# clejacquet/rust-wgpu-raytracing

Hardware: AMD Instinct MI355X
Metric: Mray/s (higher is better)
Workload: dtype f32; 1 GPU; suzanne_lowpoly.obj 1920x1080 1spp primary rays, reference camera + 2 spheres (configs[1]); width=1920, height=1080, spp=1, bounces=0, faces=111, partition=single GPU, frames_in_flight=2, device=AMD Radeon Graphics (gfx950:sramecc+:xnack-)

## Files before the change

include/rwr_hip.h:

```cpp
#ifndef RWR_HIP_H
#define RWR_HIP_H

#include <stddef.h>
#include <stdint.h>

#ifdef __cplusplus
extern "C" {
#endif

#if defined(__GNUC__)
#define RWR_API __attribute__((visibility("default")))
#else
#define RWR_API
#endif

typedef enum rwr_status {
    RWR_OK = 0,
    RWR_ERR_INVALID_ARGUMENT = -1,
    RWR_ERR_HIP = -2,
    RWR_ERR_NOT_READY = -3,
    RWR_ERR_IO = -4,
    RWR_ERR_PARSE = -5,
    RWR_ERR_UNSUPPORTED = -6
} rwr_status;


typedef struct rwr_camera_inv_uniform {
    float viewmodel_inv[4][4];
    float proj_inv[4][4];
    float origin[3];
    uint32_t _padding;
} rwr_camera_inv_uniform;

typedef struct rwr_screen {
    uint32_t width, height;
} rwr_screen;

typedef struct rwr_model_vertex_small {
    float position[3];
    float pad0;
    float tex_coords[2];
    float pad1[2];
} rwr_model_vertex_small;

typedef struct rwr_model_face_small {
    uint32_t indices[3];
    uint32_t pad0;
} rwr_model_face_small;

typedef struct rwr_material_data {
    float ambient[3];  float pad0;
    float diffuse[3];  float pad1;
    float specular[3]; float pad2;
} rwr_material_data;

typedef struct rwr_sphere_buffer_data {
    float center[3];
    float radius;
} rwr_sphere_buffer_data;

typedef struct rwr_triangle_buffer_data {
    float p0[3]; float pad0;
    float p1[3]; float pad1;
    float p2[3]; float pad2;
} rwr_triangle_buffer_data;

typedef struct rwr_instance_raw {
    float model[4][4];
} rwr_instance_raw;

typedef struct rwr_camera {
    float eye[3];
    float target[3];
    float up[3];
    float aspect;
    float fovy;
    float znear;
    float zfar;
} rwr_camera;

typedef struct rwr_render_params {
    uint32_t spp;
    uint32_t max_bounces;
    uint32_t seed;
    uint32_t flags;
} rwr_render_params;

enum {
    RWR_FLAG_AUX_OUTPUTS = 1u << 0,
    RWR_FLAG_NO_CULL     = 1u << 1,
    RWR_FLAG_USE_BVH     = 1u << 2,
    RWR_FLAG_ORTHO_RAYS  = 1u << 3,
    RWR_FLAG_NORMAL_MAP  = 1u << 4,
    RWR_FLAG_ACCUMULATE  = 1u << 5,
    RWR_FLAG_MULTI_BOUNCE = 1u << 6,
    RWR_FLAG_SHADOWS = 1u << 7,
    RWR_FLAG_DENOISE = 1u << 8,
    RWR_FLAG_SKY = 1u << 9,
    RWR_FLAG_MIRRORS = 1u << 10,
    RWR_FLAG_GLASS = 1u << 11,
    RWR_FLAG_REPROJECT = 1u << 12,
    RWR_FLAG_GLOSSY = 1u << 13
};

#define RWR_MAX_BOUNCES 8u

#define RWR_MAX_SPHERES 8
#define RWR_MAX_TRIANGLES 8


typedef struct rwr_context rwr_context;


RWR_API int rwr_ctx_create(int device_id, rwr_context **out_ctx);
RWR_API void rwr_ctx_destroy(rwr_context *ctx);
RWR_API const char *rwr_last_error_string(void);
RWR_API int rwr_device_count(int *out_count);
RWR_API int rwr_ctx_device_info(rwr_context *ctx, char *name, size_t name_cap, int *cu_count, int *wave_size);

RWR_API int rwr_ctx_set_frames_in_flight(rwr_context *ctx, uint32_t n);

RWR_API int rwr_ctx_set_stream(rwr_context *ctx, void *hip_stream);
RWR_API void *rwr_ctx_get_stream(rwr_context *ctx);


RWR_API int rwr_scene_upload_mesh(rwr_context *ctx,
                                  const rwr_model_vertex_small *verts, uint32_t n_verts,
                                  const rwr_model_face_small *faces, uint32_t n_faces,
                                  const rwr_material_data *material,
                                  const uint8_t *rgba8_srgb, uint32_t tex_w, uint32_t tex_h);

RWR_API int rwr_scene_clear(rwr_context *ctx);
RWR_API int rwr_scene_add_mesh(rwr_context *ctx,
                               const rwr_model_vertex_small *verts, uint32_t n_verts,
                               const rwr_model_face_small *faces, uint32_t n_faces,
                               const rwr_material_data *material,
                               const uint8_t *rgba8_srgb, uint32_t tex_w, uint32_t tex_h);
RWR_API int rwr_scene_commit(rwr_context *ctx);

RWR_API int rwr_scene_set_normal_map(rwr_context *ctx, uint32_t part, const uint8_t *rgba8_linear, uint32_t tex_w, uint32_t tex_h);
RWR_API int rwr_scene_part_count(rwr_context *ctx, uint32_t *n_parts);

RWR_API int rwr_scene_set_part_mirror(rwr_context *ctx, uint32_t part, const float *reflectance);
RWR_API int rwr_scene_set_sphere_mirror(rwr_context *ctx, uint32_t sphere, const float *reflectance);
RWR_API int rwr_scene_get_part_mirror(rwr_context *ctx, uint32_t part, int *is_mirror, float reflectance[3]);
RWR_API int rwr_scene_get_sphere_mirror(rwr_context *ctx, uint32_t sphere, int *is_mirror, float reflectance[3]);

RWR_API int rwr_scene_set_part_glass(rwr_context *ctx, uint32_t part, float ior, const float *tint);
RWR_API int rwr_scene_set_sphere_glass(rwr_context *ctx, uint32_t sphere, float ior, const float *tint);
RWR_API int rwr_scene_get_part_glass(rwr_context *ctx, uint32_t part, int *is_glass, float *ior, float tint[3]);
RWR_API int rwr_scene_get_sphere_glass(rwr_context *ctx, uint32_t sphere, int *is_glass, float *ior, float tint[3]);

RWR_API int rwr_scene_set_part_gloss(rwr_context *ctx, uint32_t part, const float *reflectance, float roughness);
RWR_API int rwr_scene_set_sphere_gloss(rwr_context *ctx, uint32_t sphere, const float *reflectance, float roughness);
RWR_API int rwr_scene_get_part_gloss(rwr_context *ctx, uint32_t part, int *is_glossy, float reflectance[3], float *roughness);
RWR_API int rwr_scene_get_sphere_gloss(rwr_context *ctx, uint32_t sphere, int *is_glossy, float reflectance[3], float *roughness);

RWR_API int rwr_scene_set_spheres(rwr_context *ctx, const rwr_sphere_buffer_data *spheres, uint32_t n);

RWR_API int rwr_scene_set_triangles(rwr_context *ctx, const rwr_triangle_buffer_data *triangles, uint32_t n);

RWR_API int rwr_scene_set_instances(rwr_context *ctx, const rwr_instance_raw *instances, uint32_t n);


RWR_API int rwr_resize(rwr_context *ctx, const rwr_screen *screen);

RWR_API int rwr_render(rwr_context *ctx, const rwr_camera_inv_uniform *camera, const rwr_render_params *params);

RWR_API int rwr_render_rows(rwr_context *ctx, const rwr_camera_inv_uniform *camera,
                            const rwr_render_params *params, uint32_t row_begin, uint32_t row_end);

#define RWR_STRIP_ROWS 8u
RWR_API int rwr_render_strips(rwr_context *ctx, const rwr_camera_inv_uniform *camera,
                              const rwr_render_params *params, uint32_t first_strip, uint32_t strip_stride);

RWR_API int rwr_synchronize(rwr_context *ctx);

RWR_API int rwr_readback(rwr_context *ctx, uint8_t *rgba8, float *depth,
                         float *rgba_f32, int32_t *obj_id, float *hit_t);

RWR_API int rwr_get_device_targets(rwr_context *ctx, void **d_rgba8, void **d_depth);

#define RWR_DIST_ID_BYTES 128
RWR_API int rwr_dist_get_unique_id(uint8_t id[RWR_DIST_ID_BYTES]);
RWR_API int rwr_dist_init(rwr_context *ctx, int rank, int world, const uint8_t id[RWR_DIST_ID_BYTES]);
RWR_API int rwr_dist_band(uint32_t rank, uint32_t world, uint32_t height, uint32_t *row_begin, uint32_t *row_end);
RWR_API int rwr_dist_gather_rgba8(rwr_context *ctx, int root);
RWR_API int rwr_dist_gather_strips_rgba8(rwr_context *ctx, int root);
RWR_API int rwr_dist_frame(rwr_context *ctx, void **d_rgba8);
RWR_API int rwr_dist_readback(rwr_context *ctx, uint8_t *rgba8);
RWR_API int rwr_dist_barrier(rwr_context *ctx);
RWR_API int rwr_dist_destroy(rwr_context *ctx);

typedef struct rwr_strip_layout {
    uint32_t n_strips, strips, rows, recv_row, recv_rows_total, owns_tail;
} rwr_strip_layout;
RWR_API int rwr_dist_strip_layout(uint32_t rank, uint32_t world, uint32_t height, rwr_strip_layout *out);
RWR_API int rwr_dist_host_pack_strips(uint32_t rank, uint32_t world, uint32_t width, uint32_t height,
                                      const uint8_t *frame_rgba8, uint8_t *message);
RWR_API int rwr_dist_host_deal_strips(uint32_t world, uint32_t width, uint32_t height, const uint8_t *recv, uint8_t *frame_rgba8);
RWR_API int rwr_host_texture_quads(const uint8_t *rgba8_srgb, uint32_t tex_w, uint32_t tex_h, uint32_t *out);
RWR_API int rwr_dist_loopback_deposit(rwr_context *ctx, uint32_t rank, uint32_t world, int strips);
RWR_API int rwr_dist_loopback_finish(rwr_context *ctx, uint32_t world, int strips);

RWR_API int rwr_timer_begin(rwr_context *ctx);
RWR_API int rwr_timer_end(rwr_context *ctx, float *elapsed_ms);
RWR_API int rwr_timer_stop(rwr_context *ctx);
RWR_API int rwr_timer_elapsed(rwr_context *ctx, float *elapsed_ms);

RWR_API int rwr_ctx_set_kernel_timing(rwr_context *ctx, uint32_t every_n);
RWR_API int rwr_kernel_timing_stats(rwr_context *ctx, double *mean_us, uint32_t *count);

RWR_API int rwr_last_render_stats(rwr_context *ctx, uint64_t *primary_rays, uint64_t *bounce_rays);

RWR_API int rwr_frame_setup_launches(rwr_context *ctx, uint64_t *launches);

RWR_API int rwr_ray_plane_stats(rwr_context *ctx, uint64_t *builds, uint64_t *frames);

RWR_API int rwr_debug_tile_classes(rwr_context *ctx, uint32_t *classes, size_t capacity, uint32_t *grid_x, uint32_t *grid_y);

RWR_API int rwr_debug_tile_cover(rwr_context *ctx, uint32_t *cover, size_t capacity, uint32_t *grid_x, uint32_t *grid_y);

RWR_API int rwr_tile_cover_stats(rwr_context *ctx, uint64_t *frames, uint64_t *tiles_last);

RWR_API int rwr_last_shadow_stats(rwr_context *ctx, uint64_t *shadow_rays, uint64_t *occluded);

RWR_API int rwr_last_glass_stats(rwr_context *ctx, uint64_t *reflected, uint64_t *transmitted, uint64_t *tir);

RWR_API int rwr_last_gloss_stats(rwr_context *ctx, uint64_t *glossy_rays);

RWR_API int rwr_accum_reset(rwr_context *ctx);
RWR_API int rwr_accum_samples(rwr_context *ctx, uint64_t *samples);

typedef struct rwr_denoise_params {
    uint32_t iterations;
    float sigma_color, normal_cos_min, depth_rel;
} rwr_denoise_params;
RWR_API int rwr_denoise_set_params(rwr_context *ctx, const rwr_denoise_params *params);
RWR_API int rwr_denoise_get_params(rwr_context *ctx, rwr_denoise_params *out);

typedef struct rwr_sky_params {
    float zenith[3];
    float horizon[3];
} rwr_sky_params;
#define RWR_SKY_DEFAULTS {{0.5f, 0.7f, 1.0f}, {1.0f, 1.0f, 1.0f}}
#define RWR_SKY_COMPONENT_MAX 16.0f
RWR_API int rwr_sky_set_params(rwr_context *ctx, const rwr_sky_params *params);
RWR_API int rwr_sky_get_params(rwr_context *ctx, rwr_sky_params *out);

typedef struct rwr_reproject_params {
    uint32_t max_history;
    float normal_cos_min, depth_rel;
} rwr_reproject_params;
RWR_API int rwr_reproject_set_params(rwr_context *ctx, const rwr_reproject_params *params);
RWR_API int rwr_reproject_get_params(rwr_context *ctx, rwr_reproject_params *out);
RWR_API int rwr_reproject_reset(rwr_context *ctx);
RWR_API int rwr_reproject_frames(rwr_context *ctx, uint64_t *frames);
RWR_API int rwr_last_reproject_stats(rwr_context *ctx, uint64_t *reused, uint64_t *fresh, uint64_t *background);
RWR_API int rwr_reproject_readback(rwr_context *ctx, float *history_len);

RWR_API int rwr_selftest_exact_math(rwr_context *ctx, uint32_t normalize_count, uint32_t seed, uint64_t out4[4]);

RWR_API int rwr_selftest_exact_div(rwr_context *ctx, uint32_t count, uint32_t seed, uint64_t out4[4]);

RWR_API int rwr_measure_valu_clock(rwr_context *ctx, uint32_t waves_per_simd, double out4[4]);
RWR_API int rwr_clock_probe_start(rwr_context *ctx, uint32_t micros);
RWR_API int rwr_clock_probe_read(rwr_context *ctx, double *shader_mhz);


RWR_API int rwr_camera_build_inv_uniform(const rwr_camera *camera, rwr_camera_inv_uniform *out);

enum { RWR_KEY_FORWARD = 1, RWR_KEY_BACKWARD = 2, RWR_KEY_LEFT = 4, RWR_KEY_RIGHT = 8,
       RWR_KEY_UP = 16, RWR_KEY_DOWN = 32 };
RWR_API int rwr_circle_controller_update(float speed, uint32_t pressed_keys, rwr_camera *camera);

typedef struct rwr_model rwr_model;
RWR_API int rwr_load_model_compute(const char *res_dir, const char *file_name, rwr_model **out_model);
RWR_API void rwr_model_free(rwr_model *model);
RWR_API int rwr_model_info(const rwr_model *model, uint32_t *n_meshes, uint32_t *n_materials,
                           uint32_t *n_verts, uint32_t *n_faces, uint32_t *tex_w, uint32_t *tex_h);
RWR_API const rwr_model_vertex_small *rwr_model_vertices(const rwr_model *model);
RWR_API const rwr_model_face_small *rwr_model_faces(const rwr_model *model);
RWR_API const rwr_material_data *rwr_model_material(const rwr_model *model);
RWR_API const uint8_t *rwr_model_texture_rgba8(const rwr_model *model);
RWR_API int rwr_scene_upload_model(rwr_context *ctx, const rwr_model *model);
RWR_API int rwr_model_part_count(const rwr_model *model, uint32_t *n_parts);
RWR_API int rwr_model_part(const rwr_model *model, uint32_t part,
                           const rwr_model_vertex_small **verts, uint32_t *n_verts,
                           const rwr_model_face_small **faces, uint32_t *n_faces,
                           rwr_material_data *material, const uint8_t **rgba8, uint32_t *tex_w, uint32_t *tex_h);
RWR_API int rwr_scene_upload_model_all(rwr_context *ctx, const rwr_model *model);
RWR_API int rwr_model_part_normal_map(const rwr_model *model, uint32_t part, const uint8_t **rgba8, uint32_t *tex_w, uint32_t *tex_h);

RWR_API int rwr_decode_image_rgba8(const uint8_t *bytes, size_t n_bytes,
                                   uint8_t **out_rgba, uint32_t *out_w, uint32_t *out_h);
RWR_API void rwr_free(void *p);

RWR_API int rwr_write_png_rgba8(const char *path, const uint8_t *rgba8, uint32_t width, uint32_t height,
                                int flip_vertical, int encode_srgb);

RWR_API int rwr_make_instance_grid(uint32_t per_row, float space_between, rwr_instance_raw *out);

#ifdef __cplusplus
}
#endif
#endif
```

rust-wgpu-raytracing_amd/__init__.py:

```python
from __future__ import annotations

import ctypes as C
import os
import subprocess

import numpy as np

_HERE = os.path.dirname(os.path.abspath(__file__))
LIB_PATH = os.environ.get("RWR_HIP_LIB") or os.path.join(_HERE, "lib", "librwr_hip.so")
RES_DIR = os.path.join(_HERE, "res")
HEADER_PATH = os.path.join(os.path.dirname(_HERE), "include", "rwr_hip.h")

CAMERA_INV_DTYPE = np.dtype(
    [("viewmodel_inv", "<f4", (4, 4)), ("proj_inv", "<f4", (4, 4)), ("origin", "<f4", (3,)), ("_padding", "<u4")])
SCREEN_DTYPE = np.dtype([("width", "<u4"), ("height", "<u4")])
VERTEX_DTYPE = np.dtype([("position", "<f4", (3,)), ("pad0", "<f4"), ("tex_coords", "<f4", (2,)), ("pad1", "<f4", (2,))])
FACE_DTYPE = np.dtype([("indices", "<u4", (3,)), ("pad0", "<u4")])
MATERIAL_DTYPE = np.dtype([("ambient", "<f4", (3,)), ("pad0", "<f4"), ("diffuse", "<f4", (3,)), ("pad1", "<f4"),
                           ("specular", "<f4", (3,)), ("pad2", "<f4")])
SPHERE_DTYPE = np.dtype([("center", "<f4", (3,)), ("radius", "<f4")])
INSTANCE_DTYPE = np.dtype([("model", "<f4", (4, 4))])
TRIANGLE_DTYPE = np.dtype([("p0", "<f4", (3,)), ("pad0", "<f4"), ("p1", "<f4", (3,)), ("pad1", "<f4"),
                           ("p2", "<f4", (3,)), ("pad2", "<f4")])
CAMERA_DTYPE = np.dtype([("eye", "<f4", (3,)), ("target", "<f4", (3,)), ("up", "<f4", (3,)),
                         ("aspect", "<f4"), ("fovy", "<f4"), ("znear", "<f4"), ("zfar", "<f4")])
PARAMS_DTYPE = np.dtype([("spp", "<u4"), ("max_bounces", "<u4"), ("seed", "<u4"), ("flags", "<u4")])
assert (CAMERA_INV_DTYPE.itemsize, VERTEX_DTYPE.itemsize, FACE_DTYPE.itemsize, MATERIAL_DTYPE.itemsize,
        SPHERE_DTYPE.itemsize, INSTANCE_DTYPE.itemsize, CAMERA_DTYPE.itemsize) == (144, 32, 16, 48, 16, 64, 52)

FLAG_AUX_OUTPUTS, FLAG_NO_CULL, FLAG_USE_BVH = 1, 2, 4
FLAG_ORTHO_RAYS = 1 << 3
FLAG_NORMAL_MAP = 1 << 4
FLAG_ACCUMULATE = 1 << 5
FLAG_MULTI_BOUNCE = 1 << 6
FLAG_SHADOWS = 1 << 7
FLAG_DENOISE = 1 << 8
DENOISE_PARAMS_DTYPE = np.dtype([("iterations", "<u4"), ("sigma_color", "<f4"), ("normal_cos_min", "<f4"), ("depth_rel", "<f4")])
FLAG_SKY = 1 << 9
SKY_PARAMS_DTYPE = np.dtype([("zenith", "<f4", 3), ("horizon", "<f4", 3)])
FLAG_MIRRORS = 1 << 10
FLAG_GLASS = 1 << 11
FLAG_REPROJECT = 1 << 12
FLAG_GLOSSY = 1 << 13
REPROJECT_PARAMS_DTYPE = np.dtype([("max_history", "<u4"), ("normal_cos_min", "<f4"), ("depth_rel", "<f4")])
MAX_BOUNCES = 8
FLAG_DEBUG_COUNTS, FLAG_ONE_PIXEL_PER_LANE = 1 << 16, 1 << 17
KEY_FORWARD, KEY_BACKWARD, KEY_LEFT, KEY_RIGHT, KEY_UP, KEY_DOWN = 1, 2, 4, 8, 16, 32
OK, ERR_INVALID_ARGUMENT, ERR_HIP, ERR_NOT_READY, ERR_IO, ERR_PARSE, ERR_UNSUPPORTED = 0, -1, -2, -3, -4, -5, -6

REFERENCE_SPHERES = [((0.6, 0.5, -4.0), 0.4), ((0.4, 0.4, -3.0), 0.4)]
CONTROLLER_SPEED = 0.2


class RwrError(RuntimeError):
    def __init__(self, code: int, message: str):
        super().__init__(f"rwr error {code}: {message}")
        self.code = code
        self.message = message


def build(force: bool = False) -> str:
    cmd = ["make", "-C", _HERE, "-j4"] + (["-B"] if force else [])
    r = subprocess.run(cmd, capture_output=True, text=True)
    if r.returncode != 0:
        raise RuntimeError("building librwr_hip.so failed:\n" + r.stdout + r.stderr)
    return LIB_PATH


_lib = None


def lib() -> C.CDLL:
    global _lib
    if _lib is not None:
        return _lib
    if not os.path.exists(LIB_PATH):
        raise FileNotFoundError(
            f"{LIB_PATH} is missing: run `python -c 'import __graft_entry__ as g; g.build()'` "
            "(there is no CPU fallback for the render path)")
    try:
        import torch
    except Exception:
        pass
    L = C.CDLL(LIB_PATH)
    vp, u32, i32, f32 = C.c_void_p, C.c_uint32, C.c_int, C.c_float
    L.rwr_last_error_string.restype = C.c_char_p
    L.rwr_ctx_get_stream.restype = vp
    for name in ("rwr_model_vertices", "rwr_model_faces", "rwr_model_material", "rwr_model_texture_rgba8"):
        getattr(L, name).restype = vp
        getattr(L, name).argtypes = [vp]
    sigs = {
        "rwr_ctx_create": [i32, vp], "rwr_ctx_destroy": [vp], "rwr_device_count": [vp],
        "rwr_ctx_device_info": [vp, vp, C.c_size_t, vp, vp], "rwr_ctx_set_stream": [vp, vp], "rwr_ctx_get_stream": [vp],
        "rwr_scene_upload_mesh": [vp, vp, u32, vp, u32, vp, vp, u32, u32],
        "rwr_scene_clear": [vp], "rwr_scene_add_mesh": [vp, vp, u32, vp, u32, vp, vp, u32, u32], "rwr_scene_commit": [vp],
        "rwr_model_part_count": [vp, vp], "rwr_model_part": [vp, u32, vp, vp, vp, vp, vp, vp, vp, vp],
        "rwr_scene_upload_model_all": [vp, vp], "rwr_model_part_normal_map": [vp, u32, vp, vp, vp],
        "rwr_scene_set_normal_map": [vp, u32, vp, u32, u32], "rwr_scene_part_count": [vp, vp],
        "rwr_scene_set_spheres": [vp, vp, u32], "rwr_scene_set_triangles": [vp, vp, u32], "rwr_scene_set_instances": [vp, vp, u32],
        "rwr_resize": [vp, vp], "rwr_render": [vp, vp, vp], "rwr_render_rows": [vp, vp, vp, u32, u32], "rwr_render_strips": [vp, vp, vp, u32, u32],
        "rwr_synchronize": [vp], "rwr_readback": [vp, vp, vp, vp, vp, vp], "rwr_get_device_targets": [vp, vp, vp],
        "rwr_timer_begin": [vp], "rwr_timer_end": [vp, vp], "rwr_timer_stop": [vp], "rwr_timer_elapsed": [vp, vp], "rwr_last_render_stats": [vp, vp, vp],
        "rwr_last_shadow_stats": [vp, vp, vp], "rwr_frame_setup_launches": [vp, vp], "rwr_ray_plane_stats": [vp, vp, vp],
        "rwr_debug_tile_classes": [vp, vp, C.c_size_t, vp, vp],
        "rwr_debug_tile_cover": [vp, vp, C.c_size_t, vp, vp], "rwr_tile_cover_stats": [vp, vp, vp],
        "rwr_accum_reset": [vp], "rwr_accum_samples": [vp, vp],
        "rwr_denoise_set_params": [vp, vp], "rwr_denoise_get_params": [vp, vp],
        "rwr_sky_set_params": [vp, vp], "rwr_sky_get_params": [vp, vp],
        "rwr_reproject_set_params": [vp, vp], "rwr_reproject_get_params": [vp, vp], "rwr_reproject_reset": [vp],
        "rwr_reproject_frames": [vp, vp], "rwr_last_reproject_stats": [vp, vp, vp, vp], "rwr_reproject_readback": [vp, vp],
        "rwr_scene_set_part_mirror": [vp, u32, vp], "rwr_scene_set_sphere_mirror": [vp, u32, vp],
        "rwr_scene_get_part_mirror": [vp, u32, vp, vp], "rwr_scene_get_sphere_mirror": [vp, u32, vp, vp],
        "rwr_scene_set_part_glass": [vp, u32, f32, vp], "rwr_scene_set_sphere_glass": [vp, u32, f32, vp],
        "rwr_scene_get_part_glass": [vp, u32, vp, vp, vp], "rwr_scene_get_sphere_glass": [vp, u32, vp, vp, vp],
        "rwr_last_glass_stats": [vp, vp, vp, vp],
        "rwr_scene_set_part_gloss": [vp, u32, vp, f32], "rwr_scene_set_sphere_gloss": [vp, u32, vp, f32],
        "rwr_scene_get_part_gloss": [vp, u32, vp, vp, vp], "rwr_scene_get_sphere_gloss": [vp, u32, vp, vp, vp],
        "rwr_last_gloss_stats": [vp, vp],
        "rwr_camera_build_inv_uniform": [vp, vp], "rwr_circle_controller_update": [f32, u32, vp],
        "rwr_load_model_compute": [C.c_char_p, C.c_char_p, vp], "rwr_model_free": [vp],
        "rwr_model_info": [vp, vp, vp, vp, vp, vp, vp], "rwr_scene_upload_model": [vp, vp],
        "rwr_decode_image_rgba8": [vp, C.c_size_t, vp, vp, vp], "rwr_free": [vp],
        "rwr_make_instance_grid": [u32, f32, vp],
        "rwr_write_png_rgba8": [C.c_char_p, vp, u32, u32, i32, i32],
        "rwr_ctx_set_kernel_timing": [vp, u32], "rwr_kernel_timing_stats": [vp, vp, vp],
        "rwr_selftest_exact_math": [vp, u32, u32, vp], "rwr_selftest_exact_div": [vp, u32, u32, vp], "rwr_ctx_set_frames_in_flight": [vp, u32],
        "rwr_dist_get_unique_id": [vp], "rwr_dist_init": [vp, i32, i32, vp], "rwr_dist_band": [u32, u32, u32, vp, vp],
        "rwr_dist_gather_rgba8": [vp, i32], "rwr_dist_gather_strips_rgba8": [vp, i32], "rwr_dist_frame": [vp, vp], "rwr_dist_readback": [vp, vp],
        "rwr_dist_barrier": [vp], "rwr_dist_destroy": [vp],
        "rwr_dist_strip_layout": [u32, u32, u32, vp], "rwr_dist_host_pack_strips": [u32, u32, u32, u32, vp, vp],
        "rwr_dist_host_deal_strips": [u32, u32, u32, vp, vp], "rwr_host_texture_quads": [vp, u32, u32, vp],
        "rwr_dist_loopback_deposit": [vp, u32, u32, i32], "rwr_dist_loopback_finish": [vp, u32, i32],
        "rwr_measure_valu_clock": [vp, u32, vp], "rwr_clock_probe_start": [vp, u32], "rwr_clock_probe_read": [vp, vp],
    }
    _NEWER_ENTRY_POINTS = ("rwr_last_shadow_stats", "rwr_denoise_set_params", "rwr_denoise_get_params", "rwr_frame_setup_launches", "rwr_ray_plane_stats", "rwr_debug_tile_classes", "rwr_debug_tile_cover", "rwr_tile_cover_stats",
                           "rwr_sky_set_params", "rwr_sky_get_params", "rwr_scene_set_part_mirror", "rwr_scene_set_sphere_mirror",
                           "rwr_scene_get_part_mirror", "rwr_scene_get_sphere_mirror", "rwr_scene_set_part_glass", "rwr_scene_set_sphere_glass",
                           "rwr_scene_get_part_glass", "rwr_scene_get_sphere_glass", "rwr_last_glass_stats",
                           "rwr_reproject_set_params", "rwr_reproject_get_params", "rwr_reproject_reset", "rwr_reproject_frames",
                           "rwr_last_reproject_stats", "rwr_reproject_readback", "rwr_scene_set_part_gloss", "rwr_scene_set_sphere_gloss",
                           "rwr_scene_get_part_gloss", "rwr_scene_get_sphere_gloss", "rwr_last_gloss_stats")
    for name, argtypes in sigs.items():
        fn = getattr(L, name, None)
        if fn is None and name in _NEWER_ENTRY_POINTS and os.environ.get("RWR_HIP_LIB"):
            continue
        if fn is None:
            raise AttributeError(f"{LIB_PATH} does not export {name}")
        fn.argtypes = argtypes
        if name not in ("rwr_ctx_destroy", "rwr_model_free", "rwr_free", "rwr_ctx_get_stream"):
            fn.restype = C.c_int
        elif name != "rwr_ctx_get_stream":
            fn.restype = None
    _lib = L
    return L


def _check(rc: int):
    if rc != OK:
        raise RwrError(rc, lib().rwr_last_error_string().decode("utf-8", "replace"))


def _p(a):
    return None if a is None else a.ctypes.data_as(C.c_void_p)


def make_camera(eye=(0, 0, 0), target=(0, 0, -1), up=(0, 1, 0), aspect=1.0, fovy=60.0, znear=0.1, zfar=100.0):
    cam = np.zeros(1, dtype=CAMERA_DTYPE)
    cam["eye"], cam["target"], cam["up"] = eye, target, up
    cam["aspect"], cam["fovy"], cam["znear"], cam["zfar"] = aspect, fovy, znear, zfar
    return cam


def camera_build_inv_uniform(cam: np.ndarray) -> np.ndarray:
    out = np.zeros(1, dtype=CAMERA_INV_DTYPE)
    _check(lib().rwr_camera_build_inv_uniform(_p(cam), _p(out)))
    return out


def circle_controller_update(cam: np.ndarray, keys: int, speed: float = CONTROLLER_SPEED) -> np.ndarray:
    cam = cam.copy()
    _check(lib().rwr_circle_controller_update(speed, keys, _p(cam)))
    return cam


def make_screen(w: int, h: int) -> np.ndarray:
    s = np.zeros(1, dtype=SCREEN_DTYPE)
    s["width"], s["height"] = w, h
    return s


def make_spheres(spec=REFERENCE_SPHERES) -> np.ndarray:
    s = np.zeros(len(spec), dtype=SPHERE_DTYPE)
    for i, (c, r) in enumerate(spec):
        s[i]["center"], s[i]["radius"] = c, r
    return s


def make_triangles(spec=()) -> np.ndarray:
    t = np.zeros(len(spec), dtype=TRIANGLE_DTYPE)
    for i, (p0, p1, p2) in enumerate(spec):
        t[i]["p0"], t[i]["p1"], t[i]["p2"] = p0, p1, p2
    return t


def make_params(spp=1, max_bounces=0, seed=0, flags=0) -> np.ndarray:
    p = np.zeros(1, dtype=PARAMS_DTYPE)
    p["spp"], p["max_bounces"], p["seed"], p["flags"] = spp, max_bounces, seed, flags
    return p


def make_instance_grid(per_row: int, space_between: float = 3.0) -> np.ndarray:
    out = np.zeros(per_row * per_row, dtype=INSTANCE_DTYPE)
    _check(lib().rwr_make_instance_grid(per_row, space_between, _p(out)))
    return out


def decode_image_rgba8(data: bytes) -> np.ndarray:
    buf = np.frombuffer(data, dtype=np.uint8)
    out = C.c_void_p()
    w, h = C.c_uint32(), C.c_uint32()
    _check(lib().rwr_decode_image_rgba8(_p(buf), len(data), C.byref(out), C.byref(w), C.byref(h)))
    try:
        arr = np.ctypeslib.as_array(C.cast(out, C.POINTER(C.c_uint8)), shape=(h.value, w.value, 4)).copy()
    finally:
        lib().rwr_free(out)
    return arr


def write_png(path: str, rgba8: np.ndarray, flip_vertical: bool = True, encode_srgb: bool = False):
    rgba8 = np.ascontiguousarray(rgba8, dtype=np.uint8)
    h, w = rgba8.shape[:2]
    _check(lib().rwr_write_png_rgba8(path.encode(), _p(rgba8), w, h, int(flip_vertical), int(encode_srgb)))


def load_model_compute(file_name: str, res_dir: str = RES_DIR) -> dict:
    L = lib()
    h = C.c_void_p()
    _check(L.rwr_load_model_compute(res_dir.encode(), file_name.encode(), C.byref(h)))
    try:
        n = [C.c_uint32() for _ in range(6)]
        _check(L.rwr_model_info(h, *[C.byref(x) for x in n]))
        n_meshes, n_materials, n_verts, n_faces, tw, th = [x.value for x in n]
        verts = np.frombuffer(C.string_at(L.rwr_model_vertices(h), n_verts * 32), dtype=VERTEX_DTYPE).copy()
        faces = np.frombuffer(C.string_at(L.rwr_model_faces(h), n_faces * 16), dtype=FACE_DTYPE).copy()
        material = np.frombuffer(C.string_at(L.rwr_model_material(h), 48), dtype=MATERIAL_DTYPE).copy()
        tex = np.frombuffer(C.string_at(L.rwr_model_texture_rgba8(h), tw * th * 4), dtype=np.uint8).reshape(th, tw, 4).copy()
        nmap = _part_normal_map(L, h, 0)
    finally:
        L.rwr_model_free(h)
    return {"vertices": verts, "faces": faces, "material": material, "texture": tex, "normal_map": nmap,
            "n_meshes": n_meshes, "n_materials": n_materials}


def _part_normal_map(L, h, part):
    pn, nw, nh = C.c_void_p(), C.c_uint32(), C.c_uint32()
    _check(L.rwr_model_part_normal_map(h, part, C.byref(pn), C.byref(nw), C.byref(nh)))
    if not pn.value:
        return None
    return np.frombuffer(C.string_at(pn, nw.value * nh.value * 4), dtype=np.uint8).reshape(nh.value, nw.value, 4).copy()



def load_model_parts(file_name: str, res_dir: str = RES_DIR) -> list:
    L = lib()
    h = C.c_void_p()
    _check(L.rwr_load_model_compute(res_dir.encode(), file_name.encode(), C.byref(h)))
    parts = []
    try:
        n = C.c_uint32()
        _check(L.rwr_model_part_count(h, C.byref(n)))
        for i in range(n.value):
            pv, pf, pt = C.c_void_p(), C.c_void_p(), C.c_void_p()
            nv, nf, tw, th = C.c_uint32(), C.c_uint32(), C.c_uint32(), C.c_uint32()
            mat = np.zeros(1, dtype=MATERIAL_DTYPE)
            _check(L.rwr_model_part(h, i, C.byref(pv), C.byref(nv), C.byref(pf), C.byref(nf), _p(mat), C.byref(pt), C.byref(tw), C.byref(th)))
            parts.append({
                "vertices": np.frombuffer(C.string_at(pv, nv.value * 32), dtype=VERTEX_DTYPE).copy(),
                "faces": np.frombuffer(C.string_at(pf, nf.value * 16), dtype=FACE_DTYPE).copy(),
                "material": mat,
                "texture": np.frombuffer(C.string_at(pt, tw.value * th.value * 4), dtype=np.uint8).reshape(th.value, tw.value, 4).copy(),
                "normal_map": _part_normal_map(L, h, i),
            })
    finally:
        L.rwr_model_free(h)
    return parts


DIST_ID_BYTES = 128
STRIP_ROWS = 8


def dist_get_unique_id() -> bytes:
    buf = (C.c_uint8 * DIST_ID_BYTES)()
    _check(lib().rwr_dist_get_unique_id(buf))
    return bytes(buf)


def dist_band(rank: int, world: int, height: int) -> tuple[int, int]:
    a, b = C.c_uint32(), C.c_uint32()
    _check(lib().rwr_dist_band(rank, world, height, C.byref(a), C.byref(b)))
    return a.value, b.value


class _StripLayout(C.Structure):
    _fields_ = [(n, C.c_uint32) for n in ("n_strips", "strips", "rows", "recv_row", "recv_rows_total", "owns_tail")]


def dist_strip_layout(rank: int, world: int, height: int) -> dict:
    out = _StripLayout()
    _check(lib().rwr_dist_strip_layout(rank, world, height, C.byref(out)))
    return {n: int(getattr(out, n)) for n, _ in _StripLayout._fields_}


def dist_host_pack_strips(rank: int, world: int, frame: np.ndarray) -> np.ndarray:
    frame = np.ascontiguousarray(frame, np.uint8)
    h, w = frame.shape[:2]
    lay = dist_strip_layout(rank, world, h)
    msg = np.zeros((max(1, lay["strips"] * STRIP_ROWS), w, 4), np.uint8)
    _check(lib().rwr_dist_host_pack_strips(rank, world, w, h, _p(frame), _p(msg)))
    return msg[:lay["rows"]]


def host_texture_quads(rgba8: np.ndarray) -> np.ndarray:
    rgba8 = np.ascontiguousarray(rgba8, np.uint8)
    h, w = rgba8.shape[:2]
    out = np.zeros((h + 1, w + 1, 4), np.uint32)
    _check(lib().rwr_host_texture_quads(_p(rgba8), w, h, _p(out)))
    return out


def dist_host_deal_strips(world: int, recv: np.ndarray, height: int) -> np.ndarray:
    recv = np.ascontiguousarray(recv, np.uint8)
    w = recv.shape[1]
    assert recv.shape[0] == dist_strip_layout(0, world, height)["recv_rows_total"]
    frame = np.zeros((height, w, 4), np.uint8)
    _check(lib().rwr_dist_host_deal_strips(world, w, height, _p(recv), _p(frame)))
    return frame


def device_count() -> int:
    n = C.c_int()
    lib().rwr_device_count(C.byref(n))
    return n.value


class Context:

    def __init__(self, device_id: int = 0):
        self._h = C.c_void_p()
        _check(lib().rwr_ctx_create(device_id, C.byref(self._h)))
        self.width = self.height = 0

    def close(self):
        if getattr(self, "_h", None):
            lib().rwr_ctx_destroy(self._h)
            self._h = None

    def __del__(self):
        try:
            self.close()
        except Exception:
            pass

    def __enter__(self):
        return self

    def __exit__(self, *exc):
        self.close()

    def device_info(self) -> dict:
        name = C.create_string_buffer(256)
        cu, ws = C.c_int(), C.c_int()
        _check(lib().rwr_ctx_device_info(self._h, name, 256, C.byref(cu), C.byref(ws)))
        return {"name": name.value.decode(), "cu_count": cu.value, "wave_size": ws.value}

    def set_stream(self, hip_stream: int | None):
        _check(lib().rwr_ctx_set_stream(self._h, C.c_void_p(hip_stream or 0)))

    def upload_mesh(self, vertices, faces, material, texture):
        vertices = np.ascontiguousarray(vertices, dtype=VERTEX_DTYPE)
        faces = np.ascontiguousarray(faces, dtype=FACE_DTYPE)
        material = np.ascontiguousarray(material, dtype=MATERIAL_DTYPE)
        texture = np.ascontiguousarray(texture, dtype=np.uint8)
        th, tw = texture.shape[:2] if texture.ndim == 3 else (0, 0)
        _check(lib().rwr_scene_upload_mesh(self._h, _p(vertices), len(vertices), _p(faces), len(faces),
                                           _p(material), _p(texture), tw, th))

    def upload_model(self, model: dict):
        self.upload_mesh(model["vertices"], model["faces"], model["material"], model["texture"])
        if model.get("normal_map") is not None and len(model["faces"]):
            self.set_normal_map(0, model["normal_map"])

    def set_normal_map(self, part: int, rgba8_linear):
        if rgba8_linear is None:
            _check(lib().rwr_scene_set_normal_map(self._h, part, None, 0, 0))
            return
        t = np.ascontiguousarray(rgba8_linear, dtype=np.uint8)
        _check(lib().rwr_scene_set_normal_map(self._h, part, _p(t), t.shape[1], t.shape[0]))

    def upload_parts(self, parts: list):
        _check(lib().rwr_scene_clear(self._h))
        for m in parts:
            vertices = np.ascontiguousarray(m["vertices"], dtype=VERTEX_DTYPE)
            faces = np.ascontiguousarray(m["faces"], dtype=FACE_DTYPE)
            material = np.ascontiguousarray(m["material"], dtype=MATERIAL_DTYPE)
            texture = np.ascontiguousarray(m["texture"], dtype=np.uint8)
            th, tw = texture.shape[:2]
            _check(lib().rwr_scene_add_mesh(self._h, _p(vertices), len(vertices), _p(faces), len(faces), _p(material),
                                            _p(texture), tw, th))
            if m.get("normal_map") is not None and len(faces):
                n = C.c_uint32()
                _check(lib().rwr_scene_part_count(self._h, C.byref(n)))
                self.set_normal_map(n.value - 1, m["normal_map"])
        _check(lib().rwr_scene_commit(self._h))

    def set_spheres(self, spheres):
        spheres = np.ascontiguousarray(spheres, dtype=SPHERE_DTYPE)
        _check(lib().rwr_scene_set_spheres(self._h, _p(spheres) if len(spheres) else None, len(spheres)))

    @staticmethod
    def _reflectance(reflectance):
        if reflectance is None:
            return None
        r = np.ascontiguousarray(reflectance, dtype=np.float32)
        if r.shape != (3,):
            raise ValueError("reflectance: three floats, or None")
        return r

    def set_part_mirror(self, part: int, reflectance=(1.0, 1.0, 1.0)):
        r = self._reflectance(reflectance)
        _check(lib().rwr_scene_set_part_mirror(self._h, part, _p(r)))

    def set_sphere_mirror(self, sphere: int, reflectance=(1.0, 1.0, 1.0)):
        r = self._reflectance(reflectance)
        _check(lib().rwr_scene_set_sphere_mirror(self._h, sphere, _p(r)))

    def _get_mirror(self, fn, index: int):
        on = C.c_int(0)
        r = np.zeros(3, np.float32)
        _check(fn(self._h, index, C.byref(on), _p(r)))
        return r if on.value else None

    def get_part_mirror(self, part: int):
        return self._get_mirror(lib().rwr_scene_get_part_mirror, part)

    def get_sphere_mirror(self, sphere: int):
        return self._get_mirror(lib().rwr_scene_get_sphere_mirror, sphere)

    def set_part_glass(self, part: int, ior: float = 1.5, tint=(1.0, 1.0, 1.0)):
        t = self._reflectance(tint)
        _check(lib().rwr_scene_set_part_glass(self._h, part, ior, _p(t)))

    def set_sphere_glass(self, sphere: int, ior: float = 1.5, tint=(1.0, 1.0, 1.0)):
        t = self._reflectance(tint)
        _check(lib().rwr_scene_set_sphere_glass(self._h, sphere, ior, _p(t)))

    def _get_glass(self, fn, index: int):
        on = C.c_int(0)
        ior = C.c_float(0.0)
        t = np.zeros(3, np.float32)
        _check(fn(self._h, index, C.byref(on), C.byref(ior), _p(t)))
        return (float(ior.value), t) if on.value else None

    def get_part_glass(self, part: int):
        return self._get_glass(lib().rwr_scene_get_part_glass, part)

    def get_sphere_glass(self, sphere: int):
        return self._get_glass(lib().rwr_scene_get_sphere_glass, sphere)

    def last_glass_stats(self):
        a, b, c = C.c_uint64(0), C.c_uint64(0), C.c_uint64(0)
        _check(lib().rwr_last_glass_stats(self._h, C.byref(a), C.byref(b), C.byref(c)))
        return int(a.value), int(b.value), int(c.value)

    def set_part_gloss(self, part: int, roughness: float = 0.25, reflectance=(1.0, 1.0, 1.0)):
        r = self._reflectance(reflectance)
        _check(lib().rwr_scene_set_part_gloss(self._h, part, _p(r), roughness))

    def set_sphere_gloss(self, sphere: int, roughness: float = 0.25, reflectance=(1.0, 1.0, 1.0)):
        r = self._reflectance(reflectance)
        _check(lib().rwr_scene_set_sphere_gloss(self._h, sphere, _p(r), roughness))

    def _get_gloss(self, fn, index: int):
        on = C.c_int(0)
        rough = C.c_float(0.0)
        r = np.zeros(3, np.float32)
        _check(fn(self._h, index, C.byref(on), _p(r), C.byref(rough)))
        return (float(rough.value), r) if on.value else None

    def get_part_gloss(self, part: int):
        return self._get_gloss(lib().rwr_scene_get_part_gloss, part)

    def get_sphere_gloss(self, sphere: int):
        return self._get_gloss(lib().rwr_scene_get_sphere_gloss, sphere)

    def last_gloss_stats(self):
        a = C.c_uint64(0)
        _check(lib().rwr_last_gloss_stats(self._h, C.byref(a)))
        return int(a.value)

    def set_triangles(self, triangles):
        triangles = np.ascontiguousarray(triangles, dtype=TRIANGLE_DTYPE)
        _check(lib().rwr_scene_set_triangles(self._h, _p(triangles) if len(triangles) else None, len(triangles)))

    def set_instances(self, instances):
        n = 0 if instances is None else len(instances)
        arr = None if n == 0 else np.ascontiguousarray(instances, dtype=INSTANCE_DTYPE)
        _check(lib().rwr_scene_set_instances(self._h, _p(arr), n))

    def resize(self, width: int, height: int):
        _check(lib().rwr_resize(self._h, _p(make_screen(width, height))))
        self.width, self.height = width, height

    def render(self, cam_inv, params=None, rows=None, strips=None):
        if strips is not None:
            _check(lib().rwr_render_strips(self._h, _p(cam_inv), _p(params), strips[0], strips[1]))
        elif rows is None:
            _check(lib().rwr_render(self._h, _p(cam_inv), _p(params)))
        else:
            _check(lib().rwr_render_rows(self._h, _p(cam_inv), _p(params), rows[0], rows[1]))

    def render_call(self, cam_inv, params, rows=None, strips=None):
        fn, h = (lib().rwr_render_strips if strips is not None else lib().rwr_render_rows), self._h
        a, b = _p(cam_inv), _p(params)
        if strips is None and rows is None:
            rows = (0, self.height)
        r0, r1 = (C.c_uint32(strips[0]), C.c_uint32(strips[1])) if strips is not None else (C.c_uint32(rows[0]), C.c_uint32(rows[1]))

        def call(_keep=(cam_inv, params)):
            rc = fn(h, a, b, r0, r1)
            if rc:
                _check(rc)

        return call

    def loop_call(self, cam: np.ndarray, keys: list[int], params, speed: float = CONTROLLER_SPEED, render: bool = True):
        L, h = lib(), self._h
        upd, inv, ren = L.rwr_circle_controller_update, L.rwr_camera_build_inv_uniform, L.rwr_render
        uni = np.zeros(1, dtype=CAMERA_INV_DTYPE)
        pc, pu, pp = _p(cam), _p(uni), _p(params)
        sp = C.c_float(speed)
        masks = [C.c_uint32(k) for k in keys]
        state = [0]

        def call(_keep=(cam, uni, params)):
            i = state[0]
            state[0] = i + 1 if i + 1 < len(masks) else 0
            rc = upd(sp, masks[i], pc) or inv(pc, pu) or (ren(h, pu, pp) if render else 0)
            if rc:
                _check(rc)

        return call

    def synchronize(self):
        _check(lib().rwr_synchronize(self._h))

    def readback(self, aux: bool = False) -> dict:
        h, w = self.height, self.width
        out = {"color": np.zeros((h, w, 4), np.uint8), "depth": np.zeros((h, w), np.float32)}
        if aux:
            out["color_f32"] = np.zeros((h, w, 4), np.float32)
            out["obj_id"] = np.zeros((h, w), np.int32)
            out["hit_t"] = np.zeros((h, w), np.float32)
        _check(lib().rwr_readback(self._h, _p(out["color"]), _p(out["depth"]), _p(out.get("color_f32")),
                                  _p(out.get("obj_id")), _p(out.get("hit_t"))))
        return out

    def device_targets(self) -> tuple[int, int]:
        a, b = C.c_void_p(), C.c_void_p()
        _check(lib().rwr_get_device_targets(self._h, C.byref(a), C.byref(b)))
        return a.value, b.value

    def timer_begin(self):
        _check(lib().rwr_timer_begin(self._h))

    def timer_end(self) -> float:
        ms = C.c_float()
        _check(lib().rwr_timer_end(self._h, C.byref(ms)))
        return ms.value

    def timer_stop(self):
        _check(lib().rwr_timer_stop(self._h))

    def timer_elapsed(self) -> float:
        ms = C.c_float()
        _check(lib().rwr_timer_elapsed(self._h, C.byref(ms)))
        return ms.value

    def set_frames_in_flight(self, n: int):
        _check(lib().rwr_ctx_set_frames_in_flight(self._h, n))

    def set_kernel_timing(self, every_n: int):
        _check(lib().rwr_ctx_set_kernel_timing(self._h, every_n))

    def kernel_timing_stats(self) -> tuple[float, int]:
        mean, n = C.c_double(), C.c_uint32()
        _check(lib().rwr_kernel_timing_stats(self._h, C.byref(mean), C.byref(n)))
        return mean.value, n.value

    def selftest_exact_math(self, normalize_count: int = 1 << 30, seed: int = 1) -> tuple[int, int, int, int]:
        out = (C.c_uint64 * 4)()
        _check(lib().rwr_selftest_exact_math(self._h, normalize_count, seed, out))
        return tuple(int(v) for v in out)

    def selftest_exact_div(self, count: int = 1 << 30, seed: int = 1) -> tuple[int, int, int, int]:
        out = (C.c_uint64 * 4)()
        _check(lib().rwr_selftest_exact_div(self._h, count, seed, out))
        return tuple(int(v) for v in out)

    def measure_valu_clock(self, waves_per_simd: int = 8) -> dict:
        out = (C.c_double * 4)()
        _check(lib().rwr_measure_valu_clock(self._h, waves_per_simd, out))
        return {"shader_mhz": out[0], "cycles_per_v_fma_f32": out[1], "cycles_per_v_pk_fma_f32": out[2], "shader_mhz_pk": out[3]}

    def dist_init(self, rank: int, world: int, unique_id: bytes):
        assert len(unique_id) == DIST_ID_BYTES
        buf = (C.c_uint8 * DIST_ID_BYTES).from_buffer_copy(unique_id)
        _check(lib().rwr_dist_init(self._h, rank, world, buf))

    def dist_gather(self, root: int = 0):
        _check(lib().rwr_dist_gather_rgba8(self._h, root))

    def dist_gather_call(self, root: int = 0, strips: bool = False):
        fn, h, r = (lib().rwr_dist_gather_strips_rgba8 if strips else lib().rwr_dist_gather_rgba8), self._h, C.c_int(root)

        def call():
            rc = fn(h, r)
            if rc:
                _check(rc)

        return call

    def dist_loopback_deposit(self, rank: int, world: int, strips: bool = True):
        _check(lib().rwr_dist_loopback_deposit(self._h, rank, world, 1 if strips else 0))

    def dist_loopback_finish(self, world: int, strips: bool = True):
        _check(lib().rwr_dist_loopback_finish(self._h, world, 1 if strips else 0))

    def dist_readback(self) -> np.ndarray:
        out = np.zeros((self.height, self.width, 4), np.uint8)
        _check(lib().rwr_dist_readback(self._h, _p(out)))
        return out

    def dist_barrier(self):
        _check(lib().rwr_dist_barrier(self._h))

    def dist_destroy(self):
        _check(lib().rwr_dist_destroy(self._h))

    def clock_probe_start(self, micros: int):
        _check(lib().rwr_clock_probe_start(self._h, micros))

    def clock_probe_read(self) -> float:
        mhz = C.c_double()
        _check(lib().rwr_clock_probe_read(self._h, C.byref(mhz)))
        return mhz.value

    def last_render_stats(self) -> tuple[int, int]:
        a, b = C.c_uint64(), C.c_uint64()
        _check(lib().rwr_last_render_stats(self._h, C.byref(a), C.byref(b)))
        return a.value, b.value

    def frame_setup_launches(self) -> int:
        n = C.c_uint64()
        _check(lib().rwr_frame_setup_launches(self._h, C.byref(n)))
        return n.value

    def ray_plane_stats(self) -> tuple[int, int]:
        a, b = C.c_uint64(), C.c_uint64()
        _check(lib().rwr_ray_plane_stats(self._h, C.byref(a), C.byref(b)))
        return a.value, b.value

    def tile_classes(self) -> np.ndarray:
        gx, gy = C.c_uint32(), C.c_uint32()
        _check(lib().rwr_debug_tile_classes(self._h, None, 0, C.byref(gx), C.byref(gy)))
        words = np.empty(4 * gx.value * gy.value, np.uint32)
        _check(lib().rwr_debug_tile_classes(self._h, _p(words), words.size, C.byref(gx), C.byref(gy)))
        return np.ascontiguousarray(words.reshape(gy.value, gx.value, 2, 2).transpose(0, 2, 1, 3).reshape(2 * gy.value, 2 * gx.value))

    def tile_cover(self) -> np.ndarray:
        gx, gy = C.c_uint32(), C.c_uint32()
        _check(lib().rwr_debug_tile_cover(self._h, None, 0, C.byref(gx), C.byref(gy)))
        words = np.empty(4 * gx.value * gy.value, np.uint32)
        _check(lib().rwr_debug_tile_cover(self._h, _p(words), words.size, C.byref(gx), C.byref(gy)))
        return np.ascontiguousarray(words.reshape(gy.value, gx.value, 2, 2).transpose(0, 2, 1, 3).reshape(2 * gy.value, 2 * gx.value))

    def tile_cover_stats(self) -> tuple[int, int]:
        a, b = C.c_uint64(), C.c_uint64()
        _check(lib().rwr_tile_cover_stats(self._h, C.byref(a), C.byref(b)))
        return a.value, b.value

    def last_shadow_stats(self) -> tuple[int, int]:
        a, b = C.c_uint64(), C.c_uint64()
        _check(lib().rwr_last_shadow_stats(self._h, C.byref(a), C.byref(b)))
        return a.value, b.value

    def accum_reset(self):
        _check(lib().rwr_accum_reset(self._h))

    def accum_samples(self) -> int:
        n = C.c_uint64()
        _check(lib().rwr_accum_samples(self._h, C.byref(n)))
        return n.value

    def set_denoise_params(self, iterations=None, sigma_color=None, normal_cos_min=None, depth_rel=None):
        given = {"iterations": iterations, "sigma_color": sigma_color, "normal_cos_min": normal_cos_min, "depth_rel": depth_rel}
        if all(v is None for v in given.values()):
            _check(lib().rwr_denoise_set_params(self._h, None))
            return
        p = np.zeros(1, dtype=DENOISE_PARAMS_DTYPE)
        for k, v in self.denoise_params().items():
            p[k] = v if given[k] is None else given[k]
        _check(lib().rwr_denoise_set_params(self._h, _p(p)))

    def denoise_params(self) -> dict:
        p = np.zeros(1, dtype=DENOISE_PARAMS_DTYPE)
        _check(lib().rwr_denoise_get_params(self._h, _p(p)))
        return {"iterations": int(p["iterations"][0]), "sigma_color": float(p["sigma_color"][0]),
                "normal_cos_min": float(p["normal_cos_min"][0]), "depth_rel": float(p["depth_rel"][0])}

    def set_reproject_params(self, max_history=None, normal_cos_min=None, depth_rel=None):
        given = {"max_history": max_history, "normal_cos_min": normal_cos_min, "depth_rel": depth_rel}
        if all(v is None for v in given.values()):
            _check(lib().rwr_reproject_set_params(self._h, None))
            return
        p = np.zeros(1, dtype=REPROJECT_PARAMS_DTYPE)
        for k, v in self.reproject_params().items():
            p[k] = v if given[k] is None else given[k]
        _check(lib().rwr_reproject_set_params(self._h, _p(p)))

    def reproject_params(self) -> dict:
        p = np.zeros(1, dtype=REPROJECT_PARAMS_DTYPE)
        _check(lib().rwr_reproject_get_params(self._h, _p(p)))
        return {"max_history": int(p["max_history"][0]), "normal_cos_min": float(p["normal_cos_min"][0]), "depth_rel": float(p["depth_rel"][0])}

    def reproject_reset(self):
        _check(lib().rwr_reproject_reset(self._h))

    def reproject_frames(self) -> int:
        n = C.c_uint64()
        _check(lib().rwr_reproject_frames(self._h, C.byref(n)))
        return n.value

    def last_reproject_stats(self) -> tuple[int, int, int]:
        a, b, c = C.c_uint64(0), C.c_uint64(0), C.c_uint64(0)
        _check(lib().rwr_last_reproject_stats(self._h, C.byref(a), C.byref(b), C.byref(c)))
        return int(a.value), int(b.value), int(c.value)

    def reproject_history(self) -> np.ndarray:
        out = np.zeros((self.height, self.width), np.float32)
        _check(lib().rwr_reproject_readback(self._h, _p(out)))
        return out

    def sky_set_params(self, zenith=None, horizon=None):
        if zenith is None and horizon is None:
            _check(lib().rwr_sky_set_params(self._h, None))
            return
        p = np.zeros(1, dtype=SKY_PARAMS_DTYPE)
        now = self.sky_get_params()
        p["zenith"] = now["zenith"] if zenith is None else np.asarray(zenith, np.float32)
        p["horizon"] = now["horizon"] if horizon is None else np.asarray(horizon, np.float32)
        _check(lib().rwr_sky_set_params(self._h, _p(p)))

    def sky_get_params(self) -> dict:
        p = np.zeros(1, dtype=SKY_PARAMS_DTYPE)
        _check(lib().rwr_sky_get_params(self._h, _p(p)))
        return {"zenith": p["zenith"][0].copy(), "horizon": p["horizon"][0].copy()}


def csrc_tree() -> str:
    import hashlib

    h = hashlib.sha256()
    files = []
    for sub in ("csrc", "host"):
        d = os.path.join(_HERE, sub)
        files += [os.path.join(d, f) for f in os.listdir(d) if f.endswith((".h", ".hpp", ".hip", ".cpp"))]
    files += [os.path.join(_HERE, "Makefile"), HEADER_PATH]
    for f in sorted(files):
        h.update(os.path.relpath(f, _HERE).encode())
        with open(f, "rb") as fh:
            h.update(fh.read())
    return h.hexdigest()[:16]


def exported_symbols_declared_in_header() -> list[str]:
    import re

    with open(HEADER_PATH, "r") as fh:
        text = fh.read()
    return sorted(set(re.findall(r"RWR_API\s+[^;(]*?\b(rwr_[a-z0-9_]+)\s*\(", text)))
```

rust-wgpu-raytracing_amd/csrc/context.cpp:

```cpp
#include <hip/hip_runtime.h>

#include <algorithm>
#include <cmath>
#include <cstdarg>
#include <cstdio>
#include <cstdlib>
#include <new>
#include <string>
#include <vector>

#include "rwr_context.h"

namespace rwr {

static thread_local std::string g_last_error;

int set_error(int code, const char *fmt, ...)
{
    char buf[512];
    va_list ap;
    va_start(ap, fmt);
    vsnprintf(buf, sizeof buf, fmt, ap);
    va_end(ap);
    g_last_error = buf;
    return code;
}

hipError_t ensure_frame_buffers(rwr_context *ctx)
{
    const uint32_t total = (uint32_t)instanced_faces(ctx->n_faces, ctx->n_instances);
    for (uint32_t i = 0; i < ctx->n_slots; i++) {
        FrameSlot &sl = ctx->slots[i];
        const void *const before[4] = {sl.d_ftris.ptr, sl.d_tnum.ptr, sl.d_ray_colp.ptr, sl.d_ray_row.ptr};
        hipError_t e = hipSuccess;
        if (total && (e = sl.d_ftris.ensure(total)) == hipSuccess) e = sl.d_tnum.ensure(total);
        if (e == hipSuccess && ctx->screen.width) {
            e = sl.d_ray_colp.ensure(2u * (size_t)(((ctx->screen.width + 63u) / 64u) * 32u));
            if (e == hipSuccess) e = sl.d_ray_row.ensure(ctx->screen.height + 8u);
        }
        if (before[0] != sl.d_ftris.ptr || before[1] != sl.d_tnum.ptr || before[2] != sl.d_ray_colp.ptr || before[3] != sl.d_ray_row.ptr)
            sl.records_key.clear();
        if (before[2] != sl.d_ray_colp.ptr || before[3] != sl.d_ray_row.ptr) sl.forget_ray_plane();
        if (e != hipSuccess) return e;
    }
    return hipSuccess;
}

}

using namespace rwr;

namespace {

hipError_t ensure_slot_targets(rwr_context *ctx, uint32_t i)
{
    FrameSlot &sl = ctx->slots[i];
    const size_t n = (size_t)ctx->screen.width * ctx->screen.height;
    if (n == 0) return hipSuccess;
    hipError_t e;
    if ((e = sl.d_color.ensure(n * 4)) != hipSuccess || (e = sl.d_depth.ensure(n)) != hipSuccess) return e;
    if ((e = hipMemsetAsync(sl.d_color.ptr, 0, n * 4, sl.stream)) != hipSuccess) return e;
    return hipMemsetAsync(sl.d_depth.ptr, 0, n * sizeof(float), sl.stream);
}

bool env_u64(const char *name, uint64_t *v) { const char *e = std::getenv(name); if (e) *v = std::strtoull(e, nullptr, 10); return e != nullptr; }
bool env_u32(const char *name, uint32_t *v) { uint64_t w = 0; const bool set = env_u64(name, &w); if (set) *v = (uint32_t)w; return set; }
bool env_f32(const char *name, float *v) { const char *e = std::getenv(name); if (e) *v = (float)std::atof(e); return e != nullptr; }
bool env_flag(const char *name, bool *v) { const char *e = std::getenv(name); if (e) *v = std::atoi(e) != 0; return e != nullptr; }

void read_tunables(rwr_context *ctx)
{
    env_u32("RWR_WAVE_CULL_MIN", &ctx->wave_cull_min);
    env_flag("RWR_ONE_PIXEL_PER_LANE", &ctx->force_one_pixel);
    env_flag("RWR_FRAME_GRAPH", &ctx->frame_graph);
    if (env_flag("RWR_FUSED_SETUP", &ctx->fused_setup)) ctx->fused_setup_force = ctx->fused_setup;
    env_flag("RWR_TILE_LISTS", &ctx->tile_lists);
    env_flag("RWR_SETUP_CACHE", &ctx->setup_cache);
    env_flag("RWR_RAY_PLANE", &ctx->ray_plane);
    env_flag("RWR_TILE_CLASS", &ctx->tile_class);
    env_flag("RWR_TILE_COVER", &ctx->tile_cover);
    env_f32("RWR_AUTO_BVH_FACE_PX", &ctx->auto_bvh_face_px);
    if (env_u32("RWR_WF_GROUP", &ctx->wf_group)) ctx->wf_group = std::min(kWfMaxGroup, std::max(1u, ctx->wf_group));
    bool stats = false, wide = false;
    if (env_flag("RWR_WF_STATS", &stats) && stats && ctx->d_wf_dbg.ensure(4) == hipSuccess) {
        (void)hipMemset(ctx->d_wf_dbg.ptr, 0, 32);
        wf_trace_launch_counts(ctx->wf_launches_before);
    }
    if (env_u32("RWR_WF_OVERLAP", &ctx->wf_queues)) ctx->wf_queues = std::min(kWfMaxQueues, std::max(1u, ctx->wf_queues));
    env_u32("RWR_WF_ZSPLIT", &ctx->wf_z_split);
    env_u32("RWR_WF_PACKET_RAYS", &ctx->wf_packet_dense_rays);
    if (env_flag("RWR_WF_WIDE_LANE", &wide)) ctx->wf_wide_lane = wide ? 1 : 0;
    if (env_u32("RWR_WF_LANE_ITEMS", &ctx->wf_lane_items)) ctx->wf_lane_items = std::max(1u, ctx->wf_lane_items);
    env_u32("RWR_WF_MIN_PACKET_POOLS", &ctx->wf_min_packet_pools);
    env_f32("RWR_WF_PACKET_EXTENT", &ctx->wf_packet_extent);
    env_f32("RWR_WF_PACKET_FILL", &ctx->wf_packet_fill);
    env_u32("RWR_BIN_CAPACITY", &ctx->bin_min_capacity);
    env_u32("RWR_BIN_MIN_FACES", &ctx->bin_min_faces);
    if (env_u64("RWR_ACCUM_MAX_SAMPLES", &ctx->accum_max)) ctx->accum_max = std::min<uint64_t>(1u << 24, std::max<uint64_t>(1u, ctx->accum_max));
}
}

extern "C" {

const char *rwr_last_error_string(void) { return g_last_error.c_str(); }

int rwr_device_count(int *out_count)
{
    if (!out_count) return set_error(RWR_ERR_INVALID_ARGUMENT, "out_count is NULL");
    int n = 0;
    hipError_t e = hipGetDeviceCount(&n);
    if (e != hipSuccess) {
        *out_count = 0;
        return set_error(RWR_ERR_HIP, "hipGetDeviceCount failed: %s", hipGetErrorString(e));
    }
    *out_count = n;
    return RWR_OK;
}

int rwr_ctx_create(int device_id, rwr_context **out_ctx)
{
    if (!out_ctx) return set_error(RWR_ERR_INVALID_ARGUMENT, "out_ctx is NULL");
    *out_ctx = nullptr;
    int n = 0;
    hipError_t e = hipGetDeviceCount(&n);
    if (e != hipSuccess || n == 0)
        return set_error(RWR_ERR_HIP, "no HIP device available (%s)", e == hipSuccess ? "count 0" : hipGetErrorString(e));
    if (device_id < 0 || device_id >= n)
        return set_error(RWR_ERR_INVALID_ARGUMENT, "device_id %d out of range [0,%d)", device_id, n);
    rwr_context *ctx = new (std::nothrow) rwr_context();
    if (!ctx) return set_error(RWR_ERR_HIP, "out of host memory");
    ctx->device = device_id;
    DeviceGuard g(device_id);
    if (!g.ok) {
        delete ctx;
        return set_error(RWR_ERR_HIP, "hipSetDevice(%d) failed", device_id);
    }
    if ((e = hipStreamCreateWithFlags(&ctx->own_stream.h, hipStreamNonBlocking)) != hipSuccess ||
        (e = hipEventCreate(&ctx->ev_begin.h)) != hipSuccess || (e = hipEventCreate(&ctx->ev_end.h)) != hipSuccess) {
        rwr_ctx_destroy(ctx);
        return set_error(RWR_ERR_HIP, "stream/event creation failed: %s", hipGetErrorString(e));
    }
    {
        float lut[256];
        build_srgb_lut(lut);
        if ((e = ctx->d_srgb_lut.ensure(256)) != hipSuccess || (e = hipMemcpy(ctx->d_srgb_lut.ptr, lut, sizeof lut, hipMemcpyHostToDevice)) != hipSuccess) {
            rwr_ctx_destroy(ctx);
            return set_error(RWR_ERR_HIP, "sRGB table upload failed: %s", hipGetErrorString(e));
        }
    }
    ctx->stream = ctx->own_stream;
    ctx->slots[0].stream = ctx->stream;
    (void)preload_kernels();
    read_tunables(ctx);
    *out_ctx = ctx;
    return RWR_OK;
}

void rwr_ctx_destroy(rwr_context *ctx)
{
    if (!ctx) return;
    DeviceGuard g(ctx->device);
    (void)sync_all(ctx);
    for (WfState &w : ctx->wf_state)
        for (hipStream_t q : w.streams)
            if (q) (void)hipStreamSynchronize(q);
    if (ctx->probe_stream) (void)hipStreamSynchronize(ctx->probe_stream);
    if (ctx->d_wf_dbg.ptr) {
        unsigned long long h[4] = {0, 0, 0, 0};
        (void)hipMemcpy(h, ctx->d_wf_dbg.ptr, sizeof h, hipMemcpyDeviceToHost);
        std::fprintf(stderr, "rwr wavefront pools: packets %llu pools / %llu rays, per-lane %llu pools / %llu rays (leaf extent %g)\n",
                     h[0], h[1], h[2], h[3], (double)ctx->bvh_leaf_extent);
        uint64_t n[3];
        wf_trace_launch_counts(n);
        std::fprintf(stderr, "rwr wavefront launches: packet %llu, per-lane %llu, per-lane wide %llu\n",
                     (unsigned long long)(n[0] - ctx->wf_launches_before[0]), (unsigned long long)(n[1] - ctx->wf_launches_before[1]),
                     (unsigned long long)(n[2] - ctx->wf_launches_before[2]));
    }
    (void)rwr_dist_destroy(ctx);
    delete ctx;
}

int rwr_ctx_device_info(rwr_context *ctx, char *name, size_t name_cap, int *cu_count, int *wave_size)
{
    if (!ctx) return set_error(RWR_ERR_INVALID_ARGUMENT, "ctx is NULL");
    hipDeviceProp_t prop;
    RWR_HIP_CHECK(hipGetDeviceProperties(&prop, ctx->device));
    if (name && name_cap) {
        std::snprintf(name, name_cap, "%s (%s)", prop.name, prop.gcnArchName);
    }
    if (cu_count) *cu_count = prop.multiProcessorCount;
    if (wave_size) *wave_size = prop.warpSize;
    return RWR_OK;
}

int rwr_ctx_set_stream(rwr_context *ctx, void *hip_stream)
{
    if (!ctx) return set_error(RWR_ERR_INVALID_ARGUMENT, "ctx is NULL");
    DeviceGuard g(ctx->device);
    RWR_HIP_CHECK(sync_all(ctx));
    ctx->stream = hip_stream ? reinterpret_cast<hipStream_t>(hip_stream) : ctx->own_stream;
    ctx->slots[0].stream = ctx->stream;
    return RWR_OK;
}

void *rwr_ctx_get_stream(rwr_context *ctx) { return ctx ? reinterpret_cast<void *>(ctx->stream) : nullptr; }

int rwr_resize(rwr_context *ctx, const rwr_screen *screen)
{
    if (!ctx || !screen) return set_error(RWR_ERR_INVALID_ARGUMENT, "NULL argument");
    if (screen->width == 0 || screen->height == 0) return set_error(RWR_ERR_INVALID_ARGUMENT, "zero-sized screen");
    if ((uint64_t)screen->width * screen->height > (1ull << 30)) return set_error(RWR_ERR_INVALID_ARGUMENT, "screen too large");
    DeviceGuard g(ctx->device);
    RWR_HIP_CHECK(sync_all(ctx));
    ctx->screen = *screen;
    ctx->accum.reset();
    ctx->reproj.reset();
    ctx->last_reproject_frames = 0;
    for (uint32_t i = 0; i < ctx->n_slots; i++) {
        RWR_HIP_CHECK(ensure_slot_targets(ctx, i));
        ctx->slots[i].aux_valid = false;
        ctx->slots[i].forget_ray_plane();
    }
    for (GatherSet &gs : ctx->gather) gs.valid = false;
    RWR_HIP_CHECK(ensure_frame_buffers(ctx));
    return RWR_OK;
}

int rwr_synchronize(rwr_context *ctx)
{
    if (!ctx) return set_error(RWR_ERR_INVALID_ARGUMENT, "ctx is NULL");
    DeviceGuard g(ctx->device);
    RWR_HIP_CHECK(sync_all(ctx));
    for (uint32_t i = 0; i < ctx->n_slots; i++) {
        const int rc = check_fused_frame(ctx, i);
        if (rc != RWR_OK) return rc;
    }
    return RWR_OK;
}

int rwr_readback(rwr_context *ctx, uint8_t *rgba8, float *depth, float *rgba_f32, int32_t *obj_id, float *hit_t)
{
    if (!ctx) return set_error(RWR_ERR_INVALID_ARGUMENT, "ctx is NULL");
    if (ctx->screen.width == 0) return set_error(RWR_ERR_NOT_READY, "rwr_resize has not been called");
    if ((rgba_f32 || obj_id || hit_t) && !ctx->slots[ctx->cur].aux_valid)
        return set_error(RWR_ERR_NOT_READY, "aux planes requested but the last render did not set RWR_FLAG_AUX_OUTPUTS");
    DeviceGuard g(ctx->device);
    const size_t n = (size_t)ctx->screen.width * ctx->screen.height;
    RWR_HIP_CHECK(hipStreamSynchronize(ctx->slots[ctx->cur].stream));
    {
        const int rc = check_fused_frame(ctx, ctx->cur);
        if (rc != RWR_OK) return rc;
    }
    if (rgba8) RWR_HIP_CHECK(hipMemcpy(rgba8, ctx->slots[ctx->cur].d_color.ptr, n * 4, hipMemcpyDeviceToHost));
    if (depth) RWR_HIP_CHECK(hipMemcpy(depth, ctx->slots[ctx->cur].d_depth.ptr, n * sizeof(float), hipMemcpyDeviceToHost));
    if (rgba_f32) RWR_HIP_CHECK(hipMemcpy(rgba_f32, ctx->slots[ctx->cur].d_color_f32.ptr, n * 4 * sizeof(float), hipMemcpyDeviceToHost));
    if (obj_id) RWR_HIP_CHECK(hipMemcpy(obj_id, ctx->slots[ctx->cur].d_obj_id.ptr, n * sizeof(int32_t), hipMemcpyDeviceToHost));
    if (hit_t) RWR_HIP_CHECK(hipMemcpy(hit_t, ctx->slots[ctx->cur].d_hit_t.ptr, n * sizeof(float), hipMemcpyDeviceToHost));
    return RWR_OK;
}

int rwr_get_device_targets(rwr_context *ctx, void **d_rgba8, void **d_depth)
{
    if (!ctx) return set_error(RWR_ERR_INVALID_ARGUMENT, "ctx is NULL");
    if (ctx->screen.width == 0) return set_error(RWR_ERR_NOT_READY, "rwr_resize has not been called");
    if (ctx->cur != 0u) {
        DeviceGuard g(ctx->device);
        FrameSlot &sl = ctx->slots[ctx->cur];
        RWR_HIP_CHECK(hipEventRecord(sl.done, sl.stream));
        RWR_HIP_CHECK(hipStreamWaitEvent(ctx->stream, sl.done, 0));
    }
    if (d_rgba8) *d_rgba8 = ctx->slots[ctx->cur].d_color.ptr;
    if (d_depth) *d_depth = ctx->slots[ctx->cur].d_depth.ptr;
    return RWR_OK;
}

int rwr_ctx_set_frames_in_flight(rwr_context *ctx, uint32_t n)
{
    if (!ctx) return set_error(RWR_ERR_INVALID_ARGUMENT, "ctx is NULL");
    if (n < 1u || n > kMaxFramesInFlight)
        return set_error(RWR_ERR_INVALID_ARGUMENT, "frames in flight must be 1..%u", kMaxFramesInFlight);
    DeviceGuard g(ctx->device);
    RWR_HIP_CHECK(sync_all(ctx));
    for (uint32_t i = 1; i < n; i++) {
        FrameSlot &sl = ctx->slots[i];
        if (!sl.owned) RWR_HIP_CHECK(hipStreamCreateWithFlags(&sl.owned.h, hipStreamNonBlocking));
        if (!sl.done) RWR_HIP_CHECK(hipEventCreateWithFlags(&sl.done.h, hipEventDisableTiming));
        sl.stream = sl.owned;
    }
    for (uint32_t i = n; i < kMaxFramesInFlight; i++) {
        ctx->slots[i].reset();
        ctx->wf_state[i] = WfState{};
        ctx->gather[i] = GatherSet{};
    }
    if (ctx->last_gather >= n) ctx->last_gather = 0;
    if (ctx->last_wf_state >= n) { ctx->last_wf_state = 0; ctx->last_segments = 0; ctx->last_spp = 0; }
    ctx->n_slots = n;
    if (ctx->cur >= n) ctx->cur = 0;
    for (uint32_t i = 0; i < n; i++)
        if (!ctx->slots[i].d_color.ptr) RWR_HIP_CHECK(ensure_slot_targets(ctx, i));
    RWR_HIP_CHECK(ensure_frame_buffers(ctx));
    RWR_HIP_CHECK(sync_all(ctx));
    return RWR_OK;
}

int rwr_timer_begin(rwr_context *ctx)
{
    if (!ctx) return set_error(RWR_ERR_INVALID_ARGUMENT, "ctx is NULL");
    DeviceGuard g(ctx->device);
    if (ctx->n_slots > 1u) RWR_HIP_CHECK(sync_all(ctx));
    RWR_HIP_CHECK(hipEventRecord(ctx->ev_begin, ctx->stream));
    return RWR_OK;
}

int rwr_timer_end(rwr_context *ctx, float *elapsed_ms)
{
    if (!ctx || !elapsed_ms) return set_error(RWR_ERR_INVALID_ARGUMENT, "NULL argument");
    DeviceGuard g(ctx->device);
    const int rc = rwr_timer_stop(ctx);
    return rc == RWR_OK ? rwr_timer_elapsed(ctx, elapsed_ms) : rc;
}

int rwr_timer_stop(rwr_context *ctx)
{
    if (!ctx) return set_error(RWR_ERR_INVALID_ARGUMENT, "ctx is NULL");
    DeviceGuard g(ctx->device);
    for (uint32_t i = 1; i < ctx->n_slots; i++) {
        RWR_HIP_CHECK(hipEventRecord(ctx->slots[i].done, ctx->slots[i].stream));
        RWR_HIP_CHECK(hipStreamWaitEvent(ctx->stream, ctx->slots[i].done, 0));
    }
    RWR_HIP_CHECK(hipEventRecord(ctx->ev_end, ctx->stream));
    return RWR_OK;
}

int rwr_timer_elapsed(rwr_context *ctx, float *elapsed_ms)
{
    if (!ctx || !elapsed_ms) return set_error(RWR_ERR_INVALID_ARGUMENT, "NULL argument");
    DeviceGuard g(ctx->device);
    RWR_HIP_CHECK(hipEventSynchronize(ctx->ev_end));
    RWR_HIP_CHECK(hipEventElapsedTime(elapsed_ms, ctx->ev_begin, ctx->ev_end));
    return RWR_OK;
}

int rwr_ctx_set_kernel_timing(rwr_context *ctx, uint32_t every_n)
{
    if (!ctx) return set_error(RWR_ERR_INVALID_ARGUMENT, "ctx is NULL");
    ctx->timing_every = every_n;
    ctx->timing_calls = 0;
    ctx->timing_pairs = 0;
    return RWR_OK;
}

int rwr_kernel_timing_stats(rwr_context *ctx, double *mean_us, uint32_t *count)
{
    if (!ctx || !mean_us || !count) return set_error(RWR_ERR_INVALID_ARGUMENT, "NULL argument");
    DeviceGuard g(ctx->device);
    RWR_HIP_CHECK(sync_all(ctx));
    double sum = 0.0;
    for (uint32_t i = 0; i < ctx->timing_pairs; i++) {
        float ms = 0.0f;
        RWR_HIP_CHECK(hipEventElapsedTime(&ms, ctx->timing_events[2 * i], ctx->timing_events[2 * i + 1]));
        sum += ms * 1e3;
    }
    *count = ctx->timing_pairs;
    *mean_us = ctx->timing_pairs ? sum / ctx->timing_pairs : 0.0;
    return RWR_OK;
}

int rwr_last_render_stats(rwr_context *ctx, uint64_t *primary_rays, uint64_t *bounce_rays)
{
    if (!ctx) return set_error(RWR_ERR_INVALID_ARGUMENT, "ctx is NULL");
    if (ctx->last_spp && ctx->last_had_bounce) {
        DeviceGuard g(ctx->device);
        std::vector<uint32_t> counts((size_t)ctx->last_segments * 4u);
        RWR_HIP_CHECK(hipStreamSynchronize(ctx->slots[ctx->cur].stream));
        RWR_HIP_CHECK(hipMemcpy(counts.data(), ctx->wf_state[ctx->last_wf_state].d_wave_total.ptr, counts.size() * sizeof(uint32_t), hipMemcpyDeviceToHost));
        ctx->last_bounce = 0;
        for (uint32_t c : counts) ctx->last_bounce += c;
    }
    if (primary_rays) *primary_rays = ctx->last_primary;
    if (bounce_rays) *bounce_rays = ctx->last_bounce;
    return RWR_OK;
}

int rwr_frame_setup_launches(rwr_context *ctx, uint64_t *launches)
{
    if (!ctx || !launches) return set_error(RWR_ERR_INVALID_ARGUMENT, "NULL argument");
    *launches = ctx->setup_launches;
    return RWR_OK;
}

int rwr_ray_plane_stats(rwr_context *ctx, uint64_t *builds, uint64_t *frames)
{
    if (!ctx || !builds || !frames) return set_error(RWR_ERR_INVALID_ARGUMENT, "NULL argument");
    *builds = ctx->ray_plane_builds;
    *frames = ctx->ray_plane_frames;
    return RWR_OK;
}

int rwr_last_shadow_stats(rwr_context *ctx, uint64_t *shadow_rays, uint64_t *occluded)
{
    if (!ctx || !shadow_rays || !occluded) return set_error(RWR_ERR_INVALID_ARGUMENT, "NULL argument");
    unsigned long long counts[2] = {0ull, 0ull};
    if (ctx->last_shadows && ctx->wf_state[ctx->last_wf_state].d_shadow_counts.ptr) {
        DeviceGuard g(ctx->device);
        RWR_HIP_CHECK(hipStreamSynchronize(ctx->slots[ctx->cur].stream));
        RWR_HIP_CHECK(hipMemcpy(counts, ctx->wf_state[ctx->last_wf_state].d_shadow_counts.ptr, sizeof counts, hipMemcpyDeviceToHost));
    }
    *shadow_rays = counts[0];
    *occluded = counts[1];
    return RWR_OK;
}

int rwr_last_glass_stats(rwr_context *ctx, uint64_t *reflected, uint64_t *transmitted, uint64_t *tir)
{
    if (!ctx || !reflected || !transmitted || !tir) return set_error(RWR_ERR_INVALID_ARGUMENT, "NULL argument");
    unsigned long long counts[3] = {0ull, 0ull, 0ull};
    if (ctx->last_glass && ctx->wf_state[ctx->last_wf_state].d_glass_counts.ptr) {
        DeviceGuard g(ctx->device);
        RWR_HIP_CHECK(hipStreamSynchronize(ctx->slots[ctx->cur].stream));
        RWR_HIP_CHECK(hipMemcpy(counts, ctx->wf_state[ctx->last_wf_state].d_glass_counts.ptr, sizeof counts, hipMemcpyDeviceToHost));
    }
    *reflected = counts[0];
    *transmitted = counts[1];
    *tir = counts[2];
    return RWR_OK;
}

int rwr_last_gloss_stats(rwr_context *ctx, uint64_t *glossy_rays)
{
    if (!ctx || !glossy_rays) return set_error(RWR_ERR_INVALID_ARGUMENT, "NULL argument");
    unsigned long long count = 0ull;
    if (ctx->last_gloss && ctx->wf_state[ctx->last_wf_state].d_glass_counts.ptr) {
        DeviceGuard g(ctx->device);
        RWR_HIP_CHECK(hipStreamSynchronize(ctx->slots[ctx->cur].stream));
        RWR_HIP_CHECK(hipMemcpy(&count, ctx->wf_state[ctx->last_wf_state].d_glass_counts.ptr + 3, sizeof count, hipMemcpyDeviceToHost));
    }
    *glossy_rays = count;
    return RWR_OK;
}

int rwr_denoise_set_params(rwr_context *ctx, const rwr_denoise_params *params)
{
    if (!ctx) return set_error(RWR_ERR_INVALID_ARGUMENT, "ctx is NULL");
    if (!params) {
        ctx->denoise = kDenoiseDefaults;
        return RWR_OK;
    }
    const rwr_denoise_params p = *params;
    if (p.iterations < 1u || p.iterations > 5u) return set_error(RWR_ERR_INVALID_ARGUMENT, "denoise iterations %u: 1 ... 5", p.iterations);
    const float s2 = p.sigma_color * p.sigma_color, inv4 = 1.0f / s2 * 256.0f;
    if (!(p.sigma_color > 0.0f) || !std::isfinite(p.sigma_color) || !(s2 > 0.0f) || !std::isfinite(inv4))
        return set_error(RWR_ERR_INVALID_ARGUMENT, "denoise sigma_color %g: positive, finite, 256 / sigma^2 finite", (double)p.sigma_color);
    if (std::isnan(p.normal_cos_min)) return set_error(RWR_ERR_INVALID_ARGUMENT, "denoise normal_cos_min is NaN");
    if (!(p.depth_rel >= 0.0f)) return set_error(RWR_ERR_INVALID_ARGUMENT, "denoise depth_rel %g: >= 0", (double)p.depth_rel);
    ctx->denoise = p;
    return RWR_OK;
}

int rwr_denoise_get_params(rwr_context *ctx, rwr_denoise_params *out)
{
    if (!ctx || !out) return set_error(RWR_ERR_INVALID_ARGUMENT, "NULL argument");
    *out = ctx->denoise;
    return RWR_OK;
}

int rwr_reproject_set_params(rwr_context *ctx, const rwr_reproject_params *params)
{
    if (!ctx) return set_error(RWR_ERR_INVALID_ARGUMENT, "ctx is NULL");
    rwr_reproject_params p = kReprojectDefaults;
    if (params) p = *params;
    if (p.max_history < 1u || p.max_history > 1024u) return set_error(RWR_ERR_INVALID_ARGUMENT, "reproject max_history %u: 1 ... 1024", p.max_history);
    if (!(p.normal_cos_min >= -1.0f && p.normal_cos_min <= 1.0f))
        return set_error(RWR_ERR_INVALID_ARGUMENT, "reproject normal_cos_min %g: finite, -1 ... 1", (double)p.normal_cos_min);
    if (!(p.depth_rel >= 0.0f) || !std::isfinite(p.depth_rel))
        return set_error(RWR_ERR_INVALID_ARGUMENT, "reproject depth_rel %g: finite, >= 0", (double)p.depth_rel);
    ctx->reproject = p;
    ctx->reproj.key.clear();
    return RWR_OK;
}

int rwr_reproject_get_params(rwr_context *ctx, rwr_reproject_params *out)
{
    if (!ctx || !out) return set_error(RWR_ERR_INVALID_ARGUMENT, "NULL argument");
    *out = ctx->reproject;
    return RWR_OK;
}

int rwr_reproject_reset(rwr_context *ctx)
{
    if (!ctx) return set_error(RWR_ERR_INVALID_ARGUMENT, "ctx is NULL");
    ctx->reproj.key.clear();
    return RWR_OK;
}

int rwr_reproject_frames(rwr_context *ctx, uint64_t *frames)
{
    if (!ctx || !frames) return set_error(RWR_ERR_INVALID_ARGUMENT, "NULL argument");
    *frames = ctx->last_reproject_frames;
    return RWR_OK;
}

int rwr_last_reproject_stats(rwr_context *ctx, uint64_t *reused, uint64_t *fresh, uint64_t *background)
{
    if (!ctx || !reused || !fresh || !background) return set_error(RWR_ERR_INVALID_ARGUMENT, "NULL argument");
    unsigned long long counts[3] = {0ull, 0ull, 0ull};
    if (ctx->last_reproject_frames != 0 && ctx->reproj.d_counts.ptr) {
        DeviceGuard g(ctx->device);
        RWR_HIP_CHECK(hipStreamSynchronize(ctx->slots[ctx->cur].stream));
        RWR_HIP_CHECK(hipMemcpy(counts, ctx->reproj.d_counts.ptr + 3u * ctx->last_reproject_set, sizeof counts, hipMemcpyDeviceToHost));
    }
    *reused = counts[0];
    *fresh = counts[1];
    *background = counts[2];
    return RWR_OK;
}

int rwr_reproject_readback(rwr_context *ctx, float *history_len)
{
    if (!ctx || !history_len) return set_error(RWR_ERR_INVALID_ARGUMENT, "NULL argument");
    const DeviceBuffer<float4> &plane = ctx->reproj.d_colour[ctx->last_reproject_set];
    const size_t n = (size_t)ctx->screen.width * ctx->screen.height;
    if (ctx->last_reproject_frames == 0 || !plane.ptr || plane.count < n)
        return set_error(RWR_ERR_NOT_READY, "the last render did not set RWR_FLAG_REPROJECT");
    DeviceGuard g(ctx->device);
    RWR_HIP_CHECK(hipStreamSynchronize(ctx->slots[ctx->cur].stream));
    std::vector<float4> records(n);
    RWR_HIP_CHECK(hipMemcpy(records.data(), plane.ptr, n * sizeof(float4), hipMemcpyDeviceToHost));
    for (size_t i = 0; i < n; i++) history_len[i] = records[i].w;
    return RWR_OK;
}

int rwr_sky_set_params(rwr_context *ctx, const rwr_sky_params *params)
{
    if (!ctx) return set_error(RWR_ERR_INVALID_ARGUMENT, "ctx is NULL");
    if (!params) {
        ctx->sky = kSkyDefaults;
        return RWR_OK;
    }
    const rwr_sky_params p = *params;
    for (int c = 0; c < 3; c++) {
        if (!(p.zenith[c] >= 0.0f && p.zenith[c] <= RWR_SKY_COMPONENT_MAX))
            return set_error(RWR_ERR_INVALID_ARGUMENT, "sky zenith[%d] %g: finite, 0 ... 16", c, (double)p.zenith[c]);
        if (!(p.horizon[c] >= 0.0f && p.horizon[c] <= RWR_SKY_COMPONENT_MAX))
            return set_error(RWR_ERR_INVALID_ARGUMENT, "sky horizon[%d] %g: finite, 0 ... 16", c, (double)p.horizon[c]);
    }
    ctx->sky = p;
    return RWR_OK;
}

int rwr_sky_get_params(rwr_context *ctx, rwr_sky_params *out)
{
    if (!ctx || !out) return set_error(RWR_ERR_INVALID_ARGUMENT, "NULL argument");
    *out = ctx->sky;
    return RWR_OK;
}

int rwr_accum_reset(rwr_context *ctx)
{
    if (!ctx) return set_error(RWR_ERR_INVALID_ARGUMENT, "ctx is NULL");
    ctx->accum.key.clear();
    ctx->accum.samples = 0;
    return RWR_OK;
}

int rwr_accum_samples(rwr_context *ctx, uint64_t *samples)
{
    if (!ctx || !samples) return set_error(RWR_ERR_INVALID_ARGUMENT, "NULL argument");
    *samples = ctx->last_accum_samples;
    return RWR_OK;
}

}
```

rust-wgpu-raytracing_amd/csrc/diagnostics.cpp:

```cpp
#include <hip/hip_runtime.h>

#include <algorithm>
#include <vector>

#include "rwr_context.h"

using namespace rwr;

template <typename Launch>
static int run_selftest(rwr_context *ctx, uint64_t out4[4], Launch launch)
{
    if (!ctx || !out4) return set_error(RWR_ERR_INVALID_ARGUMENT, "NULL argument");
    DeviceGuard g(ctx->device);
    DeviceBuffer<unsigned long long> d_out;
    RWR_HIP_CHECK(d_out.ensure(4));
    RWR_HIP_CHECK(hipMemsetAsync(d_out.ptr, 0, 4 * sizeof(unsigned long long), ctx->stream));
    RWR_HIP_CHECK(launch(d_out.ptr));
    unsigned long long h[4];
    RWR_HIP_CHECK(hipMemcpyAsync(h, d_out.ptr, sizeof(h), hipMemcpyDeviceToHost, ctx->stream));
    RWR_HIP_CHECK(hipStreamSynchronize(ctx->stream));
    for (int k = 0; k < 4; k++) out4[k] = h[k];
    return RWR_OK;
}

extern "C" {

int rwr_selftest_exact_math(rwr_context *ctx, uint32_t normalize_count, uint32_t seed, uint64_t out4[4])
{
    return run_selftest(ctx, out4, [&](unsigned long long *d) { return launch_selftest_exact_math(ctx->stream, d, normalize_count, seed); });
}

int rwr_selftest_exact_div(rwr_context *ctx, uint32_t count, uint32_t seed, uint64_t out4[4])
{
    return run_selftest(ctx, out4, [&](unsigned long long *d) { return launch_selftest_exact_div(ctx->stream, d, count, seed); });
}

int rwr_debug_tile_classes(rwr_context *ctx, uint32_t *classes, size_t capacity, uint32_t *grid_x, uint32_t *grid_y)
{
    if (!ctx || !grid_x || !grid_y) return set_error(RWR_ERR_INVALID_ARGUMENT, "NULL argument");
    const rwr_context::LastClasses lc = ctx->last_classes;
    const size_t n = (size_t)lc.gx * lc.gy * 4u;
    if (n == 0 || lc.slot >= ctx->n_slots || ctx->slots[lc.slot].d_tile_lists.count < tile_list_words(lc.gx, lc.gy))
        return set_error(RWR_ERR_NOT_READY, "the frame rendered last has no tile classes (they come with the per-tile face sets of the "
                         "two-pixel frame kernel's two-launch form: a scene of at most %u faces, culled)", kTileListMaxFaces);
    *grid_x = lc.gx;
    *grid_y = lc.gy;
    if (!classes) return RWR_OK;
    if (capacity < n) return set_error(RWR_ERR_INVALID_ARGUMENT, "room for %zu class words, the frame has %zu", capacity, n);
    DeviceGuard g(ctx->device);
    FrameSlot &sl = ctx->slots[lc.slot];
    RWR_HIP_CHECK(hipMemcpyAsync(classes, sl.d_tile_lists.ptr + n * kTileListWords, n * sizeof(uint32_t), hipMemcpyDeviceToHost, sl.stream));
    RWR_HIP_CHECK(hipStreamSynchronize(sl.stream));
    return RWR_OK;
}

int rwr_debug_tile_cover(rwr_context *ctx, uint32_t *cover, size_t capacity, uint32_t *grid_x, uint32_t *grid_y)
{
    if (!ctx || !grid_x || !grid_y) return set_error(RWR_ERR_INVALID_ARGUMENT, "NULL argument");
    const rwr_context::LastClasses lc = ctx->last_classes;
    const size_t n = (size_t)lc.gx * lc.gy * 4u;
    if (n == 0 || lc.slot >= ctx->n_slots || ctx->slots[lc.slot].d_tile_lists.count < tile_list_words(lc.gx, lc.gy))
        return set_error(RWR_ERR_NOT_READY, "the frame rendered last has no cover words (they lie beside the tile classes: rwr_debug_tile_classes)");
    *grid_x = lc.gx;
    *grid_y = lc.gy;
    if (!cover) return RWR_OK;
    if (capacity < n) return set_error(RWR_ERR_INVALID_ARGUMENT, "room for %zu cover words, the frame has %zu", capacity, n);
    DeviceGuard g(ctx->device);
    FrameSlot &sl = ctx->slots[lc.slot];
    RWR_HIP_CHECK(hipMemcpyAsync(cover, sl.d_tile_lists.ptr + n * (kTileListWords + 1u), n * sizeof(uint32_t), hipMemcpyDeviceToHost, sl.stream));
    RWR_HIP_CHECK(hipStreamSynchronize(sl.stream));
    return RWR_OK;
}

int rwr_tile_cover_stats(rwr_context *ctx, uint64_t *frames, uint64_t *tiles_last)
{
    if (!ctx || !frames || !tiles_last) return set_error(RWR_ERR_INVALID_ARGUMENT, "NULL argument");
    *frames = ctx->tile_cover_frames;
    *tiles_last = 0;
    if (ctx->last_cover_frames < 2u) return RWR_OK;
    uint32_t gx = 0, gy = 0;
    int rc = rwr_debug_tile_cover(ctx, nullptr, 0, &gx, &gy);
    if (rc != RWR_OK) return rc;
    std::vector<uint32_t> words((size_t)gx * gy * 4u);
    if ((rc = rwr_debug_tile_cover(ctx, words.data(), words.size(), &gx, &gy)) != RWR_OK) return rc;
    for (uint32_t w : words) *tiles_last += w == kTileCovered ? 1u : 0u;
    return RWR_OK;
}

int rwr_measure_valu_clock(rwr_context *ctx, uint32_t waves_per_simd, double out4[4])
{
    if (!ctx || !out4) return set_error(RWR_ERR_INVALID_ARGUMENT, "NULL argument");
    if (waves_per_simd < 1u || waves_per_simd > 8u) return set_error(RWR_ERR_INVALID_ARGUMENT, "waves_per_simd must be 1..8");
    DeviceGuard g(ctx->device);
    hipDeviceProp_t prop;
    RWR_HIP_CHECK(hipGetDeviceProperties(&prop, ctx->device));
    const uint32_t n_wg = (uint32_t)prop.multiProcessorCount * waves_per_simd, n_waves = n_wg * 4u, iters = 1u << 15;
    DeviceBuffer<ulonglong2> d_out;
    OwnedEvent e0, e1;
    RWR_HIP_CHECK(d_out.ensure(n_waves));
    RWR_HIP_CHECK(hipEventCreate(&e0.h));
    RWR_HIP_CHECK(hipEventCreate(&e1.h));
    std::vector<ulonglong2> h(n_waves);
    RWR_HIP_CHECK(sync_all(ctx));
    for (int mode = 0; mode < 2; mode++) {
        RWR_HIP_CHECK(launch_measure_valu(ctx->stream, mode, d_out.ptr, n_wg, iters));
        RWR_HIP_CHECK(hipEventRecord(e0, ctx->stream));
        RWR_HIP_CHECK(launch_measure_valu(ctx->stream, mode, d_out.ptr, n_wg, iters));
        RWR_HIP_CHECK(hipEventRecord(e1, ctx->stream));
        RWR_HIP_CHECK(hipMemcpyAsync(h.data(), d_out.ptr, n_waves * sizeof(ulonglong2), hipMemcpyDeviceToHost, ctx->stream));
        RWR_HIP_CHECK(hipStreamSynchronize(ctx->stream));
        float ms = 0.0f;
        RWR_HIP_CHECK(hipEventElapsedTime(&ms, e0, e1));
        std::vector<double> mhz(n_waves);
        for (uint32_t i = 0; i < n_waves; i++) mhz[i] = h[i].y ? (double)h[i].x / (double)h[i].y * 100.0 : 0.0;
        std::nth_element(mhz.begin(), mhz.begin() + n_waves / 2, mhz.end());
        const double clock_mhz = mhz[n_waves / 2];
        const double instr_per_simd = (double)n_waves / (4.0 * prop.multiProcessorCount) * iters * 8.0;
        const double per_instr = (double)ms * 1e-3 * clock_mhz * 1e6 / instr_per_simd;
        if (mode == 0) { out4[0] = clock_mhz; out4[1] = per_instr; }
        else { out4[2] = per_instr; out4[3] = clock_mhz; }
    }
    return RWR_OK;
}

int rwr_clock_probe_start(rwr_context *ctx, uint32_t micros)
{
    if (!ctx) return set_error(RWR_ERR_INVALID_ARGUMENT, "ctx is NULL");
    if (micros == 0u || micros > 100000u) return set_error(RWR_ERR_INVALID_ARGUMENT, "probe duration must be 1..100000 us");
    DeviceGuard g(ctx->device);
    if (!ctx->probe_stream) RWR_HIP_CHECK(hipStreamCreateWithFlags(&ctx->probe_stream.h, hipStreamNonBlocking));
    RWR_HIP_CHECK(ctx->d_probe.ensure(1));
    RWR_HIP_CHECK(hipStreamSynchronize(ctx->probe_stream));
    RWR_HIP_CHECK(launch_clock_probe(ctx->probe_stream, ctx->d_probe.ptr, micros * 100u));
    return RWR_OK;
}

int rwr_clock_probe_read(rwr_context *ctx, double *shader_mhz)
{
    if (!ctx || !shader_mhz) return set_error(RWR_ERR_INVALID_ARGUMENT, "NULL argument");
    if (!ctx->probe_stream) return set_error(RWR_ERR_NOT_READY, "rwr_clock_probe_start has not been called");
    DeviceGuard g(ctx->device);
    ulonglong2 h{0, 0};
    RWR_HIP_CHECK(hipMemcpyAsync(&h, ctx->d_probe.ptr, sizeof h, hipMemcpyDeviceToHost, ctx->probe_stream));
    RWR_HIP_CHECK(hipStreamSynchronize(ctx->probe_stream));
    *shader_mhz = h.y ? (double)h.x / (double)h.y * 100.0 : 0.0;
    return RWR_OK;
}

}
```

rust-wgpu-raytracing_amd/csrc/kernels_primary_p2.hip:

```cpp
#include <hip/hip_ext.h>

#include "rwr_frame_setup.h"
#include "rwr_p2_tile.h"
#include "rwr_primary.h"
#include "rwr_shade_p2.h"

namespace rwr {

#ifndef RWR_P2_OCC
#define RWR_P2_OCC 7
#endif
template <bool AUX, bool CULL, bool NMAP, bool FUSED = false, bool PLANE = false, bool COVER = false>
__global__ void __launch_bounds__(256, (AUX || NMAP) ? 4 : RWR_P2_OCC)
k_primary_p2(const FrameTri *__restrict__ ftris, const float4 *__restrict__ ray_colp, const float4 *__restrict__ ray_row,
             uint32_t n_tris, uint32_t row_begin, uint32_t bins_enabled, uint32_t row_pitch,
             int32_t mesh_x0, int32_t mesh_y0, int32_t mesh_x1, int32_t mesh_y1,
             const FrameParams p, const TriRecord *__restrict__ tris, const ShadeRec *__restrict__ shade,
             const QuadTex tex, const Targets tg, const FusedSetup fs)
{
    static_assert(!PLANE || (CULL && !NMAP && !FUSED), "the loading form exists for the culled two-launch frame without normal maps");
    static_assert(!COVER || (CULL && !NMAP && !FUSED), "cover words lie beside the face sets of the culled two-launch frame; normal maps take the general path");
    const uint32_t wave = threadIdx.x >> 6, lane = threadIdx.x & 63u;
    uint32_t by = blockIdx.y;
    const_ptr<TriRecord> tris_c = nullptr;
    const_ptr<ShadeRec> shade_c = nullptr;
    const_ptr<float> tnum_c = nullptr;
    if (FUSED) {
        if (blockIdx.y < fs.extra_rows) {
            const uint32_t f = blockIdx.y * gridDim.x + blockIdx.x;
            if (f < fs.n_blocks) {
                frame_setup_block(f, fs.n_blocks, fs.cc, p.cam, p.width, p.height, fs.cull, tris, n_tris, fs.nb_tris, fs.out);
                __threadfence();
                __syncthreads();
                if (threadIdx.x == 0u) atomicAdd(fs.flag, 1u);
            }
            return;
        }
        by -= fs.extra_rows;
        __shared__ uint32_t s_ready;
        if (wave == 0u) {
            uint32_t spins = 0;
            bool ok = true;
            while (__hip_atomic_load(fs.flag, __ATOMIC_RELAXED, __HIP_MEMORY_SCOPE_AGENT) - fs.flag_base < fs.n_blocks) {
                __builtin_amdgcn_s_sleep(16);
                if (++spins > (1u << 15)) { ok = false; break; }
            }
            if (lane == 0u) {
                s_ready = ok ? 1u : 0u;
                if (!ok) atomicOr(fs.flag + 1, 1u);
            }
        }
        __syncthreads();
        if (s_ready == 0u) return;
        asm volatile("" : "+s"(ftris), "+s"(ray_colp), "+s"(ray_row));
        const float *tn = p.tnum;
        asm volatile("" : "+s"(tn));
        tnum_c = to_const_space(tn);
        tris_c = to_const_space(tris);
        shade_c = to_const_space(shade);
    }
    const uint32_t blk_x0 = blockIdx.x * 64u;
#if RWR_P2_TILE_32x4
    const uint32_t tile_x0 = blk_x0 + (wave & 1u) * 32u;
    const uint32_t tile_y0 = row_begin + by * row_pitch + (wave >> 1) * 4u;
    const uint32_t px0 = tile_x0 + 2u * (lane & 15u), py = tile_y0 + (lane >> 4);
    constexpr float kTileWf = 32.0f, kTileHf = 4.0f;
#else
    const uint32_t tile_x0 = blk_x0 + wave * 16u;
    const uint32_t tile_y0 = p.row_begin + by * row_pitch;
    const uint32_t px0 = tile_x0 + 2u * (lane & 7u), py = tile_y0 + (lane >> 3);
    constexpr float kTileWf = 16.0f, kTileHf = 8.0f;
#endif

    const uint32_t wu = __builtin_amdgcn_readfirstlane(wave);
    uint32_t n_list = n_tris;
    const uint32_t *__restrict__ src = nullptr;
    bool live = true;
    if (CULL) {
        if (bins_enabled) {
            const uint32_t bin = ((by * row_pitch) / kBinH) * p.bins.bins_x + blk_x0 / kBinW;
            const uint32_t off = p.bins.offsets[bin];
            if (off != kBinNoList) {
                n_list = p.bins.counts[bin];
                src = p.bins.lists + off;
            }
        }
        const int32_t bx0 = (int32_t)blk_x0, by0 = (int32_t)(row_begin + by * row_pitch);
#if RWR_P2_TILE_32x4
        const int32_t sx0 = bx0 + (int32_t)(wu & 1u) * 32, sy0 = by0 + (int32_t)(wu >> 1) * 4;
        const int32_t sx1 = sx0 + 32, sy1 = sy0 + 4;
#else
        const int32_t sx0 = bx0 + (int32_t)wu * 16, sy0 = by0;
        const int32_t sx1 = sx0 + 16, sy1 = sy0 + 8;
#endif
        if (sx1 < mesh_x0 || sx0 > mesh_x1 || sy1 < mesh_y0 || sy0 > mesh_y1) live = false;
        if (bx0 + 64 < mesh_x0 || bx0 > mesh_x1 || by0 + 8 < mesh_y0 || by0 > mesh_y1) n_list = 0u;
    }
    n_list = __builtin_amdgcn_readfirstlane(n_list);
    const bool lists = CULL && !FUSED && p.tile_lists != nullptr;
    uint32_t set[kTileListWords] = {};
    if (lists) {
        const const_ptr<uint32_t> rec = to_const_space(p.tile_lists) + ((by * gridDim.x + blockIdx.x) * 4u + wu) * kTileListWords;
#pragma unroll
        for (uint32_t k = 0; k < kTileListWords; k++) set[k] = rec[k];
        n_list = 0u;
    }
    const bool classed = lists && (p.flags & RWR_FLAG_TILE_CLASS) != 0u;
    uint32_t cls = 0u;
    if (classed) cls = to_const_space(p.tile_lists)[gridDim.x * gridDim.y * 4u * kTileListWords + (by * gridDim.x + blockIdx.x) * 4u + wu];
    __shared__ float4 s_rec[CULL ? 4 : 1][CULL ? 256 : 1];
    __shared__ uint32_t s_face[CULL ? 256 : 1];
    __shared__ float s_lut[256];
    const uint32_t slot = 64u * wu + lane;
    auto load_round = [&](uint32_t base) {
        const uint32_t e = base + slot;
        if (e < n_list) {
            const uint32_t f = src ? src[e] : e;
            s_face[slot] = f;
            const char *r = reinterpret_cast<const char *>(ftris + f);
#pragma unroll
            for (int k = 0; k < 4; k++)
                __builtin_amdgcn_global_load_lds((__attribute__((address_space(1))) void *)(r + 16 * k),
                                                 (__attribute__((address_space(3))) void *)&s_rec[k][64u * wu], 16, 0, 0);
        }
    };
    auto rwait = []() { __builtin_amdgcn_s_waitcnt(0xF70); };
    if (CULL && !lists) load_round(0u);
    __builtin_amdgcn_global_load_lds((__attribute__((address_space(1))) void *)(tex.lut + threadIdx.x),
                                     (__attribute__((address_space(3))) void *)&s_lut[64u * wu], 4, 0, 0);

    const f3 O = ld3(p.cam.origin);
    v3 D;
    if constexpr (PLANE) {
        const uint32_t i = (by * gridDim.x + blockIdx.x) * 256u + threadIdx.x;
        const float4 dxy = ray_colp[i];
        const float2 dz = reinterpret_cast<const float2 *>(ray_row)[i];
        D = v3{f2{dxy.x, dxy.y}, f2{dxy.z, dxy.w}, f2{dz.x, dz.y}};
    } else {
        D = pixel_pair_ray_dir_tab(p.cam, ray_colp, ray_row, px0, py);
    }

    struct PairSlot { bool in_frame, both, pair_store; uint32_t o; };
    auto pair_slot = [&](uint32_t px0, uint32_t py) {
        PairSlot ps;
        ps.in_frame = py < p.row_end && px0 < p.width;
        ps.o = py * p.width + px0;
        ps.both = px0 + 1u < p.width;
        ps.pair_store = ps.both && (ps.o & 1u) == 0u;
        return ps;
    };
    auto store_depth = [&](const PairSlot &ps, f2 depth_tex) {
        if (ps.in_frame) {
            if (ps.pair_store) {
                __builtin_nontemporal_store(depth_tex, reinterpret_cast<f2 *>(tg.depth + ps.o));
            } else {
                tg.depth[ps.o] = depth_tex.x;
                if (ps.both) tg.depth[ps.o + 1] = depth_tex.y;
            }
        }
    };
    auto store_colour = [&](const PairSlot &ps, const uint32_t (&rgba)[2], const float4 (&cf)[2], i2 obj, f2 win_t, uint32_t dbg_listed,
                            uint32_t dbg_tested) {
        if (ps.in_frame) {
            const uint32_t o = ps.o;
            if (ps.pair_store) {
                __builtin_nontemporal_store(u2{rgba[0], rgba[1]}, reinterpret_cast<u2 *>(reinterpret_cast<uint32_t *>(tg.color) + o));
            } else {
                reinterpret_cast<uint32_t *>(tg.color)[o] = rgba[0];
                if (ps.both) reinterpret_cast<uint32_t *>(tg.color)[o + 1] = rgba[1];
            }
            if (AUX) {
                const bool dbg = (p.flags & RWR_FLAG_DEBUG_COUNTS) != 0;
                reinterpret_cast<float4 *>(tg.color_f32)[o] = cf[0];
                tg.obj_id[o] = dbg ? (int32_t)dbg_listed : obj.x;
                tg.hit_t[o] = dbg ? (float)dbg_tested : win_t.x;
                if (ps.both) {
                    reinterpret_cast<float4 *>(tg.color_f32)[o + 1] = cf[1];
                    tg.obj_id[o + 1] = dbg ? (int32_t)dbg_listed : obj.y;
                    tg.hit_t[o + 1] = dbg ? (float)dbg_tested : win_t.y;
                }
            }
        }
    };
    auto pack_mesh = [&](i2 obj, f2 cr, f2 cg, f2 cb, uint32_t (&rgba)[2], float4 (&cf)[2]) {
        const f2 sr = cr * 255.0f, sg = cg * 255.0f, sb = cb * 255.0f;
        const uint32_t m0 = pack_rgba8_scaled(sr.x, sg.x, sb.x, 0xff000000u);
        const uint32_t m1 = pack_rgba8_scaled(sr.y, sg.y, sb.y, 0xff000000u);
        rgba[0] = obj.x >= 0 ? m0 : rgba[0];
        rgba[1] = obj.y >= 0 ? m1 : rgba[1];
        if (AUX) {
            if (obj.x >= 0) cf[0] = make_float4(cr.x, cg.x, cb.x, 2.0f);
            if (obj.y >= 0) cf[1] = make_float4(cr.y, cg.y, cb.y, 2.0f);
        }
    };

    constexpr uint32_t kWayNone = 0u, kWayOne = 1u, kWayAll = 2u;
    const uint32_t tile_class = cls & (kTileFacesMask | kTileSphereMask);
    const uint32_t way = !classed ? kWayAll
                         : tile_class == kTileFacesNone ? kWayNone
                         : (tile_class == kTileFacesOne && !NMAP && !(p.n_materials > 1u)) ? kWayOne : kWayAll;
    f2 depth_tex = splat(0.0f), win_t = splat(0.0f);
    i2 obj = i2{-1, -1};
    MeshHit2 best;
    best.have = i2{0, 0};
    best.t = best.u = best.v = best.ndotd = splat(0.0f);
    best.idx = u2{0u, 0u};
    uint32_t dbg_listed = 0, dbg_tested = 0;
    uint32_t n_tested = 0;
    uint32_t last_idx = 0;
    ShadeRec one_shade = {};
    if (way == kWayNone) {
        rwait();
        __syncthreads();
    } else if (way == kWayOne) {
        const uint32_t idx = (cls >> kTileFaceShift) & 0xffu;
        const TriRecord T = tris[idx];
        const float tnum = to_const_space(p.tnum)[idx];
        one_shade = shade[idx];
        constexpr uint32_t kTileNotCovering = 2u;
        auto cover_at = [&](uint32_t w) { return gridDim.x * gridDim.y * 4u * (kTileListWords + 1u) + (by * gridDim.x + blockIdx.x) * 4u + w; };
        uint32_t cov = kTileNotCovering;
        if constexpr (COVER) {
            if ((p.flags & RWR_FLAG_TILE_COVER) != 0u) cov = to_const_space(p.tile_lists)[cover_at(wu)];
        }
        rwait();
        if constexpr (COVER) asm volatile("" ::"s"(T.p0[0]), "s"(T.p0[1]), "s"(T.p0[2]), "s"(T.e0[0]), "s"(T.e0[1]), "s"(T.e0[2]));
        __syncthreads();
        best.idx = u2{idx, idx};
        last_idx = idx;
        n_tested = 1u;
        if (AUX) dbg_listed = dbg_tested = 1u;
        if (COVER && cov == kTileCovered) {
            triangle_covered(T, tnum, O, D, best.t, best.u, best.v, best.ndotd);
            best.have = i2{-1, -1};
            depth_tex = 1.0f - to_non_linear_depth_fast(best.t);
            obj = i2{(int)idx, (int)idx};
            win_t = best.t;
        } else {
            f2 u, v;
            best.have = triangle_hit(T, tnum, O, D, best.t, u, v, best.ndotd);
            best.u = best.have ? u : splat(0.0f);
            best.v = best.have ? v : splat(0.0f);
            const bool fast = !__any(any2(best.have & ~depth_fast_domain(best.t)));
            const f2 depth = fast ? to_non_linear_depth_fast(best.t) : to_non_linear_depth(best.t);
            const i2 win = best.have & ~(depth >= 1.0f);
            depth_tex = win ? (1.0f - depth) : splat(0.0f);
            obj = win ? i2{(int)idx, (int)idx} : i2{-1, -1};
            win_t = win ? best.t : splat(0.0f);
            if (COVER && cov != kTileNotCovering) {
                const bool all = fast && hit_div_num_domain(tnum) && hit_div_lanes_in_domain(abs2(best.ndotd)) &&
                                 __builtin_amdgcn_ballot_w64((win.x & win.y) != 0) == __builtin_amdgcn_read_exec();
                uint32_t w = wu;
                asm volatile("" : "+s"(w));
                if (all && lane == 0u) const_cast<uint32_t *>(p.tile_lists)[cover_at(w)] = kTileCovered;
            }
        }
    } else {

    const float tx0 = (float)tile_x0, ty0 = (float)tile_y0;
    const uint32_t sph = classed ? (cls >> kTileSphereShift) & 0xffu : 0xffu;
    for (uint32_t s = 0; sph != 0u && s < p.n_spheres; s++) {
        if (classed ? ((sph >> s) & 1u) == 0u
                    : (CULL && ((tx0 + kTileWf < p.sphere_rect[s][0]) || (tx0 > p.sphere_rect[s][2]) ||
                                (ty0 + kTileHf < p.sphere_rect[s][1]) || (ty0 > p.sphere_rect[s][3]))))
            continue;
        f2 t = splat(0.0f);
        const i2 hit = sphere_ray_intersect_t(ld3(p.spheres[s].center), p.spheres[s].radius, O, D, t);
        if (any2(hit)) {
            const f2 current_depth = 1.0f - depth_tex;
            const f2 depth = to_non_linear_depth(t);
            const i2 win = hit & ~(depth >= current_depth);
            depth_tex = win ? (1.0f - depth) : depth_tex;
            obj = win ? i2{-2 - (int)s, -2 - (int)s} : obj;
            win_t = win ? t : win_t;
        }
    }

    if constexpr (CULL) {
        const TileRect tile_rect = {tx0, ty0, tx0 + kTileWf, ty0 + kTileHf};
        if (lists) {
            rwait();
            __syncthreads();
#pragma unroll
            for (uint32_t k = 0; k < kTileListWords / 2u; k++) {
                unsigned long long m = live ? ((unsigned long long)set[2u * k + 1u] << 32 | set[2u * k]) : 0ull;
                if (AUX) dbg_listed += (uint32_t)__popcll(m);
                while (m) {
                    const uint32_t idx = 64u * k + (uint32_t)__builtin_ctzll(m);
                    m &= m - 1ull;
                    intersect_and_select(tris[idx], to_const_space(p.tnum)[idx], idx, O, D, best);
                    last_idx = idx;
                    n_tested++;
                    if (AUX) dbg_tested++;
                }
            }
        }
        for (uint32_t base = 0; base < n_list; base += 256u) {
            if (base) {
                __syncthreads();
                load_round(base);
            }
            rwait();
            __syncthreads();
            const uint32_t n_round = min(n_list - base, 256u);
            for (uint32_t b = 0; b < n_round; b += 64u) {
                const uint32_t i = b + lane;
                const float4 q0 = s_rec[0][i], q1 = s_rec[1][i], q2 = s_rec[2][i], q3 = s_rec[3][i];
                const FrameTri rec = {q0.x, q0.y, q0.z, q0.w, {q1.x, q1.y, q1.z}, q1.w,
                                      {q2.x, q2.y, q2.z}, q2.w, {q3.x, q3.y, q3.z}, q3.w};
                const uint32_t my_face = s_face[i];
                unsigned long long m = live ? __builtin_amdgcn_ballot_w64(i < n_round && !rect_culls(rec, tile_rect)) : 0ull;
                if (AUX) dbg_listed += (uint32_t)__popcll(m);
                while (m) {
                    const uint32_t bit = (uint32_t)__builtin_ctzll(m);
                    m &= m - 1ull;
                    const uint32_t idx = (uint32_t)__builtin_amdgcn_readlane((int)my_face, (int)bit);
                    if (FUSED) intersect_and_select(load_tri_record(tris_c + idx), tnum_c[idx], idx, O, D, best);
                    else intersect_and_select(tris[idx], to_const_space(p.tnum)[idx], idx, O, D, best);
                    last_idx = idx;
                    n_tested++;
                    if (AUX) dbg_tested++;
                }
            }
        }
        if (n_list == 0u && !lists) {
            rwait();
            __syncthreads();
        }
    } else {
        rwait();
        __syncthreads();
        for (uint32_t base = 0; base < n_list; base += 64u) {
            unsigned long long m = __ballot(base + lane < n_list);
            if (AUX) dbg_listed += (uint32_t)__popcll(m);
            while (m) {
                const uint32_t idx = base + (uint32_t)__builtin_ctzll(m);
                m &= m - 1ull;
                intersect_and_select(tris[idx], to_const_space(p.tnum)[idx], idx, O, D, best);
                last_idx = idx;
                n_tested++;
                if (AUX) dbg_tested++;
            }
        }
    }
    if (any2(best.have)) {
        const f2 current_depth = 1.0f - depth_tex;
        const bool fast = !__any(any2(best.have & ~depth_fast_domain(best.t)));
        const f2 depth = fast ? to_non_linear_depth_fast(best.t) : to_non_linear_depth(best.t);
        const i2 win = best.have & ~(depth >= current_depth);
        depth_tex = win ? (1.0f - depth) : depth_tex;
        obj = win ? i2{(int)best.idx.x, (int)best.idx.y} : obj;
        win_t = win ? best.t : win_t;
    }
    }

    const PairSlot ps = pair_slot(px0, py);
    store_depth(ps, depth_tex);

    uint32_t rgba[2] = {0u, 0u};
    float4 cf[2];
    if (AUX) cf[0] = cf[1] = make_float4(0.0f, 0.0f, 0.0f, 0.0f);
    if (any2(obj < -1)) {
#pragma unroll
        for (int k = 0; k < 2; k++) {
            const int o = k ? obj.y : obj.x;
            if (o < -1) {
                const f3 Dk = lane3(D, k);
                const f3 center = ld3(p.spheres[-2 - o].center);
                float t = 0.0f;
                (void)sphere_ray_intersect_t(center, p.spheres[-2 - o].radius, O, Dk, t);
                const f3 c = shade_sphere(cnormalize(sub3(along(O, t, Dk), center)), Dk);
                rgba[k] = pack_rgba8(c.x, c.y, c.z, 2.0f);
                if (AUX) cf[k] = make_float4(c.x, c.y, c.z, 2.0f);
            }
        }
    }
    if (__any(any2(obj >= 0))) {
        f2 cr, cg, cb;
        QuadTex qt = tex;
        qt.lut = s_lut;
        const ShadeRec unused = {};
        if (NMAP) shade_mesh_pair<true, false, true, FrameParams, QuadTex>(p, shade, qt, obj, unused, best, D, cr, cg, cb);
        else if (p.n_materials > 1u) shade_mesh_pair<true, false, false, FrameParams, QuadTex>(p, shade, qt, obj, unused, best, D, cr, cg, cb);
        else if (n_tested == 1u) {
            const ShadeRec last_shade = way == kWayOne ? one_shade : FUSED ? load_shade_record(shade_c + last_idx) : shade[last_idx];
            shade_mesh_pair<false, true, false, FrameParams, QuadTex>(p, shade, qt, obj, last_shade, best, D, cr, cg, cb);
        } else shade_mesh_pair<false, false, false, FrameParams, QuadTex>(p, shade, qt, obj, unused, best, D, cr, cg, cb);
        pack_mesh(obj, cr, cg, cb, rgba, cf);
    }
    store_colour(ps, rgba, cf, obj, win_t, dbg_listed, dbg_tested);
}

uint32_t primary_p2_fused_rows(const FrameParams &fp, uint32_t n_blocks)
{
    const uint32_t gx = (fp.width + 63u) / 64u;
    return gx ? (n_blocks + gx - 1u) / gx : 0u;
}

hipError_t launch_primary_p2(hipStream_t s, const FrameParams &fp, const TriRecord *tris, const ShadeRec *shade,
                             const FrameTri *ftris, const QuadTex &tex, const Targets &tg, hipEvent_t ev_start,
                             hipEvent_t ev_stop, const FusedSetup *fused, const RayPlane *plane)
{
    if (fp.row_end <= fp.row_begin || fp.width == 0) return hipSuccess;
    if (fp.row_pitch % kStripRows != 0u) return hipErrorInvalidValue;
    if (!tex.lut) return hipErrorInvalidValue;
    const dim3 grid((fp.width + 63u) / 64u, band_strips(fp) + (fused ? fused->extra_rows : 0u));
    const dim3 block(256);
    const bool aux = (fp.flags & RWR_FLAG_AUX_OUTPUTS) != 0;
    const bool do_cull = (fp.flags & RWR_FLAG_NO_CULL) == 0;
    const bool nmap = (fp.flags & RWR_FLAG_NORMAL_MAP) != 0 && fp.tangents != nullptr;
    const FusedSetup fs = fused ? *fused : FusedSetup{};
#define RWR_P2_LAUNCH(A, C, N, F) hipExtLaunchKernelGGL((k_primary_p2<A, C, N, F>), grid, block, 0, s, ev_start, ev_stop, 0, ftris, fp.ray_colp, fp.ray_row, \
    fp.n_tris, fp.row_begin, fp.bins.enabled, fp.row_pitch, fp.mesh_px[0], fp.mesh_px[1], fp.mesh_px[2], fp.mesh_px[3], fp, tris, shade, tex, tg, fs)
    if (plane) {
        if (fused || nmap || !do_cull || !plane->xy || !plane->z) return hipErrorInvalidValue;
        const bool cover = (fp.flags & RWR_FLAG_TILE_COVER) != 0u;
        const float4 *const pxy = plane->xy, *const pz = reinterpret_cast<const float4 *>(plane->z);
#define RWR_P2_LAUNCH_PLANE(A, V) hipExtLaunchKernelGGL((k_primary_p2<A, true, false, false, true, V>), grid, block, 0, s, ev_start, ev_stop, 0, ftris, pxy, pz, \
    fp.n_tris, fp.row_begin, fp.bins.enabled, fp.row_pitch, fp.mesh_px[0], fp.mesh_px[1], fp.mesh_px[2], fp.mesh_px[3], fp, tris, shade, tex, tg, fs)
        if (aux && cover) RWR_P2_LAUNCH_PLANE(true, true);
        else if (aux) RWR_P2_LAUNCH_PLANE(true, false);
        else if (cover) RWR_P2_LAUNCH_PLANE(false, true);
        else RWR_P2_LAUNCH_PLANE(false, false);
#undef RWR_P2_LAUNCH_PLANE
    } else if (fused) {
        RWR_P2_LAUNCH(false, true, false, true);
    } else if (nmap) {
        if (aux && do_cull) RWR_P2_LAUNCH(true, true, true, false);
        else if (aux) RWR_P2_LAUNCH(true, false, true, false);
        else if (do_cull) RWR_P2_LAUNCH(false, true, true, false);
        else RWR_P2_LAUNCH(false, false, true, false);
    } else if ((fp.flags & RWR_FLAG_TILE_COVER) != 0u) {
        if (!do_cull) return hipErrorInvalidValue;
#define RWR_P2_LAUNCH_COVER(A) hipExtLaunchKernelGGL((k_primary_p2<A, true, false, false, false, true>), grid, block, 0, s, ev_start, ev_stop, 0, ftris, fp.ray_colp, fp.ray_row, \
    fp.n_tris, fp.row_begin, fp.bins.enabled, fp.row_pitch, fp.mesh_px[0], fp.mesh_px[1], fp.mesh_px[2], fp.mesh_px[3], fp, tris, shade, tex, tg, fs)
        if (aux) RWR_P2_LAUNCH_COVER(true);
        else RWR_P2_LAUNCH_COVER(false);
#undef RWR_P2_LAUNCH_COVER
    } else {
        if (aux && do_cull) RWR_P2_LAUNCH(true, true, false, false);
        else if (aux) RWR_P2_LAUNCH(true, false, false, false);
        else if (do_cull) RWR_P2_LAUNCH(false, true, false, false);
        else RWR_P2_LAUNCH(false, false, false, false);
    }
#undef RWR_P2_LAUNCH
    return hipGetLastError();
}

hipError_t preload_kernels_primary_p2()
{
    hipFuncAttributes attr;
    return hipFuncGetAttributes(&attr, reinterpret_cast<const void *>((&k_primary_p2<false, true, false>)));
}

}
```

rust-wgpu-raytracing_amd/csrc/render_reference.cpp:

```cpp
#include <algorithm>
#include <cstring>

#include "rwr_frame.h"

namespace rwr {

namespace {

int launch_frame_graph(rwr_context *ctx, FrameSlot &sl, const FrameConsts &fc, const FrameSetupOut &so, const QuadTex &quad_tex, const Targets &tg)
{
    const FrameParams &fp = fc.fp;
    const hipStream_t stream = sl.stream;
    sl.records_key.clear();
    std::vector<unsigned char> key(sizeof(FrameParams) + sizeof(CullConsts));
    std::memcpy(key.data(), &fp, sizeof fp);
    std::memcpy(key.data() + sizeof fp, &fc.cc, sizeof fc.cc);
    if (!sl.frame_graph || key != sl.frame_graph_key) {
        hipGraph_t g = nullptr;
        RWR_HIP_CHECK(hipStreamBeginCapture(stream, hipStreamCaptureModeThreadLocal));
        hipError_t e = launch_records(ctx, sl, fc, so, true);
        if (e == hipSuccess) e = launch_primary_p2(stream, fp, ctx->d_tris.ptr, ctx->d_shade.ptr, sl.d_ftris.ptr, quad_tex, tg);
        const hipError_t e2 = hipStreamEndCapture(stream, &g);
        RWR_HIP_CHECK(e);
        RWR_HIP_CHECK(e2);
        bool updated = false;
        if (sl.frame_graph) {
            hipGraphNode_t bad = nullptr;
            hipGraphExecUpdateResult res;
            updated = hipGraphExecUpdate(sl.frame_graph, g, &bad, &res) == hipSuccess;
            if (!updated) { (void)hipGetLastError(); sl.frame_graph = OwnedGraphExec{}; }
        }
        if (!updated) {
            const hipError_t e3 = hipGraphInstantiate(&sl.frame_graph.h, g, nullptr, nullptr, 0);
            if (e3 != hipSuccess) { (void)hipGraphDestroy(g); RWR_HIP_CHECK(e3); }
        }
        (void)hipGraphDestroy(g);
        sl.frame_graph_key.swap(key);
    }
    RWR_HIP_CHECK(hipGraphLaunch(sl.frame_graph, stream));
    ctx->setup_launches++;
    return RWR_OK;
}

bool fused_pays(const rwr_context *ctx, const FrameParams &fp)
{
    const uint32_t render_groups = ((fp.width + 63u) / 64u) * ((fp.row_end - fp.row_begin + fp.row_pitch - 1u) / std::max(1u, fp.row_pitch));
    return ctx->fused_setup_force || (ctx->n_slots > 1u && render_groups <= 1200u);
}

int launch_fused_frame(rwr_context *ctx, FrameSlot &sl, const FrameConsts &fc, const FrameSetupOut &so, const QuadTex &quad_tex, const Targets &tg)
{
    const hipStream_t stream = sl.stream;
    sl.records_key.clear();
    FusedSetup fs{};
    fs.cc = fc.cc;
    fs.cull = ctx->d_cull.ptr;
    fs.out = so;
    fs.nb_tris = (ctx->n_tris + 255u) / 256u;
    fs.n_blocks = fs.nb_tris + (so.ray_pairs + so.ray_rows + 255u) / 256u;
    fs.extra_rows = primary_p2_fused_rows(fc.fp, fs.n_blocks);
    if (!sl.d_fused.ptr || sl.fused_blocks != fs.n_blocks) {
        RWR_HIP_CHECK(hipStreamSynchronize(stream));
        RWR_HIP_CHECK(sl.d_fused.ensure(2));
        RWR_HIP_CHECK(hipMemsetAsync(sl.d_fused.ptr, 0, 2 * sizeof(uint32_t), stream));
        sl.fused_count = 0;
        sl.fused_blocks = fs.n_blocks;
    }
    fs.flag = sl.d_fused.ptr;
    fs.flag_base = sl.fused_count;
    sl.fused_count += fs.n_blocks;
    sl.fused_used = true;
    RWR_HIP_CHECK(launch_primary_p2(stream, fc.fp, ctx->d_tris.ptr, ctx->d_shade.ptr, sl.d_ftris.ptr, quad_tex, tg, nullptr, nullptr, &fs));
    return RWR_OK;
}

}

int enqueue_reference(rwr_context *ctx, FrameSlot &sl, const FrameRequest &rq, FrameKernel kernel, FrameConsts &fc, const Targets &tg,
                      FrameTiming &timing)
{
    FrameParams &fp = fc.fp;
    const hipStream_t stream = sl.stream;
    FrameSetupOut so{};
    int rc = frame_tables(ctx, sl, fp, so);
    if (rc != RWR_OK) return rc;
    const bool small_culled = small_culled_frame(ctx, rq, kernel), band = fp.row_end > fp.row_begin;
    if (small_culled && ctx->tile_lists && ctx->n_tris <= kTileListMaxFaces && band) {
        so.list_gx = (fp.width + 63u) / 64u;
        so.list_gy = band_strips(fp);
        so.list_row_begin = fp.row_begin;
        so.list_row_pitch = fp.row_pitch;
        const uint32_t regions = ((so.list_gx + kListRegionWgs - 1u) / kListRegionWgs) * ((so.list_gy + kListRegionWgs - 1u) / kListRegionWgs);
        so.list_blocks = (regions + 4u * kListRegionsPerWave - 1u) / (4u * kListRegionsPerWave);
        RWR_HIP_CHECK(sl.d_tile_lists.ensure(tile_list_words(so.list_gx, so.list_gy)));
        so.tile_lists = sl.d_tile_lists.ptr;
        fp.tile_lists = so.tile_lists;
    }
    fp.flags &= ~(RWR_FLAG_TILE_CLASS | RWR_FLAG_TILE_COVER);
    if (so.tile_lists && ctx->tile_class) fp.flags |= RWR_FLAG_TILE_CLASS;
    ctx->last_classes = rwr_context::LastClasses{so.tile_lists ? ctx->cur : 0u, so.list_gx, so.tile_lists ? so.list_gy : 0u};
    ctx->last_cover_frames = 0;
    const QuadTex quad_tex{ctx->d_quads.empty() ? nullptr : ctx->d_quads[0].ptr, ctx->d_mat_quads.ptr, ctx->d_srgb_lut.ptr};
    const bool plain = small_culled && !rq.aux && !ctx->timing_every;
    if (plain && ctx->frame_graph) return launch_frame_graph(ctx, sl, fc, so, quad_tex, tg);
    if (plain && ctx->fused_setup && fused_pays(ctx, fp) && !(fp.flags & RWR_FLAG_NORMAL_MAP) && band) {
        ctx->last_classes = rwr_context::LastClasses{};
        return launch_fused_frame(ctx, sl, fc, so, quad_tex, tg);
    }
    bool kept = false;
    if ((rc = enqueue_records(ctx, sl, kernel, fc, so, timing, &kept)) != RWR_OK) return rc;
    switch (kernel) {
    case FrameKernel::kDormant: {
        SingleTriangles st{};
        st.n = ctx->n_triangles;
        for (uint32_t i = 0; i < ctx->n_triangles; i++) st.t[i] = ctx->triangles[i];
        RWR_HIP_CHECK(launch_primary_dormant(stream, fp, st, ctx->d_tris.ptr, ctx->d_shade.ptr, tex0_of(ctx), tg));
        break;
    }
    case FrameKernel::kBvh: {
        const BvhDevice bvh_p{ctx->d_bvh_nodes.ptr, ctx->d_bvh_leaf_faces.ptr, ctx->bvh_n_nodes, 3u * ctx->bvh_depth + 2u, 0.0f, 0u, 0u, 0u, 0u};
        RWR_HIP_CHECK(launch_primary_bvh(stream, fp, ctx->d_tris.ptr, ctx->d_shade.ptr, bvh_p, tex0_of(ctx), tg));
        break;
    }
    case FrameKernel::kOnePixel:
        RWR_HIP_CHECK(launch_primary(stream, fp, ctx->d_tris.ptr, ctx->d_shade.ptr, sl.d_ftris.ptr, tex0_of(ctx), tg));
        break;
    default: {
        RayPlane plane{};
        const bool can_load = !(fp.flags & RWR_FLAG_NO_CULL) && !((fp.flags & RWR_FLAG_NORMAL_MAP) && fp.tangents);
        const bool load = can_load && ray_plane_step(ctx, sl, fp, plane);
        if (kept && (fp.flags & RWR_FLAG_TILE_CLASS) && ctx->tile_cover && can_load && fp.n_materials <= 1u) {
            fp.flags |= RWR_FLAG_TILE_COVER;
            ctx->tile_cover_frames++;
            ctx->last_cover_frames = ++sl.cover_frames;
        }
        RWR_HIP_CHECK(launch_primary_p2(stream, fp, ctx->d_tris.ptr, ctx->d_shade.ptr, sl.d_ftris.ptr, quad_tex, tg,
                                        timing.dispatch ? ctx->timing_events[2 * ctx->timing_pairs].h : nullptr,
                                        timing.dispatch ? ctx->timing_events[2 * ctx->timing_pairs + 1].h : nullptr, nullptr,
                                        load ? &plane : nullptr));
    }
    }
    return RWR_OK;
}

int check_fused_frame(rwr_context *ctx, uint32_t i)
{
    FrameSlot &sl = ctx->slots[i];
    if (!sl.fused_used || !sl.d_fused.ptr) return RWR_OK;
    uint32_t timed_out = 0;
    RWR_HIP_CHECK(hipMemcpy(&timed_out, sl.d_fused.ptr + 1, sizeof timed_out, hipMemcpyDeviceToHost));
    if (timed_out) {
        sl.fused_blocks = 0;
        return set_error(RWR_ERR_HIP, "a frame is incomplete: workgroups of the fused frame kernel waited in vain for the frame's records "
                         "(RWR_FUSED_SETUP=0 renders with two launches per frame)");
    }
    return RWR_OK;
}

}
```

rust-wgpu-raytracing_amd/csrc/rwr_context.h:

```cpp
#pragma once

#include <hip/hip_runtime.h>

#include <utility>
#include <vector>

#include "rwr_internal.h"

typedef struct ncclComm *ncclComm_t;

namespace rwr {

#define RWR_HIP_CHECK(expr)                                                                          \
    do {                                                                                             \
        hipError_t _e = (expr);                                                                      \
        if (_e != hipSuccess)                                                                        \
            return set_error(RWR_ERR_HIP, "%s failed: %s (%s:%d)", #expr, hipGetErrorString(_e), __FILE__, __LINE__); \
    } while (0)

template <typename T>
struct DeviceBuffer {
    T *ptr = nullptr;
    size_t count = 0;
    DeviceBuffer() = default;
    DeviceBuffer(const DeviceBuffer &) = delete;
    DeviceBuffer(DeviceBuffer &&o) noexcept : ptr(o.ptr), count(o.count) { o.ptr = nullptr; o.count = 0; }
    DeviceBuffer &operator=(DeviceBuffer &&o) noexcept { std::swap(ptr, o.ptr); std::swap(count, o.count); return *this; }
    ~DeviceBuffer() { release(); }
    hipError_t ensure(size_t n)
    {
        if (n <= count && ptr) return hipSuccess;
        release();
        if (n == 0) return hipSuccess;
        hipError_t e = hipMalloc(reinterpret_cast<void **>(&ptr), n * sizeof(T));
        if (e == hipSuccess) count = n;
        else ptr = nullptr;
        return e;
    }
    void release()
    {
        if (ptr) (void)hipFree(ptr);
        ptr = nullptr;
        count = 0;
    }
};

template <typename T, hipError_t (*Destroy)(T)>
struct Owned {
    T h = nullptr;
    Owned() = default;
    Owned(Owned &&o) noexcept : h(o.h) { o.h = nullptr; }
    Owned &operator=(Owned &&o) noexcept { std::swap(h, o.h); return *this; }
    ~Owned() { if (h) (void)Destroy(h); }
    operator T() const { return h; }
};
inline hipError_t free_pinned_words(uint32_t *p) { return hipHostFree(p); }
using OwnedStream = Owned<hipStream_t, hipStreamDestroy>;
using OwnedEvent = Owned<hipEvent_t, hipEventDestroy>;
using OwnedGraphExec = Owned<hipGraphExec_t, hipGraphExecDestroy>;
using PinnedWords = Owned<uint32_t *, free_pinned_words>;
struct MirrorRec { float r, g, b, on; };
static_assert(sizeof(MirrorRec) == sizeof(float4), "MirrorRec is a float4");
inline hipError_t free_pinned_mirror(MirrorRec *p) { return hipHostFree(p); }
using PinnedMirror = Owned<MirrorRec *, free_pinned_mirror>;

enum class SurfaceModel { kDiffuse, kMirror, kGlass, kGloss };
inline SurfaceModel surface_model(const MirrorRec &m)
{
    return m.on > 1.0f ? SurfaceModel::kGloss : m.on > 0.0f ? SurfaceModel::kMirror : m.on < 0.0f ? SurfaceModel::kGlass : SurfaceModel::kDiffuse;
}
constexpr float kGlassIorMin = 1.0f, kGlassIorMax = 4.0f, kGlossRoughnessMin = 0x1p-10f, kGlossRoughnessMax = 1.0f;
constexpr MirrorRec kDiffuseRec{0.0f, 0.0f, 0.0f, 0.0f};
inline MirrorRec mirror_rec(const float rgb[3]) { return MirrorRec{rgb[0], rgb[1], rgb[2], 1.0f}; }
inline MirrorRec glass_rec(const float rgb[3], float ior) { return MirrorRec{rgb[0], rgb[1], rgb[2], -ior}; }
inline MirrorRec gloss_rec(const float rgb[3], float roughness) { return MirrorRec{rgb[0], rgb[1], rgb[2], 1.0f + roughness}; }
inline float surface_param(const MirrorRec &m) { return m.on < 0.0f ? -m.on : m.on > 1.0f ? m.on - 1.0f : 0.0f; }
constexpr uint32_t surface_mode(SurfaceModel s)
{
    return s == SurfaceModel::kMirror ? 1u : s == SurfaceModel::kGlass ? 2u : s == SurfaceModel::kGloss ? 4u : 0u;
}

struct FrameSlot {
    hipStream_t stream = nullptr;
    OwnedStream owned;
    OwnedEvent done;
    DeviceBuffer<uint8_t> d_color;
    DeviceBuffer<float> d_depth;
    DeviceBuffer<float> d_color_f32;
    DeviceBuffer<int32_t> d_obj_id;
    DeviceBuffer<float> d_hit_t;
    DeviceBuffer<FrameTri> d_ftris;
    DeviceBuffer<float> d_tnum;
    DeviceBuffer<float4> d_ray_colp, d_ray_row;
    DeviceBuffer<uint32_t> d_tile_lists;
    DeviceBuffer<uint32_t> d_bin_lists, d_bin_counts, d_bin_offsets, d_bin_total;
    PinnedWords h_bin_total;
    bool aux_valid = false;
    DeviceBuffer<float4> d_dn_guide, d_dn_a, d_dn_b;
    OwnedGraphExec frame_graph;
    std::vector<unsigned char> frame_graph_key;
    std::vector<unsigned char> records_key;
    uint32_t cover_frames = 0;
    DeviceBuffer<float2> d_ray_plane;
    std::vector<unsigned char> ray_plane_key;
    bool ray_plane_built = false;
    void forget_ray_plane() { ray_plane_key.clear(); ray_plane_built = false; }
    DeviceBuffer<uint32_t> d_fused;
    uint32_t fused_count = 0, fused_blocks = 0;
    bool fused_used = false;
    void reset()
    {
        FrameSlot fresh;
        fresh.stream = stream;
        fresh.owned = std::move(owned);
        fresh.done = std::move(done);
        *this = std::move(fresh);
    }
};
constexpr uint32_t kMaxFramesInFlight = 3;
constexpr rwr_denoise_params kDenoiseDefaults{5u, 0.04f, 0.95f, 0.05f};
constexpr rwr_reproject_params kReprojectDefaults{32u, 0.95f, 0.05f};
constexpr rwr_sky_params kSkyDefaults = RWR_SKY_DEFAULTS;
constexpr uint32_t kWfMaxQueues = 4;

struct WfState {
    OwnedStream streams[kWfMaxQueues];
    OwnedEvent fork, join[kWfMaxQueues];
    DeviceBuffer<float4> d_rays;
    bool fix_clean = false;
    DeviceBuffer<unsigned long long> d_masks;
    DeviceBuffer<unsigned long long> d_masks_next;
    DeviceBuffer<uint16_t> d_sorted, d_bins;
    DeviceBuffer<uint32_t> d_wave_total;
    DeviceBuffer<unsigned long long> d_fix;
    DeviceBuffer<uint8_t> d_pool_info;
    DeviceBuffer<uint32_t> d_live;
    DeviceBuffer<uint32_t> d_pool_list;
    DeviceBuffer<ShadowRec> d_shadow_recs;
    DeviceBuffer<unsigned long long> d_shadow_masks, d_shadow_counts;
    DeviceBuffer<uint32_t> d_tiles;
    DeviceBuffer<float4> d_mirror;
    PinnedMirror h_mirror;
    size_t h_mirror_count = 0;
    OwnedEvent mirror_copied;
    uint64_t mirror_version = 0;
    uint32_t mirror_modes = 0;
    DeviceBuffer<unsigned long long> d_glass_counts;
};

struct Accum {
    DeviceBuffer<unsigned long long> d_hist;
    DeviceBuffer<float> d_depth;
    DeviceBuffer<int32_t> d_obj_id;
    DeviceBuffer<float> d_hit_t;
    std::vector<unsigned char> key;
    uint64_t samples = 0;
    OwnedEvent done;
    bool done_recorded = false;
    void reset()
    {
        Accum fresh;
        fresh.done = std::move(done);
        fresh.done_recorded = done_recorded;
        *this = std::move(fresh);
    }
};

struct Reproject {
    DeviceBuffer<float4> d_colour[2], d_guide[2];
    DeviceBuffer<int32_t> d_id[2];
    DeviceBuffer<unsigned long long> d_counts;
    std::vector<unsigned char> key;
    uint64_t frames = 0;
    RpCamera camera{};
    OwnedEvent done;
    bool done_recorded = false;
    void reset()
    {
        Reproject fresh;
        fresh.done = std::move(done);
        fresh.done_recorded = done_recorded;
        *this = std::move(fresh);
    }
};

struct GatherSet {
    DeviceBuffer<uint8_t> d_gathered;
    DeviceBuffer<uint8_t> d_pack, d_recv;
    OwnedEvent done;
    bool valid = false;
};

}

struct rwr_context {
    int device = 0;
    rwr::OwnedStream own_stream;
    hipStream_t stream = nullptr;
    rwr::OwnedEvent ev_begin, ev_end;
    rwr::FrameSlot slots[rwr::kMaxFramesInFlight];
    uint32_t n_slots = 1;
    uint32_t cur = 0;

    rwr::DeviceBuffer<rwr_model_vertex_small> d_verts;
    rwr::DeviceBuffer<rwr_model_face_small> d_faces;
    rwr::DeviceBuffer<rwr_instance_raw> d_instances;
    rwr::DeviceBuffer<rwr::TriRecord> d_tris;
    rwr::DeviceBuffer<rwr::ShadeRec> d_shade;
    rwr::DeviceBuffer<rwr::CullRec> d_cull;
    rwr::DeviceBuffer<rwr::TangentRec> d_tangent;
    std::vector<rwr::DeviceBuffer<float4>> d_nmaps;
    uint32_t bin_min_faces = 256;
    uint32_t bin_min_capacity = 65536;
    bool force_one_pixel = false;
    bool frame_graph = false;
    bool fused_setup = true;
    bool fused_setup_force = false;
    bool tile_lists = true;
    bool setup_cache = true;
    uint64_t setup_launches = 0;
    bool ray_plane = true;
    uint64_t ray_plane_builds = 0, ray_plane_frames = 0;
    bool tile_class = true;
    struct LastClasses { uint32_t slot = 0, gx = 0, gy = 0; };
    LastClasses last_classes;
    bool tile_cover = true;
    uint64_t tile_cover_frames = 0;
    uint32_t last_cover_frames = 0;
    rwr::DeviceBuffer<rwr::BvhNode4> d_bvh_nodes;
    rwr::DeviceBuffer<uint32_t> d_bvh_leaf_faces;
    uint32_t bvh_n_nodes = 0, bvh_depth = 0;
    float bvh_leaf_extent = 0.0f;
    float wf_packet_extent = 0.5f;
    uint32_t wf_min_packet_pools = 64;
    uint32_t wf_lane_items = 0;
    int32_t wf_wide_lane = -1;
    uint32_t wf_packet_dense_rays = 16384;
    float aabb_lo[3] = {0, 0, 0}, aabb_hi[3] = {0, 0, 0};
    float auto_bvh_face_px = 150.0f;
    rwr::PinnedWords h_wf_live;
    uint32_t wf_z_split = 0;
    rwr::DeviceBuffer<unsigned long long> d_wf_dbg;
    uint64_t wf_launches_before[3] = {0, 0, 0};
    uint32_t wf_group = 0;
    float wf_packet_fill = 0.25f;
    uint32_t last_segments = 0;
    uint32_t last_wf_state = 0;
    uint32_t wf_queues = 2;
    rwr::WfState wf_state[rwr::kMaxFramesInFlight];
    uint32_t last_spp = 0;
    bool last_had_bounce = false;
    rwr::Accum accum;
    uint64_t accum_max = 1u << 24;
    uint64_t last_accum_samples = 0;
    rwr::Reproject reproj;
    rwr_reproject_params reproject = rwr::kReprojectDefaults;
    uint64_t last_reproject_frames = 0;
    uint32_t last_reproject_set = 0;
    rwr_denoise_params denoise = rwr::kDenoiseDefaults;
    rwr_sky_params sky = rwr::kSkyDefaults;
    uint64_t scene_generation = 0;
    std::vector<rwr::DeviceBuffer<float4>> d_texs;
    std::vector<rwr::DeviceBuffer<uint4>> d_quads;
    rwr::DeviceBuffer<const uint4 *> d_mat_quads;
    rwr::DeviceBuffer<float> d_srgb_lut;
    rwr::DeviceBuffer<uint32_t> d_face_mat;
    rwr::DeviceBuffer<rwr::MaterialRec> d_materials;
    std::vector<rwr_model_vertex_small> st_verts;
    std::vector<rwr_model_face_small> st_faces;
    std::vector<uint32_t> st_face_mat;
    std::vector<rwr::MaterialRec> st_materials;
    uint32_t n_verts = 0, n_faces = 0, n_instances = 0, n_tris = 0;
    uint32_t tex_w = 0, tex_h = 0;
    rwr_material_data material{};
    bool have_mesh = false;
    bool tris_dirty = false;
    rwr_sphere_buffer_data spheres[RWR_MAX_SPHERES]{};
    uint32_t n_spheres = 0;
    std::vector<rwr::MirrorRec> part_mirrors;
    rwr::MirrorRec sphere_mirrors[RWR_MAX_SPHERES]{};
    uint64_t mirror_version = 1;
    rwr_triangle_buffer_data triangles[RWR_MAX_TRIANGLES]{};
    uint32_t n_triangles = 0;

    rwr_screen screen{0, 0};

    uint64_t last_primary = 0, last_bounce = 0;
    bool last_shadows = false;
    bool last_gloss = false;
    bool last_glass = false;
    uint32_t timing_every = 0;
    uint64_t timing_calls = 0;
    std::vector<rwr::OwnedEvent> timing_events;
    uint32_t timing_pairs = 0;
    uint32_t wave_cull_min = 4;
    ncclComm_t comm = nullptr;
    int dist_rank = 0, dist_world = 0;
    rwr::GatherSet gather[rwr::kMaxFramesInFlight];
    uint32_t last_gather = 0;
    rwr::OwnedEvent exchange_done;
    rwr::OwnedStream probe_stream;
    rwr::DeviceBuffer<ulonglong2> d_probe;
};

namespace rwr {

struct DeviceGuard {
    int prev = -1;
    bool ok = true;
    explicit DeviceGuard(int dev)
    {
        if (hipGetDevice(&prev) != hipSuccess) prev = -1;
        if (prev != dev) ok = (hipSetDevice(dev) == hipSuccess);
    }
    ~DeviceGuard()
    {
        if (prev >= 0) (void)hipSetDevice(prev);
    }
};

inline hipError_t sync_all(rwr_context *ctx)
{
    hipError_t first = hipSuccess;
    for (uint32_t i = 0; i < kMaxFramesInFlight; i++) {
        if (!ctx->slots[i].stream) continue;
        const hipError_t e = hipStreamSynchronize(ctx->slots[i].stream);
        if (first == hipSuccess) first = e;
    }
    return first;
}

inline uint64_t instanced_faces(uint64_t n_faces, uint32_t n_instances) { return n_faces * (n_instances ? n_instances : 1u); }

inline uint32_t surface_modes(const rwr_context *ctx)
{
    uint32_t modes = 0;
    for (const MirrorRec &m : ctx->part_mirrors) modes |= surface_mode(surface_model(m));
    for (uint32_t i = 0; i < ctx->n_spheres; i++) modes |= surface_mode(surface_model(ctx->sphere_mirrors[i]));
    return modes;
}

hipError_t ensure_frame_buffers(rwr_context *ctx);
int rebuild_tris(rwr_context *ctx);
int check_fused_frame(rwr_context *ctx, uint32_t i);

}
```

rust-wgpu-raytracing_amd/csrc/rwr_internal.h:

```cpp
#pragma once

#include <hip/hip_runtime.h>
#include <stdint.h>

#include "../../include/rwr_hip.h"

namespace rwr {

constexpr uint32_t RWR_FLAG_DEBUG_COUNTS = 1u << 16;
constexpr uint32_t RWR_FLAG_ONE_PIXEL_PER_LANE = 1u << 17;
constexpr uint32_t RWR_FLAG_TILE_CLASS = 1u << 18;
constexpr uint32_t RWR_FLAG_TILE_COVER = 1u << 19;

struct alignas(16) TriRecord {
    float p0[3]; float d;
    float p1[3]; float denom;
    float p2[3]; float pad0;
    float N[3];  float pad1;
    float e0[3]; float pad2;
    float e1[3]; float pad3;
    float e2[3]; float pad4;
    float nhat[3]; float pad5;
};
static_assert(sizeof(TriRecord) == 128, "TriRecord is 128 B");

struct alignas(16) ShadeRec {
    float n[3];  float ndl0;
    float c0[2], c1[2];
    float c2[2]; uint32_t material;
    float pad;
};
static_assert(sizeof(ShadeRec) == 48, "ShadeRec is 48 B");

constexpr uint32_t kMaxTextureDim = 16384;

struct alignas(16) MaterialRec {
    float ambient[3];  uint32_t tex_w;
    float specular[3]; uint32_t tex_h;
    const float4 *tex;
    float wmax, hmax;
    const float4 *nmap;
    uint32_t nmap_w, nmap_h;
};
static_assert(sizeof(MaterialRec) == 64, "MaterialRec is 64 B");

struct QuadTex {
    const uint4 *quad0;
    const uint4 *const *mats;
    const float *lut;
};
void build_tex_quads(const uint8_t *rgba8, uint32_t w, uint32_t h, uint32_t *out);
void build_srgb_lut(float *lut);

struct alignas(16) TangentRec {
    float t[3]; float pad0;
    float b[3]; float pad1;
};
static_assert(sizeof(TangentRec) == 32, "TangentRec is 32 B");

struct alignas(16) CullRec {
    float p0[3], p1[3], p2[3];
    float pad[3];
};
static_assert(sizeof(CullRec) == 48, "CullRec is 48 B");

struct Targets {
    uint8_t *color;
    float *depth;
    float *color_f32;
    int32_t *obj_id;
    float *hit_t;
};

constexpr double kCullRelHost = 2e-5;
constexpr double kCullWorldHost = 12.0 * 5.9604645e-8;
constexpr float kCullRel = (float)kCullRelHost;
constexpr float kCullWorld = (float)kCullWorldHost;

struct CullConsts {
    float A[4], Bx[4], By[4];
    float Ux[4], Vx[4];
    float Uy[4], Vy[4];
    float origin[4];
    float vxa, vya;
    float corner_margin;
    uint32_t enabled;
};

struct alignas(16) FrameTri {
    float bx0, by0, bx1, by1;
    float ea[3]; float me0;
    float ex[3]; float me1;
    float ey[3]; float me2;
};
static_assert(sizeof(FrameTri) == 64, "FrameTri is 64 B");

constexpr uint32_t kBinW = 64, kBinH = 32;
struct BinGrid {
    const uint32_t *lists;
    const uint32_t *counts;
    const uint32_t *offsets;
    uint32_t bins_x, bins_y, capacity, enabled;
};
constexpr uint32_t kBinNoList = 0xffffffffu;
constexpr uint32_t kStripRows = 8;
constexpr uint32_t kTileListMaxFaces = 256, kTileListWords = kTileListMaxFaces / 32;
constexpr uint32_t kListRegionWgs = 4, kListRegionsPerWave = 1;
constexpr uint32_t kTileFacesNone = 0u, kTileFacesOne = 1u, kTileFacesMore = 2u, kTileFacesMask = 3u;
constexpr uint32_t kTileFaceShift = 8u, kTileSphereShift = 16u, kTileSphereMask = 0xffu << kTileSphereShift;
static_assert(RWR_MAX_SPHERES <= 8 && kTileListMaxFaces <= 256, "a class word has 8 bits for the spheres and 8 for a face index");
constexpr uint32_t kTileCovered = 1u;
inline size_t tile_list_words(uint32_t gx, uint32_t gy) { return (size_t)gx * gy * 4u * (kTileListWords + 2u); }

struct FrameParams {
    rwr_camera_inv_uniform cam;
    BinGrid bins;
    uint32_t width, height;
    uint32_t row_begin, row_end;
    uint32_t row_pitch;
    uint32_t n_spheres;
    uint32_t n_tris;
    uint32_t tex_w, tex_h;
    float tex_wmax, tex_hmax;
    uint32_t flags;
    uint32_t wave_cull_min;
    uint32_t spp, jitter_spp, seed, bounces;
    rwr_sphere_buffer_data spheres[RWR_MAX_SPHERES];
    float sphere_rect[RWR_MAX_SPHERES][4];
    float mesh_rect[4];
    int32_t mesh_px[4];
    float ambient[4];
    float specular[4];
    const float4 *ray_colp;
    const float4 *ray_row;
    const float *tnum;
    const MaterialRec *materials;
    uint32_t n_materials;
    uint32_t pad_m;
    const TangentRec *tangents;
    const uint32_t *tile_lists;
};
inline uint32_t band_strips(const FrameParams &fp) { return fp.row_end > fp.row_begin ? (fp.row_end - fp.row_begin + fp.row_pitch - 1u) / fp.row_pitch : 0u; }

struct FrameScene {
    uint32_t width, height;
    const rwr_sphere_buffer_data *spheres;
    uint32_t n_spheres;
    uint32_t n_tris, tex_w, tex_h;
    const float *aabb_lo, *aabb_hi;
    const rwr_material_data *material;
    const MaterialRec *materials;
    uint32_t n_materials;
    const TangentRec *tangents;
    uint32_t wave_cull_min;
};
struct FrameConsts {
    FrameParams fp;
    CullConsts cc;
    double mean_face_px;
};
void fill_frame_consts(const FrameScene &scene, const rwr_camera_inv_uniform &cam, const rwr_render_params &rp, bool accumulate,
                       uint32_t row_begin, uint32_t row_end, uint32_t row_pitch, FrameConsts &out);

int set_error(int code, const char *fmt, ...) __attribute__((format(printf, 2, 3)));

hipError_t launch_prebake(hipStream_t s, const rwr_model_vertex_small *verts, const rwr_model_face_small *faces,
                          const uint32_t *face_material, uint32_t n_faces, const rwr_instance_raw *instances,
                          uint32_t n_instances, const MaterialRec *materials, TriRecord *tris, ShadeRec *shade, CullRec *cull,
                          TangentRec *tangents);
constexpr uint32_t kWfTileW = 64, kWfTileH = 8, kWfTilePixels = kWfTileW * kWfTileH;
#ifndef RWR_WF_MAX_GROUP
#define RWR_WF_MAX_GROUP 64
#endif
constexpr uint32_t kWfMaxGroup = RWR_WF_MAX_GROUP;
constexpr float kWfFixedScale = 67108864.0f;
constexpr uint32_t kWfE0Cap = 16;
#ifndef RWR_WF_CELL_BITS
#define RWR_WF_CELL_BITS 4
#endif
constexpr uint32_t kWfDirCellBits = RWR_WF_CELL_BITS;
constexpr uint32_t kWfDirBins = 8u << (2u * kWfDirCellBits);
struct WfBuffers {
    unsigned long long *fix;
    float4 *rays;
    unsigned long long *masks;
    uint16_t *bins;
    uint16_t *sorted;
    uint32_t *wave_total;
    uint32_t group;
    uint32_t tiles_x;
    unsigned long long *dbg;
    uint32_t *counters;
    uint32_t shared_planes;
    const uint32_t *live_list;
    const uint32_t *live_count;
    const uint32_t *tile_live;
};
struct WfEmit {
    unsigned long long *masks_out;
    uint32_t next_dim;
    uint32_t sample_base;
};
struct alignas(16) ShadowRec {
    float o[3]; uint32_t flags;
    uint32_t d[3]; uint32_t pad;
};
static_assert(sizeof(ShadowRec) == 32, "ShadowRec is 32 B");
struct WfShadow {
    ShadowRec *recs;
    unsigned long long *masks;
    unsigned long long *counts;
};
struct WfSky {
    float zr, zg, zb, hr, hg, hb;
};
static_assert(sizeof(WfSky) == sizeof(rwr_sky_params), "WfSky is rwr_sky_params");
struct WfMirror {
    const float4 *table;
    uint32_t n_parts;
    uint32_t pad;
    unsigned long long *glass_counts;
};
constexpr int kSurfNone = 0, kSurfMirrors = 1, kSurfGlass = 2, kSurfGloss = 3;
struct WfFeatures {
    WfEmit emit{nullptr, 0u, 0u};
    WfShadow shadow{nullptr, nullptr, nullptr};
    WfSky sky{0.0f, 0.0f, 0.0f, 0.0f, 0.0f, 0.0f};
    WfMirror mirror{nullptr, 0u, 0u, nullptr};
    bool emits = false, shadows = false, sky_on = false;
    int surf = kSurfNone;
    int primary_surf(const FrameParams &fp) const { return fp.bounces != 0u ? surf : kSurfNone; }
    int trace_surf() const { return emits ? surf : kSurfNone; }
};
struct BvhNode4;
struct BvhDevice {
    const BvhNode4 *nodes;
    const uint32_t *leaf_faces;
    uint32_t n_nodes;
    uint32_t stack_depth;
    float packet_extent;
    uint32_t min_packet_pools;
    uint32_t lane_items;
    uint32_t packet_dense_rays;
    uint32_t wide_lane;
};

struct RayPlane {
    float4 *xy;
    float2 *z;
};
constexpr uint32_t kRayPlaneMaxW = 3840, kRayPlaneMaxH = 2160;
inline size_t ray_plane_entries(const FrameParams &fp) { return (size_t)((fp.width + 63u) / 64u) * band_strips(fp) * 256u; }
hipError_t launch_ray_plane(hipStream_t s, const FrameParams &fp, const RayPlane &plane);
hipError_t preload_kernels_ray_plane();

struct FusedSetup;
hipError_t launch_primary_p2(hipStream_t s, const FrameParams &fp, const TriRecord *tris, const ShadeRec *shade,
                             const FrameTri *ftris, const QuadTex &tex, const Targets &tg, hipEvent_t ev_start = nullptr,
                             hipEvent_t ev_stop = nullptr, const FusedSetup *fused = nullptr, const RayPlane *plane = nullptr);
uint32_t primary_p2_fused_rows(const FrameParams &fp, uint32_t n_blocks);
hipError_t launch_wf_primary(hipStream_t s, const FrameParams &fp, const TriRecord *tris, const ShadeRec *shade,
                             const FrameTri *ftris, const float4 *tex, const Targets &tg,
                             const WfBuffers &wf, uint32_t sample_begin, uint32_t sample_count, uint32_t z_split, const WfFeatures &ft);
hipError_t launch_wf_classify(hipStream_t s, const FrameParams &fp, const FrameTri *ftris, const Targets &tg, uint32_t tiles_x,
                              uint32_t *live_list, uint32_t *live_count, uint32_t *tile_live);
hipError_t launch_wf_bounce(hipStream_t s, const FrameParams &fp, const TriRecord *tris, const ShadeRec *shade,
                            const BvhDevice &bvh, const float4 *tex, const WfBuffers &wf,
                            uint32_t n_tiles, uint32_t sample_count, uint32_t packet_min_rays, void *pool_info, uint32_t *pool_list,
                            const WfFeatures &ft);
hipError_t launch_wf_shadow(hipStream_t s, const FrameParams &fp, const TriRecord *tris, const BvhDevice &bvh, const WfBuffers &wf,
                            const WfShadow &shadow, uint32_t n_tiles, uint32_t expected_tiles, uint32_t sample_count, const float light_mesh[3],
                            const float light_sphere[3]);
size_t wf_pool_info_bytes();
void wf_trace_launch_counts(uint64_t out[3]);
hipError_t launch_primary_bvh(hipStream_t s, const FrameParams &fp, const TriRecord *tris, const ShadeRec *shade,
                              const BvhDevice &bvh, const float4 *tex, const Targets &tg);
hipError_t launch_wf_resolve(hipStream_t s, const FrameParams &fp, const Targets &tg, const WfBuffers &wf, const uint32_t *live_counters = nullptr,
                             uint32_t *host_live = nullptr);
struct AccumBuffers {
    unsigned long long *hist;
    float *depth;
    int32_t *obj_id;
    float *hit_t;
};
enum class AccumMode { kFirst, kAdd, kShow };
hipError_t launch_wf_resolve_accum(hipStream_t s, const FrameParams &fp, const Targets &tg, const WfBuffers &wf, const AccumBuffers &ac,
                                   AccumMode mode, uint32_t total_samples, const uint32_t *live_counters = nullptr,
                                   uint32_t *host_live = nullptr);

hipError_t launch_wf_denoise(hipStream_t s, uint32_t width, uint32_t height, const TriRecord *tris, const Targets &tg,
                             const rwr_denoise_params &dp, float4 *guide, float4 *plane_a, float4 *plane_b);

struct RpCamera {
    float o[3], c0[3], cx[3], cy[3], nrm[3];
    float nc0, nn;
};
struct RpHistory {
    float4 *colour;
    float4 *guide;
    int32_t *id;
};
hipError_t launch_wf_reproject(hipStream_t s, uint32_t width, uint32_t height, const TriRecord *tris, const Targets &tg,
                               const rwr_camera_inv_uniform &cam, const RpCamera *prev, const rwr_reproject_params &rp,
                               const RpHistory &from, const RpHistory &to, unsigned long long *counts);

struct FrameSetupOut {
    FrameTri *ftris;
    float *tnum;
    float4 *ray_colp;
    float4 *ray_row;
    uint32_t ray_pairs, ray_rows;
    uint32_t *zero_a, *zero_b;
    uint32_t n_zero_a, n_zero_b;
    uint32_t *tile_lists;
    uint32_t list_gx, list_gy, list_row_begin, list_row_pitch, list_blocks;
};
struct TileClassIn {
    uint32_t *classes;
    uint32_t *cover;
    int32_t mesh_px[4];
    uint32_t n_spheres, pad;
    float sphere_rect[RWR_MAX_SPHERES][4];
};
static_assert(sizeof(TileClassIn) == 8 + 8 + 16 + 8 + RWR_MAX_SPHERES * 16, "TileClassIn has no padding");
struct FusedSetup {
    CullConsts cc;
    const CullRec *cull;
    FrameSetupOut out;
    uint32_t n_blocks;
    uint32_t nb_tris;
    uint32_t extra_rows;
    uint32_t flag_base;
    uint32_t *flag;
};

struct SingleTriangles {
    uint32_t n;
    uint32_t pad[3];
    rwr_triangle_buffer_data t[RWR_MAX_TRIANGLES];
};
hipError_t launch_primary_dormant(hipStream_t s, const FrameParams &fp, const SingleTriangles &st, const TriRecord *tris,
                                  const ShadeRec *shade, const float4 *tex, const Targets &tg);

hipError_t preload_kernels();
hipError_t preload_kernels_primary();
hipError_t preload_kernels_primary_p2();
hipError_t preload_kernels_wavefront();
hipError_t preload_kernels_wf_primary();
hipError_t preload_kernels_wf_bounce();
hipError_t preload_kernels_wf_shadow();
hipError_t preload_kernels_dist();

struct StripLayout;
hipError_t launch_strips_pack(hipStream_t s, const StripLayout &L, uint32_t rank, uint32_t row_bytes, const uint8_t *frame, uint8_t *message);
hipError_t launch_strips_deal(hipStream_t s, const StripLayout &L, uint32_t row_bytes, const uint8_t *recv, uint8_t *frame);
void strips_pack_host(const StripLayout &L, uint32_t rank, size_t row_bytes, const uint8_t *frame, uint8_t *message);
void strips_deal_host(const StripLayout &L, size_t row_bytes, const uint8_t *recv, uint8_t *frame);

hipError_t launch_selftest_exact_math(hipStream_t s, unsigned long long *d_out4, uint32_t normalize_count, uint32_t seed);
hipError_t launch_selftest_exact_div(hipStream_t s, unsigned long long *d_out4, uint32_t count, uint32_t seed);

hipError_t launch_clock_probe(hipStream_t s, ulonglong2 *d_out, uint32_t ticks_100mhz);
hipError_t launch_measure_valu(hipStream_t s, int mode, ulonglong2 *d_out, uint32_t n_workgroups, uint32_t iters);

hipError_t launch_frame_setup(hipStream_t s, const CullConsts &cc, const rwr_camera_inv_uniform &cam, uint32_t width,
                              uint32_t height, const CullRec *cull, const TriRecord *tris, uint32_t n_tris,
                              const FrameSetupOut &out, const TileClassIn &tc);
hipError_t launch_bin_faces(hipStream_t s, const FrameTri *ftris, uint32_t n_tris, uint32_t row_begin, uint32_t *lists,
                            uint32_t *counts, uint32_t *offsets, uint32_t *total_out, uint32_t bins_x, uint32_t bins_y, uint32_t capacity,
                            const int32_t mesh_px[4], uint32_t *total_host);
hipError_t launch_primary(hipStream_t s, const FrameParams &fp, const TriRecord *tris, const ShadeRec *shade,
                          const FrameTri *ftris, const float4 *tex, const Targets &tg);

}
```

Before: 218,100 Mray/s.

## Add lean rest-of-frame primary kernel variant sharing a common body header

Moves the primary P2 kernel body into a shared header parameterised by a LISTS constexpr, so a lean specialisation can be built that reads tile lists directly and skips block-wide barriers and the multi-material path. The variant is gated by the RWR_LEAN_REST environment flag and counted via a new stats entry point. The aim is to cut per-block synchronisation and setup for tiles that already have precomputed face sets. Replacing __syncthreads with a compiler fence in the lists path assumes no cross-wave LDS dependency beyond the LUT.

```diff
diff --git a/include/rwr_hip.h b/include/rwr_hip.h
--- a/include/rwr_hip.h
+++ b/include/rwr_hip.h
@@ -222,6 +222,8 @@
 RWR_API int rwr_debug_tile_cover(rwr_context *ctx, uint32_t *cover, size_t capacity, uint32_t *grid_x, uint32_t *grid_y);
 
 RWR_API int rwr_tile_cover_stats(rwr_context *ctx, uint64_t *frames, uint64_t *tiles_last);
+
+RWR_API int rwr_lean_rest_stats(rwr_context *ctx, uint64_t *frames);
 
 RWR_API int rwr_last_shadow_stats(rwr_context *ctx, uint64_t *shadow_rays, uint64_t *occluded);
 
diff --git a/rust-wgpu-raytracing_amd/__init__.py b/rust-wgpu-raytracing_amd/__init__.py
--- a/rust-wgpu-raytracing_amd/__init__.py
+++ b/rust-wgpu-raytracing_amd/__init__.py
@@ -103,7 +103,7 @@
         "rwr_timer_begin": [vp], "rwr_timer_end": [vp, vp], "rwr_timer_stop": [vp], "rwr_timer_elapsed": [vp, vp], "rwr_last_render_stats": [vp, vp, vp],
         "rwr_last_shadow_stats": [vp, vp, vp], "rwr_frame_setup_launches": [vp, vp], "rwr_ray_plane_stats": [vp, vp, vp],
         "rwr_debug_tile_classes": [vp, vp, C.c_size_t, vp, vp],
-        "rwr_debug_tile_cover": [vp, vp, C.c_size_t, vp, vp], "rwr_tile_cover_stats": [vp, vp, vp],
+        "rwr_debug_tile_cover": [vp, vp, C.c_size_t, vp, vp], "rwr_tile_cover_stats": [vp, vp, vp], "rwr_lean_rest_stats": [vp, vp],
         "rwr_accum_reset": [vp], "rwr_accum_samples": [vp, vp],
         "rwr_denoise_set_params": [vp, vp], "rwr_denoise_get_params": [vp, vp],
         "rwr_sky_set_params": [vp, vp], "rwr_sky_get_params": [vp, vp],
@@ -133,7 +133,7 @@
         "rwr_dist_loopback_deposit": [vp, u32, u32, i32], "rwr_dist_loopback_finish": [vp, u32, i32],
         "rwr_measure_valu_clock": [vp, u32, vp], "rwr_clock_probe_start": [vp, u32], "rwr_clock_probe_read": [vp, vp],
     }
-    _NEWER_ENTRY_POINTS = ("rwr_last_shadow_stats", "rwr_denoise_set_params", "rwr_denoise_get_params", "rwr_frame_setup_launches", "rwr_ray_plane_stats", "rwr_debug_tile_classes", "rwr_debug_tile_cover", "rwr_tile_cover_stats",
+    _NEWER_ENTRY_POINTS = ("rwr_last_shadow_stats", "rwr_denoise_set_params", "rwr_denoise_get_params", "rwr_frame_setup_launches", "rwr_ray_plane_stats", "rwr_debug_tile_classes", "rwr_debug_tile_cover", "rwr_tile_cover_stats", "rwr_lean_rest_stats",
                            "rwr_sky_set_params", "rwr_sky_get_params", "rwr_scene_set_part_mirror", "rwr_scene_set_sphere_mirror",
                            "rwr_scene_get_part_mirror", "rwr_scene_get_sphere_mirror", "rwr_scene_set_part_glass", "rwr_scene_set_sphere_glass",
                            "rwr_scene_get_part_glass", "rwr_scene_get_sphere_glass", "rwr_last_glass_stats",
@@ -690,6 +690,11 @@
         _check(lib().rwr_tile_cover_stats(self._h, C.byref(a), C.byref(b)))
         return a.value, b.value
 
+    def lean_rest_stats(self) -> int:
+        a = C.c_uint64()
+        _check(lib().rwr_lean_rest_stats(self._h, C.byref(a)))
+        return a.value
+
     def last_shadow_stats(self) -> tuple[int, int]:
         a, b = C.c_uint64(), C.c_uint64()
         _check(lib().rwr_last_shadow_stats(self._h, C.byref(a), C.byref(b)))
diff --git a/rust-wgpu-raytracing_amd/csrc/context.cpp b/rust-wgpu-raytracing_amd/csrc/context.cpp
--- a/rust-wgpu-raytracing_amd/csrc/context.cpp
+++ b/rust-wgpu-raytracing_amd/csrc/context.cpp
@@ -79,6 +79,7 @@
     env_flag("RWR_RAY_PLANE", &ctx->ray_plane);
     env_flag("RWR_TILE_CLASS", &ctx->tile_class);
     env_flag("RWR_TILE_COVER", &ctx->tile_cover);
+    env_flag("RWR_LEAN_REST", &ctx->lean_rest);
     env_f32("RWR_AUTO_BVH_FACE_PX", &ctx->auto_bvh_face_px);
     if (env_u32("RWR_WF_GROUP", &ctx->wf_group)) ctx->wf_group = std::min(kWfMaxGroup, std::max(1u, ctx->wf_group));
     bool stats = false, wide = false;
diff --git a/rust-wgpu-raytracing_amd/csrc/diagnostics.cpp b/rust-wgpu-raytracing_amd/csrc/diagnostics.cpp
--- a/rust-wgpu-raytracing_amd/csrc/diagnostics.cpp
+++ b/rust-wgpu-raytracing_amd/csrc/diagnostics.cpp
@@ -87,6 +87,13 @@
     return RWR_OK;
 }
 
+int rwr_lean_rest_stats(rwr_context *ctx, uint64_t *frames)
+{
+    if (!ctx || !frames) return set_error(RWR_ERR_INVALID_ARGUMENT, "NULL argument");
+    *frames = ctx->lean_rest_frames;
+    return RWR_OK;
+}
+
 int rwr_measure_valu_clock(rwr_context *ctx, uint32_t waves_per_simd, double out4[4])
 {
     if (!ctx || !out4) return set_error(RWR_ERR_INVALID_ARGUMENT, "NULL argument");
diff --git a/rust-wgpu-raytracing_amd/csrc/kernels_primary_p2.hip b/rust-wgpu-raytracing_amd/csrc/kernels_primary_p2.hip
--- a/rust-wgpu-raytracing_amd/csrc/kernels_primary_p2.hip
+++ b/rust-wgpu-raytracing_amd/csrc/kernels_primary_p2.hip
@@ -18,377 +18,25 @@
              const FrameParams p, const TriRecord *__restrict__ tris, const ShadeRec *__restrict__ shade,
              const QuadTex tex, const Targets tg, const FusedSetup fs)
 {
-    static_assert(!PLANE || (CULL && !NMAP && !FUSED), "the loading form exists for the culled two-launch frame without normal maps");
-    static_assert(!COVER || (CULL && !NMAP && !FUSED), "cover words lie beside the face sets of the culled two-launch frame; normal maps take the general path");
-    const uint32_t wave = threadIdx.x >> 6, lane = threadIdx.x & 63u;
-    uint32_t by = blockIdx.y;
-    const_ptr<TriRecord> tris_c = nullptr;
-    const_ptr<ShadeRec> shade_c = nullptr;
-    const_ptr<float> tnum_c = nullptr;
-    if (FUSED) {
-        if (blockIdx.y < fs.extra_rows) {
-            const uint32_t f = blockIdx.y * gridDim.x + blockIdx.x;
-            if (f < fs.n_blocks) {
-                frame_setup_block(f, fs.n_blocks, fs.cc, p.cam, p.width, p.height, fs.cull, tris, n_tris, fs.nb_tris, fs.out);
-                __threadfence();
-                __syncthreads();
-                if (threadIdx.x == 0u) atomicAdd(fs.flag, 1u);
-            }
-            return;
-        }
-        by -= fs.extra_rows;
-        __shared__ uint32_t s_ready;
-        if (wave == 0u) {
-            uint32_t spins = 0;
-            bool ok = true;
-            while (__hip_atomic_load(fs.flag, __ATOMIC_RELAXED, __HIP_MEMORY_SCOPE_AGENT) - fs.flag_base < fs.n_blocks) {
-                __builtin_amdgcn_s_sleep(16);
-                if (++spins > (1u << 15)) { ok = false; break; }
-            }
-            if (lane == 0u) {
-                s_ready = ok ? 1u : 0u;
-                if (!ok) atomicOr(fs.flag + 1, 1u);
-            }
-        }
-        __syncthreads();
-        if (s_ready == 0u) return;
-        asm volatile("" : "+s"(ftris), "+s"(ray_colp), "+s"(ray_row));
-        const float *tn = p.tnum;
-        asm volatile("" : "+s"(tn));
-        tnum_c = to_const_space(tn);
-        tris_c = to_const_space(tris);
-        shade_c = to_const_space(shade);
-    }
-    const uint32_t blk_x0 = blockIdx.x * 64u;
-#if RWR_P2_TILE_32x4
-    const uint32_t tile_x0 = blk_x0 + (wave & 1u) * 32u;
-    const uint32_t tile_y0 = row_begin + by * row_pitch + (wave >> 1) * 4u;
-    const uint32_t px0 = tile_x0 + 2u * (lane & 15u), py = tile_y0 + (lane >> 4);
-    constexpr float kTileWf = 32.0f, kTileHf = 4.0f;
-#else
-    const uint32_t tile_x0 = blk_x0 + wave * 16u;
-    const uint32_t tile_y0 = p.row_begin + by * row_pitch;
-    const uint32_t px0 = tile_x0 + 2u * (lane & 7u), py = tile_y0 + (lane >> 3);
-    constexpr float kTileWf = 16.0f, kTileHf = 8.0f;
-#endif
+    constexpr bool LISTS = false;
+    const auto tl = [&]() { return p.tile_lists; };
+    const float *const lut_src = tex.lut;
+#include "rwr_primary_p2_body.h"
+}
 
-    const uint32_t wu = __builtin_amdgcn_readfirstlane(wave);
-    uint32_t n_list = n_tris;
-    const uint32_t *__restrict__ src = nullptr;
-    bool live = true;
-    if (CULL) {
-        if (bins_enabled) {
-            const uint32_t bin = ((by * row_pitch) / kBinH) * p.bins.bins_x + blk_x0 / kBinW;
-            const uint32_t off = p.bins.offsets[bin];
-            if (off != kBinNoList) {
-                n_list = p.bins.counts[bin];
-                src = p.bins.lists + off;
-            }
-        }
-        const int32_t bx0 = (int32_t)blk_x0, by0 = (int32_t)(row_begin + by * row_pitch);
-#if RWR_P2_TILE_32x4
-        const int32_t sx0 = bx0 + (int32_t)(wu & 1u) * 32, sy0 = by0 + (int32_t)(wu >> 1) * 4;
-        const int32_t sx1 = sx0 + 32, sy1 = sy0 + 4;
-#else
-        const int32_t sx0 = bx0 + (int32_t)wu * 16, sy0 = by0;
-        const int32_t sx1 = sx0 + 16, sy1 = sy0 + 8;
-#endif
-        if (sx1 < mesh_x0 || sx0 > mesh_x1 || sy1 < mesh_y0 || sy0 > mesh_y1) live = false;
-        if (bx0 + 64 < mesh_x0 || bx0 > mesh_x1 || by0 + 8 < mesh_y0 || by0 > mesh_y1) n_list = 0u;
-    }
-    n_list = __builtin_amdgcn_readfirstlane(n_list);
-    const bool lists = CULL && !FUSED && p.tile_lists != nullptr;
-    uint32_t set[kTileListWords] = {};
-    if (lists) {
-        const const_ptr<uint32_t> rec = to_const_space(p.tile_lists) + ((by * gridDim.x + blockIdx.x) * 4u + wu) * kTileListWords;
-#pragma unroll
-        for (uint32_t k = 0; k < kTileListWords; k++) set[k] = rec[k];
-        n_list = 0u;
-    }
-    const bool classed = lists && (p.flags & RWR_FLAG_TILE_CLASS) != 0u;
-    uint32_t cls = 0u;
-    if (classed) cls = to_const_space(p.tile_lists)[gridDim.x * gridDim.y * 4u * kTileListWords + (by * gridDim.x + blockIdx.x) * 4u + wu];
-    __shared__ float4 s_rec[CULL ? 4 : 1][CULL ? 256 : 1];
-    __shared__ uint32_t s_face[CULL ? 256 : 1];
-    __shared__ float s_lut[256];
-    const uint32_t slot = 64u * wu + lane;
-    auto load_round = [&](uint32_t base) {
-        const uint32_t e = base + slot;
-        if (e < n_list) {
-            const uint32_t f = src ? src[e] : e;
-            s_face[slot] = f;
-            const char *r = reinterpret_cast<const char *>(ftris + f);
-#pragma unroll
-            for (int k = 0; k < 4; k++)
-                __builtin_amdgcn_global_load_lds((__attribute__((address_space(1))) void *)(r + 16 * k),
-                                                 (__attribute__((address_space(3))) void *)&s_rec[k][64u * wu], 16, 0, 0);
-        }
-    };
-    auto rwait = []() { __builtin_amdgcn_s_waitcnt(0xF70); };
-    if (CULL && !lists) load_round(0u);
-    __builtin_amdgcn_global_load_lds((__attribute__((address_space(1))) void *)(tex.lut + threadIdx.x),
-                                     (__attribute__((address_space(3))) void *)&s_lut[64u * wu], 4, 0, 0);
-
-    const f3 O = ld3(p.cam.origin);
-    v3 D;
-    if constexpr (PLANE) {
-        const uint32_t i = (by * gridDim.x + blockIdx.x) * 256u + threadIdx.x;
-        const float4 dxy = ray_colp[i];
-        const float2 dz = reinterpret_cast<const float2 *>(ray_row)[i];
-        D = v3{f2{dxy.x, dxy.y}, f2{dxy.z, dxy.w}, f2{dz.x, dz.y}};
-    } else {
-        D = pixel_pair_ray_dir_tab(p.cam, ray_colp, ray_row, px0, py);
-    }
-
-    struct PairSlot { bool in_frame, both, pair_store; uint32_t o; };
-    auto pair_slot = [&](uint32_t px0, uint32_t py) {
-        PairSlot ps;
-        ps.in_frame = py < p.row_end && px0 < p.width;
-        ps.o = py * p.width + px0;
-        ps.both = px0 + 1u < p.width;
-        ps.pair_store = ps.both && (ps.o & 1u) == 0u;
-        return ps;
-    };
-    auto store_depth = [&](const PairSlot &ps, f2 depth_tex) {
-        if (ps.in_frame) {
-            if (ps.pair_store) {
-                __builtin_nontemporal_store(depth_tex, reinterpret_cast<f2 *>(tg.depth + ps.o));
-            } else {
-                tg.depth[ps.o] = depth_tex.x;
-                if (ps.both) tg.depth[ps.o + 1] = depth_tex.y;
-            }
-        }
-    };
-    auto store_colour = [&](const PairSlot &ps, const uint32_t (&rgba)[2], const float4 (&cf)[2], i2 obj, f2 win_t, uint32_t dbg_listed,
-                            uint32_t dbg_tested) {
-        if (ps.in_frame) {
-            const uint32_t o = ps.o;
-            if (ps.pair_store) {
-                __builtin_nontemporal_store(u2{rgba[0], rgba[1]}, reinterpret_cast<u2 *>(reinterpret_cast<uint32_t *>(tg.color) + o));
-            } else {
-                reinterpret_cast<uint32_t *>(tg.color)[o] = rgba[0];
-                if (ps.both) reinterpret_cast<uint32_t *>(tg.color)[o + 1] = rgba[1];
-            }
-            if (AUX) {
-                const bool dbg = (p.flags & RWR_FLAG_DEBUG_COUNTS) != 0;
-                reinterpret_cast<float4 *>(tg.color_f32)[o] = cf[0];
-                tg.obj_id[o] = dbg ? (int32_t)dbg_listed : obj.x;
-                tg.hit_t[o] = dbg ? (float)dbg_tested : win_t.x;
-                if (ps.both) {
-                    reinterpret_cast<float4 *>(tg.color_f32)[o + 1] = cf[1];
-                    tg.obj_id[o + 1] = dbg ? (int32_t)dbg_listed : obj.y;
-                    tg.hit_t[o + 1] = dbg ? (float)dbg_tested : win_t.y;
-                }
-            }
-        }
-    };
-    auto pack_mesh = [&](i2 obj, f2 cr, f2 cg, f2 cb, uint32_t (&rgba)[2], float4 (&cf)[2]) {
-        const f2 sr = cr * 255.0f, sg = cg * 255.0f, sb = cb * 255.0f;
-        const uint32_t m0 = pack_rgba8_scaled(sr.x, sg.x, sb.x, 0xff000000u);
-        const uint32_t m1 = pack_rgba8_scaled(sr.y, sg.y, sb.y, 0xff000000u);
-        rgba[0] = obj.x >= 0 ? m0 : rgba[0];
-        rgba[1] = obj.y >= 0 ? m1 : rgba[1];
-        if (AUX) {
-            if (obj.x >= 0) cf[0] = make_float4(cr.x, cg.x, cb.x, 2.0f);
-            if (obj.y >= 0) cf[1] = make_float4(cr.y, cg.y, cb.y, 2.0f);
-        }
-    };
-
-    constexpr uint32_t kWayNone = 0u, kWayOne = 1u, kWayAll = 2u;
-    const uint32_t tile_class = cls & (kTileFacesMask | kTileSphereMask);
-    const uint32_t way = !classed ? kWayAll
-                         : tile_class == kTileFacesNone ? kWayNone
-                         : (tile_class == kTileFacesOne && !NMAP && !(p.n_materials > 1u)) ? kWayOne : kWayAll;
-    f2 depth_tex = splat(0.0f), win_t = splat(0.0f);
-    i2 obj = i2{-1, -1};
-    MeshHit2 best;
-    best.have = i2{0, 0};
-    best.t = best.u = best.v = best.ndotd = splat(0.0f);
-    best.idx = u2{0u, 0u};
-    uint32_t dbg_listed = 0, dbg_tested = 0;
-    uint32_t n_tested = 0;
-    uint32_t last_idx = 0;
-    ShadeRec one_shade = {};
-    if (way == kWayNone) {
-        rwait();
-        __syncthreads();
-    } else if (way == kWayOne) {
-        const uint32_t idx = (cls >> kTileFaceShift) & 0xffu;
-        const TriRecord T = tris[idx];
-        const float tnum = to_const_space(p.tnum)[idx];
-        one_shade = shade[idx];
-        constexpr uint32_t kTileNotCovering = 2u;
-        auto cover_at = [&](uint32_t w) { return gridDim.x * gridDim.y * 4u * (kTileListWords + 1u) + (by * gridDim.x + blockIdx.x) * 4u + w; };
-        uint32_t cov = kTileNotCovering;
-        if constexpr (COVER) {
-            if ((p.flags & RWR_FLAG_TILE_COVER) != 0u) cov = to_const_space(p.tile_lists)[cover_at(wu)];
-        }
-        rwait();
-        if constexpr (COVER) asm volatile("" ::"s"(T.p0[0]), "s"(T.p0[1]), "s"(T.p0[2]), "s"(T.e0[0]), "s"(T.e0[1]), "s"(T.e0[2]));
-        __syncthreads();
-        best.idx = u2{idx, idx};
-        last_idx = idx;
-        n_tested = 1u;
-        if (AUX) dbg_listed = dbg_tested = 1u;
-        if (COVER && cov == kTileCovered) {
-            triangle_covered(T, tnum, O, D, best.t, best.u, best.v, best.ndotd);
-            best.have = i2{-1, -1};
-            depth_tex = 1.0f - to_non_linear_depth_fast(best.t);
-            obj = i2{(int)idx, (int)idx};
-            win_t = best.t;
-        } else {
-            f2 u, v;
-            best.have = triangle_hit(T, tnum, O, D, best.t, u, v, best.ndotd);
-            best.u = best.have ? u : splat(0.0f);
-            best.v = best.have ? v : splat(0.0f);
-            const bool fast = !__any(any2(best.have & ~depth_fast_domain(best.t)));
-            const f2 depth = fast ? to_non_linear_depth_fast(best.t) : to_non_linear_depth(best.t);
-            const i2 win = best.have & ~(depth >= 1.0f);
-            depth_tex = win ? (1.0f - depth) : splat(0.0f);
-            obj = win ? i2{(int)idx, (int)idx} : i2{-1, -1};
-            win_t = win ? best.t : splat(0.0f);
-            if (COVER && cov != kTileNotCovering) {
-                const bool all = fast && hit_div_num_domain(tnum) && hit_div_lanes_in_domain(abs2(best.ndotd)) &&
-                                 __builtin_amdgcn_ballot_w64((win.x & win.y) != 0) == __builtin_amdgcn_read_exec();
-                uint32_t w = wu;
-                asm volatile("" : "+s"(w));
-                if (all && lane == 0u) const_cast<uint32_t *>(p.tile_lists)[cover_at(w)] = kTileCovered;
-            }
-        }
-    } else {
-
-    const float tx0 = (float)tile_x0, ty0 = (float)tile_y0;
-    const uint32_t sph = classed ? (cls >> kTileSphereShift) & 0xffu : 0xffu;
-    for (uint32_t s = 0; sph != 0u && s < p.n_spheres; s++) {
-        if (classed ? ((sph >> s) & 1u) == 0u
-                    : (CULL && ((tx0 + kTileWf < p.sphere_rect[s][0]) || (tx0 > p.sphere_rect[s][2]) ||
-                                (ty0 + kTileHf < p.sphere_rect[s][1]) || (ty0 > p.sphere_rect[s][3]))))
-            continue;
-        f2 t = splat(0.0f);
-        const i2 hit = sphere_ray_intersect_t(ld3(p.spheres[s].center), p.spheres[s].radius, O, D, t);
-        if (any2(hit)) {
-            const f2 current_depth = 1.0f - depth_tex;
-            const f2 depth = to_non_linear_depth(t);
-            const i2 win = hit & ~(depth >= current_depth);
-            depth_tex = win ? (1.0f - depth) : depth_tex;
-            obj = win ? i2{-2 - (int)s, -2 - (int)s} : obj;
-            win_t = win ? t : win_t;
-        }
-    }
-
-    if constexpr (CULL) {
-        const TileRect tile_rect = {tx0, ty0, tx0 + kTileWf, ty0 + kTileHf};
-        if (lists) {
-            rwait();
-            __syncthreads();
-#pragma unroll
-            for (uint32_t k = 0; k < kTileListWords / 2u; k++) {
-                unsigned long long m = live ? ((unsigned long long)set[2u * k + 1u] << 32 | set[2u * k]) : 0ull;
-                if (AUX) dbg_listed += (uint32_t)__popcll(m);
-                while (m) {
-                    const uint32_t idx = 64u * k + (uint32_t)__builtin_ctzll(m);
-                    m &= m - 1ull;
-                    intersect_and_select(tris[idx], to_const_space(p.tnum)[idx], idx, O, D, best);
-                    last_idx = idx;
-                    n_tested++;
-                    if (AUX) dbg_tested++;
-                }
-            }
-        }
-        for (uint32_t base = 0; base < n_list; base += 256u) {
-            if (base) {
-                __syncthreads();
-                load_round(base);
-            }
-            rwait();
-            __syncthreads();
-            const uint32_t n_round = min(n_list - base, 256u);
-            for (uint32_t b = 0; b < n_round; b += 64u) {
-                const uint32_t i = b + lane;
-                const float4 q0 = s_rec[0][i], q1 = s_rec[1][i], q2 = s_rec[2][i], q3 = s_rec[3][i];
-                const FrameTri rec = {q0.x, q0.y, q0.z, q0.w, {q1.x, q1.y, q1.z}, q1.w,
-                                      {q2.x, q2.y, q2.z}, q2.w, {q3.x, q3.y, q3.z}, q3.w};
-                const uint32_t my_face = s_face[i];
-                unsigned long long m = live ? __builtin_amdgcn_ballot_w64(i < n_round && !rect_culls(rec, tile_rect)) : 0ull;
-                if (AUX) dbg_listed += (uint32_t)__popcll(m);
-                while (m) {
-                    const uint32_t bit = (uint32_t)__builtin_ctzll(m);
-                    m &= m - 1ull;
-                    const uint32_t idx = (uint32_t)__builtin_amdgcn_readlane((int)my_face, (int)bit);
-                    if (FUSED) intersect_and_select(load_tri_record(tris_c + idx), tnum_c[idx], idx, O, D, best);
-                    else intersect_and_select(tris[idx], to_const_space(p.tnum)[idx], idx, O, D, best);
-                    last_idx = idx;
-                    n_tested++;
-                    if (AUX) dbg_tested++;
-                }
-            }
-        }
-        if (n_list == 0u && !lists) {
-            rwait();
-            __syncthreads();
-        }
-    } else {
-        rwait();
-        __syncthreads();
-        for (uint32_t base = 0; base < n_list; base += 64u) {
-            unsigned long long m = __ballot(base + lane < n_list);
-            if (AUX) dbg_listed += (uint32_t)__popcll(m);
-            while (m) {
-                const uint32_t idx = base + (uint32_t)__builtin_ctzll(m);
-                m &= m - 1ull;
-                intersect_and_select(tris[idx], to_const_space(p.tnum)[idx], idx, O, D, best);
-                last_idx = idx;
-                n_tested++;
-                if (AUX) dbg_tested++;
-            }
-        }
-    }
-    if (any2(best.have)) {
-        const f2 current_depth = 1.0f - depth_tex;
-        const bool fast = !__any(any2(best.have & ~depth_fast_domain(best.t)));
-        const f2 depth = fast ? to_non_linear_depth_fast(best.t) : to_non_linear_depth(best.t);
-        const i2 win = best.have & ~(depth >= current_depth);
-        depth_tex = win ? (1.0f - depth) : depth_tex;
-        obj = win ? i2{(int)best.idx.x, (int)best.idx.y} : obj;
-        win_t = win ? best.t : win_t;
-    }
-    }
-
-    const PairSlot ps = pair_slot(px0, py);
-    store_depth(ps, depth_tex);
-
-    uint32_t rgba[2] = {0u, 0u};
-    float4 cf[2];
-    if (AUX) cf[0] = cf[1] = make_float4(0.0f, 0.0f, 0.0f, 0.0f);
-    if (any2(obj < -1)) {
-#pragma unroll
-        for (int k = 0; k < 2; k++) {
-            const int o = k ? obj.y : obj.x;
-            if (o < -1) {
-                const f3 Dk = lane3(D, k);
-                const f3 center = ld3(p.spheres[-2 - o].center);
-                float t = 0.0f;
-                (void)sphere_ray_intersect_t(center, p.spheres[-2 - o].radius, O, Dk, t);
-                const f3 c = shade_sphere(cnormalize(sub3(along(O, t, Dk), center)), Dk);
-                rgba[k] = pack_rgba8(c.x, c.y, c.z, 2.0f);
-                if (AUX) cf[k] = make_float4(c.x, c.y, c.z, 2.0f);
-            }
-        }
-    }
-    if (__any(any2(obj >= 0))) {
-        f2 cr, cg, cb;
-        QuadTex qt = tex;
-        qt.lut = s_lut;
-        const ShadeRec unused = {};
-        if (NMAP) shade_mesh_pair<true, false, true, FrameParams, QuadTex>(p, shade, qt, obj, unused, best, D, cr, cg, cb);
-        else if (p.n_materials > 1u) shade_mesh_pair<true, false, false, FrameParams, QuadTex>(p, shade, qt, obj, unused, best, D, cr, cg, cb);
-        else if (n_tested == 1u) {
-            const ShadeRec last_shade = way == kWayOne ? one_shade : FUSED ? load_shade_record(shade_c + last_idx) : shade[last_idx];
-            shade_mesh_pair<false, true, false, FrameParams, QuadTex>(p, shade, qt, obj, last_shade, best, D, cr, cg, cb);
-        } else shade_mesh_pair<false, false, false, FrameParams, QuadTex>(p, shade, qt, obj, unused, best, D, cr, cg, cb);
-        pack_mesh(obj, cr, cg, cb, rgba, cf);
-    }
-    store_colour(ps, rgba, cf, obj, win_t, dbg_listed, dbg_tested);
+__global__ void __launch_bounds__(256, 8)
+k_primary_p2_lean(const float4 *__restrict__ ray_colp, const float4 *__restrict__ ray_row, const uint32_t *__restrict__ tile_lists,
+                  const float *__restrict__ lut_src, uint32_t row_begin, uint32_t row_pitch,
+                  const FrameParams p, const TriRecord *__restrict__ tris, const ShadeRec *__restrict__ shade,
+                  const QuadTex tex, const Targets tg)
+{
+    constexpr bool AUX = false, CULL = true, NMAP = false, FUSED = false, PLANE = true, COVER = true, LISTS = true;
+    const FrameTri *ftris = nullptr;
+    const uint32_t n_tris = 0u, bins_enabled = 0u;
+    const int32_t mesh_x0 = 0, mesh_y0 = 0, mesh_x1 = 0, mesh_y1 = 0;
+    const FusedSetup fs{};
+    const auto tl = [&]() { return tile_lists; };
+#include "rwr_primary_p2_body.h"
 }
 
 uint32_t primary_p2_fused_rows(const FrameParams &fp, uint32_t n_blocks)
@@ -399,8 +47,10 @@
 
 hipError_t launch_primary_p2(hipStream_t s, const FrameParams &fp, const TriRecord *tris, const ShadeRec *shade,
                              const FrameTri *ftris, const QuadTex &tex, const Targets &tg, hipEvent_t ev_start,
-                             hipEvent_t ev_stop, const FusedSetup *fused, const RayPlane *plane)
+                             hipEvent_t ev_stop, const FusedSetup *fused, const RayPlane *plane, bool *lean)
 {
+    const bool lean_allowed = lean && *lean;
+    if (lean) *lean = false;
     if (fp.row_end <= fp.row_begin || fp.width == 0) return hipSuccess;
     if (fp.row_pitch % kStripRows != 0u) return hipErrorInvalidValue;
     if (!tex.lut) return hipErrorInvalidValue;
@@ -418,7 +68,11 @@
         const float4 *const pxy = plane->xy, *const pz = reinterpret_cast<const float4 *>(plane->z);
 #define RWR_P2_LAUNCH_PLANE(A, V) hipExtLaunchKernelGGL((k_primary_p2<A, true, false, false, true, V>), grid, block, 0, s, ev_start, ev_stop, 0, ftris, pxy, pz, \
     fp.n_tris, fp.row_begin, fp.bins.enabled, fp.row_pitch, fp.mesh_px[0], fp.mesh_px[1], fp.mesh_px[2], fp.mesh_px[3], fp, tris, shade, tex, tg, fs)
-        if (aux && cover) RWR_P2_LAUNCH_PLANE(true, true);
+        if (lean_allowed && cover && !aux && fp.tile_lists && (fp.flags & RWR_FLAG_TILE_CLASS) != 0u && fp.n_materials <= 1u) {
+            hipExtLaunchKernelGGL(k_primary_p2_lean, grid, block, 0, s, ev_start, ev_stop, 0, pxy, pz, fp.tile_lists, tex.lut, fp.row_begin, fp.row_pitch,
+                                  fp, tris, shade, tex, tg);
+            *lean = true;
+        } else if (aux && cover) RWR_P2_LAUNCH_PLANE(true, true);
         else if (aux) RWR_P2_LAUNCH_PLANE(true, false);
         else if (cover) RWR_P2_LAUNCH_PLANE(false, true);
         else RWR_P2_LAUNCH_PLANE(false, false);
diff --git a/rust-wgpu-raytracing_amd/csrc/render_reference.cpp b/rust-wgpu-raytracing_amd/csrc/render_reference.cpp
--- a/rust-wgpu-raytracing_amd/csrc/render_reference.cpp
+++ b/rust-wgpu-raytracing_amd/csrc/render_reference.cpp
@@ -134,10 +134,12 @@
             ctx->tile_cover_frames++;
             ctx->last_cover_frames = ++sl.cover_frames;
         }
+        bool lean = ctx->lean_rest;
         RWR_HIP_CHECK(launch_primary_p2(stream, fp, ctx->d_tris.ptr, ctx->d_shade.ptr, sl.d_ftris.ptr, quad_tex, tg,
                                         timing.dispatch ? ctx->timing_events[2 * ctx->timing_pairs].h : nullptr,
                                         timing.dispatch ? ctx->timing_events[2 * ctx->timing_pairs + 1].h : nullptr, nullptr,
-                                        load ? &plane : nullptr));
+                                        load ? &plane : nullptr, &lean));
+        if (lean) ctx->lean_rest_frames++;
     }
     }
     return RWR_OK;
diff --git a/rust-wgpu-raytracing_amd/csrc/rwr_context.h b/rust-wgpu-raytracing_amd/csrc/rwr_context.h
--- a/rust-wgpu-raytracing_amd/csrc/rwr_context.h
+++ b/rust-wgpu-raytracing_amd/csrc/rwr_context.h
@@ -227,6 +227,8 @@
     bool tile_cover = true;
     uint64_t tile_cover_frames = 0;
     uint32_t last_cover_frames = 0;
+    bool lean_rest = true;
+    uint64_t lean_rest_frames = 0;
     rwr::DeviceBuffer<rwr::BvhNode4> d_bvh_nodes;
     rwr::DeviceBuffer<uint32_t> d_bvh_leaf_faces;
     uint32_t bvh_n_nodes = 0, bvh_depth = 0;
diff --git a/rust-wgpu-raytracing_amd/csrc/rwr_internal.h b/rust-wgpu-raytracing_amd/csrc/rwr_internal.h
--- a/rust-wgpu-raytracing_amd/csrc/rwr_internal.h
+++ b/rust-wgpu-raytracing_amd/csrc/rwr_internal.h
@@ -257,7 +257,8 @@
 struct FusedSetup;
 hipError_t launch_primary_p2(hipStream_t s, const FrameParams &fp, const TriRecord *tris, const ShadeRec *shade,
                              const FrameTri *ftris, const QuadTex &tex, const Targets &tg, hipEvent_t ev_start = nullptr,
-                             hipEvent_t ev_stop = nullptr, const FusedSetup *fused = nullptr, const RayPlane *plane = nullptr);
+                             hipEvent_t ev_stop = nullptr, const FusedSetup *fused = nullptr, const RayPlane *plane = nullptr,
+                             bool *lean = nullptr);
 uint32_t primary_p2_fused_rows(const FrameParams &fp, uint32_t n_blocks);
 hipError_t launch_wf_primary(hipStream_t s, const FrameParams &fp, const TriRecord *tris, const ShadeRec *shade,
                              const FrameTri *ftris, const float4 *tex, const Targets &tg,
diff --git a/rust-wgpu-raytracing_amd/csrc/rwr_primary_p2_body.h b/rust-wgpu-raytracing_amd/csrc/rwr_primary_p2_body.h
--- /dev/null
+++ b/rust-wgpu-raytracing_amd/csrc/rwr_primary_p2_body.h
@@ -0,0 +1,399 @@
+    static_assert(!LISTS || (PLANE && COVER && !AUX), "the lean form is the resting frame's: rays from the plane, cover words, no extra outputs");
+    static_assert(!PLANE || (CULL && !NMAP && !FUSED), "the loading form exists for the culled two-launch frame without normal maps");
+    static_assert(!COVER || (CULL && !NMAP && !FUSED), "cover words lie beside the face sets of the culled two-launch frame; normal maps take the general path");
+    const uint32_t wave = threadIdx.x >> 6, lane = threadIdx.x & 63u;
+    uint32_t by = blockIdx.y;
+    const_ptr<TriRecord> tris_c = nullptr;
+    const_ptr<ShadeRec> shade_c = nullptr;
+    const_ptr<float> tnum_c = nullptr;
+    if (FUSED) {
+        if (blockIdx.y < fs.extra_rows) {
+            const uint32_t f = blockIdx.y * gridDim.x + blockIdx.x;
+            if (f < fs.n_blocks) {
+                frame_setup_block(f, fs.n_blocks, fs.cc, p.cam, p.width, p.height, fs.cull, tris, n_tris, fs.nb_tris, fs.out);
+                __threadfence();
+                __syncthreads();
+                if (threadIdx.x == 0u) atomicAdd(fs.flag, 1u);
+            }
+            return;
+        }
+        by -= fs.extra_rows;
+        __shared__ uint32_t s_ready;
+        if (wave == 0u) {
+            uint32_t spins = 0;
+            bool ok = true;
+            while (__hip_atomic_load(fs.flag, __ATOMIC_RELAXED, __HIP_MEMORY_SCOPE_AGENT) - fs.flag_base < fs.n_blocks) {
+                __builtin_amdgcn_s_sleep(16);
+                if (++spins > (1u << 15)) { ok = false; break; }
+            }
+            if (lane == 0u) {
+                s_ready = ok ? 1u : 0u;
+                if (!ok) atomicOr(fs.flag + 1, 1u);
+            }
+        }
+        __syncthreads();
+        if (s_ready == 0u) return;
+        asm volatile("" : "+s"(ftris), "+s"(ray_colp), "+s"(ray_row));
+        const float *tn = p.tnum;
+        asm volatile("" : "+s"(tn));
+        tnum_c = to_const_space(tn);
+        tris_c = to_const_space(tris);
+        shade_c = to_const_space(shade);
+    }
+    const uint32_t blk_x0 = blockIdx.x * 64u;
+#if RWR_P2_TILE_32x4
+    const uint32_t tile_x0 = blk_x0 + (wave & 1u) * 32u;
+    const uint32_t tile_y0 = row_begin + by * row_pitch + (wave >> 1) * 4u;
+    const uint32_t px0 = tile_x0 + 2u * (lane & 15u), py = tile_y0 + (lane >> 4);
+    constexpr float kTileWf = 32.0f, kTileHf = 4.0f;
+#else
+    const uint32_t tile_x0 = blk_x0 + wave * 16u;
+    const uint32_t tile_y0 = p.row_begin + by * row_pitch;
+    const uint32_t px0 = tile_x0 + 2u * (lane & 7u), py = tile_y0 + (lane >> 3);
+    constexpr float kTileWf = 16.0f, kTileHf = 8.0f;
+#endif
+
+    const uint32_t wu = __builtin_amdgcn_readfirstlane(wave);
+    uint32_t n_list = n_tris;
+    const uint32_t *__restrict__ src = nullptr;
+    bool live = true;
+    if (CULL && !LISTS) {
+        if (bins_enabled) {
+            const uint32_t bin = ((by * row_pitch) / kBinH) * p.bins.bins_x + blk_x0 / kBinW;
+            const uint32_t off = p.bins.offsets[bin];
+            if (off != kBinNoList) {
+                n_list = p.bins.counts[bin];
+                src = p.bins.lists + off;
+            }
+        }
+        const int32_t bx0 = (int32_t)blk_x0, by0 = (int32_t)(row_begin + by * row_pitch);
+#if RWR_P2_TILE_32x4
+        const int32_t sx0 = bx0 + (int32_t)(wu & 1u) * 32, sy0 = by0 + (int32_t)(wu >> 1) * 4;
+        const int32_t sx1 = sx0 + 32, sy1 = sy0 + 4;
+#else
+        const int32_t sx0 = bx0 + (int32_t)wu * 16, sy0 = by0;
+        const int32_t sx1 = sx0 + 16, sy1 = sy0 + 8;
+#endif
+        if (sx1 < mesh_x0 || sx0 > mesh_x1 || sy1 < mesh_y0 || sy0 > mesh_y1) live = false;
+        if (bx0 + 64 < mesh_x0 || bx0 > mesh_x1 || by0 + 8 < mesh_y0 || by0 > mesh_y1) n_list = 0u;
+    }
+    n_list = __builtin_amdgcn_readfirstlane(n_list);
+    const bool lists = LISTS || (CULL && !FUSED && tl() != nullptr);
+    uint32_t set[kTileListWords] = {};
+    if (lists) {
+        if constexpr (!LISTS) {
+            const const_ptr<uint32_t> rec = to_const_space(tl()) + ((by * gridDim.x + blockIdx.x) * 4u + wu) * kTileListWords;
+#pragma unroll
+            for (uint32_t k = 0; k < kTileListWords; k++) set[k] = rec[k];
+        }
+        n_list = 0u;
+    }
+    const bool classed = LISTS || (lists && (p.flags & RWR_FLAG_TILE_CLASS) != 0u);
+    uint32_t cls = 0u;
+    if (classed) cls = to_const_space(tl())[gridDim.x * gridDim.y * 4u * kTileListWords + (by * gridDim.x + blockIdx.x) * 4u + wu];
+    if constexpr (LISTS) live = (cls & kTileFacesMask) != kTileFacesNone;
+    constexpr bool kRounds = CULL && !LISTS;
+    __shared__ float4 s_rec[kRounds ? 4 : 1][kRounds ? 256 : 1];
+    __shared__ uint32_t s_face[kRounds ? 256 : 1];
+    __shared__ float s_lut[256];
+    const uint32_t slot = 64u * wu + lane;
+    auto load_round = [&](uint32_t base) {
+        const uint32_t e = base + slot;
+        if (e < n_list) {
+            const uint32_t f = src ? src[e] : e;
+            s_face[slot] = f;
+            const char *r = reinterpret_cast<const char *>(ftris + f);
+#pragma unroll
+            for (int k = 0; k < 4; k++)
+                __builtin_amdgcn_global_load_lds((__attribute__((address_space(1))) void *)(r + 16 * k),
+                                                 (__attribute__((address_space(3))) void *)&s_rec[k][64u * wu], 16, 0, 0);
+        }
+    };
+    auto rwait = []() { __builtin_amdgcn_s_waitcnt(0xF70); };
+    if (kRounds && !lists) load_round(0u);
+    if constexpr (LISTS) {
+        if ((reinterpret_cast<uintptr_t>(lut_src) & 15u) == 0u) {
+            __builtin_amdgcn_global_load_lds((__attribute__((address_space(1))) void *)(lut_src + 4u * lane),
+                                             (__attribute__((address_space(3))) void *)&s_lut[0], 16, 0, 0);
+        } else {
+#pragma unroll
+            for (uint32_t k = 0; k < 4u; k++)
+                __builtin_amdgcn_global_load_lds((__attribute__((address_space(1))) void *)(lut_src + 64u * k + lane),
+                                                 (__attribute__((address_space(3))) void *)&s_lut[64u * k], 4, 0, 0);
+        }
+    } else {
+        __builtin_amdgcn_global_load_lds((__attribute__((address_space(1))) void *)(lut_src + threadIdx.x),
+                                         (__attribute__((address_space(3))) void *)&s_lut[64u * wu], 4, 0, 0);
+    }
+    auto lut_ready = [&]() {
+        rwait();
+        if constexpr (LISTS) asm volatile("" ::: "memory");
+        else __syncthreads();
+    };
+
+    const f3 O = ld3(p.cam.origin);
+    v3 D;
+    if constexpr (PLANE) {
+        const uint32_t i = (by * gridDim.x + blockIdx.x) * 256u + threadIdx.x;
+        const float4 dxy = ray_colp[i];
+        const float2 dz = reinterpret_cast<const float2 *>(ray_row)[i];
+        D = v3{f2{dxy.x, dxy.y}, f2{dxy.z, dxy.w}, f2{dz.x, dz.y}};
+    } else {
+        D = pixel_pair_ray_dir_tab(p.cam, ray_colp, ray_row, px0, py);
+    }
+
+    struct PairSlot { bool in_frame, both, pair_store; uint32_t o; };
+    auto pair_slot = [&](uint32_t px0, uint32_t py) {
+        PairSlot ps;
+        ps.in_frame = py < p.row_end && px0 < p.width;
+        ps.o = py * p.width + px0;
+        ps.both = px0 + 1u < p.width;
+        ps.pair_store = ps.both && (ps.o & 1u) == 0u;
+        return ps;
+    };
+    auto store_depth = [&](const PairSlot &ps, f2 depth_tex) {
+        if (ps.in_frame) {
+            if (ps.pair_store) {
+                __builtin_nontemporal_store(depth_tex, reinterpret_cast<f2 *>(tg.depth + ps.o));
+            } else {
+                tg.depth[ps.o] = depth_tex.x;
+                if (ps.both) tg.depth[ps.o + 1] = depth_tex.y;
+            }
+        }
+    };
+    auto store_colour = [&](const PairSlot &ps, const uint32_t (&rgba)[2], const float4 (&cf)[2], i2 obj, f2 win_t, uint32_t dbg_listed,
+                            uint32_t dbg_tested) {
+        if (ps.in_frame) {
+            const uint32_t o = ps.o;
+            if (ps.pair_store) {
+                __builtin_nontemporal_store(u2{rgba[0], rgba[1]}, reinterpret_cast<u2 *>(reinterpret_cast<uint32_t *>(tg.color) + o));
+            } else {
+                reinterpret_cast<uint32_t *>(tg.color)[o] = rgba[0];
+                if (ps.both) reinterpret_cast<uint32_t *>(tg.color)[o + 1] = rgba[1];
+            }
+            if (AUX) {
+                const bool dbg = (p.flags & RWR_FLAG_DEBUG_COUNTS) != 0;
+                reinterpret_cast<float4 *>(tg.color_f32)[o] = cf[0];
+                tg.obj_id[o] = dbg ? (int32_t)dbg_listed : obj.x;
+                tg.hit_t[o] = dbg ? (float)dbg_tested : win_t.x;
+                if (ps.both) {
+                    reinterpret_cast<float4 *>(tg.color_f32)[o + 1] = cf[1];
+                    tg.obj_id[o + 1] = dbg ? (int32_t)dbg_listed : obj.y;
+                    tg.hit_t[o + 1] = dbg ? (float)dbg_tested : win_t.y;
+                }
+            }
+        }
+    };
+    auto pack_mesh = [&](i2 obj, f2 cr, f2 cg, f2 cb, uint32_t (&rgba)[2], float4 (&cf)[2]) {
+        const f2 sr = cr * 255.0f, sg = cg * 255.0f, sb = cb * 255.0f;
+        const uint32_t m0 = pack_rgba8_scaled(sr.x, sg.x, sb.x, 0xff000000u);
+        const uint32_t m1 = pack_rgba8_scaled(sr.y, sg.y, sb.y, 0xff000000u);
+        rgba[0] = obj.x >= 0 ? m0 : rgba[0];
+        rgba[1] = obj.y >= 0 ? m1 : rgba[1];
+        if (AUX) {
+            if (obj.x >= 0) cf[0] = make_float4(cr.x, cg.x, cb.x, 2.0f);
+            if (obj.y >= 0) cf[1] = make_float4(cr.y, cg.y, cb.y, 2.0f);
+        }
+    };
+
+    constexpr uint32_t kWayNone = 0u, kWayOne = 1u, kWayAll = 2u;
+    const uint32_t tile_class = cls & (kTileFacesMask | kTileSphereMask);
+    const uint32_t way = !classed ? kWayAll
+                         : tile_class == kTileFacesNone ? kWayNone
+                         : (tile_class == kTileFacesOne && !NMAP && (LISTS || !(p.n_materials > 1u))) ? kWayOne : kWayAll;
+    f2 depth_tex = splat(0.0f), win_t = splat(0.0f);
+    i2 obj = i2{-1, -1};
+    MeshHit2 best;
+    best.have = i2{0, 0};
+    best.t = best.u = best.v = best.ndotd = splat(0.0f);
+    best.idx = u2{0u, 0u};
+    uint32_t dbg_listed = 0, dbg_tested = 0;
+    uint32_t n_tested = 0;
+    uint32_t last_idx = 0;
+    ShadeRec one_shade = {};
+    if (way == kWayNone) {
+        lut_ready();
+    } else if (way == kWayOne) {
+        const uint32_t idx = (cls >> kTileFaceShift) & 0xffu;
+        const TriRecord T = tris[idx];
+        const float tnum = to_const_space(p.tnum)[idx];
+        one_shade = shade[idx];
+        constexpr uint32_t kTileNotCovering = 2u;
+        auto cover_at = [&](uint32_t w) { return gridDim.x * gridDim.y * 4u * (kTileListWords + 1u) + (by * gridDim.x + blockIdx.x) * 4u + w; };
+        uint32_t cov = kTileNotCovering;
+        if constexpr (COVER) {
+            if (LISTS || (p.flags & RWR_FLAG_TILE_COVER) != 0u) cov = to_const_space(tl())[cover_at(wu)];
+        }
+        rwait();
+        if constexpr (COVER && !LISTS) asm volatile("" ::"s"(T.p0[0]), "s"(T.p0[1]), "s"(T.p0[2]), "s"(T.e0[0]), "s"(T.e0[1]), "s"(T.e0[2]));
+        if constexpr (LISTS) asm volatile("" ::: "memory");
+        else __syncthreads();
+        best.idx = u2{idx, idx};
+        last_idx = idx;
+        n_tested = 1u;
+        if (AUX) dbg_listed = dbg_tested = 1u;
+        if (COVER && cov == kTileCovered) {
+            triangle_covered(T, tnum, O, D, best.t, best.u, best.v, best.ndotd);
+            best.have = i2{-1, -1};
+            depth_tex = 1.0f - to_non_linear_depth_fast(best.t);
+            obj = i2{(int)idx, (int)idx};
+            win_t = best.t;
+        } else {
+            f2 u, v;
+            best.have = triangle_hit(T, tnum, O, D, best.t, u, v, best.ndotd);
+            best.u = best.have ? u : splat(0.0f);
+            best.v = best.have ? v : splat(0.0f);
+            const bool fast = !__any(any2(best.have & ~depth_fast_domain(best.t)));
+            const f2 depth = fast ? to_non_linear_depth_fast(best.t) : to_non_linear_depth(best.t);
+            const i2 win = best.have & ~(depth >= 1.0f);
+            depth_tex = win ? (1.0f - depth) : splat(0.0f);
+            obj = win ? i2{(int)idx, (int)idx} : i2{-1, -1};
+            win_t = win ? best.t : splat(0.0f);
+            if (COVER && cov != kTileNotCovering) {
+                const bool all = fast && hit_div_num_domain(tnum) && hit_div_lanes_in_domain(abs2(best.ndotd)) &&
+                                 __builtin_amdgcn_ballot_w64((win.x & win.y) != 0) == __builtin_amdgcn_read_exec();
+                uint32_t w = wu;
+                asm volatile("" : "+s"(w));
+                if (all && lane == 0u) const_cast<uint32_t *>(tl())[cover_at(w)] = kTileCovered;
+            }
+        }
+    } else {
+    if constexpr (LISTS) {
+        const const_ptr<uint32_t> rec = to_const_space(tl()) + ((by * gridDim.x + blockIdx.x) * 4u + wu) * kTileListWords;
+#pragma unroll
+        for (uint32_t k = 0; k < kTileListWords; k++) set[k] = rec[k];
+    }
+
+    const float tx0 = (float)tile_x0, ty0 = (float)tile_y0;
+    const uint32_t sph = classed ? (cls >> kTileSphereShift) & 0xffu : 0xffu;
+    for (uint32_t s = 0; sph != 0u && s < p.n_spheres; s++) {
+        if (classed ? ((sph >> s) & 1u) == 0u
+                    : (CULL && ((tx0 + kTileWf < p.sphere_rect[s][0]) || (tx0 > p.sphere_rect[s][2]) ||
+                                (ty0 + kTileHf < p.sphere_rect[s][1]) || (ty0 > p.sphere_rect[s][3]))))
+            continue;
+        f2 t = splat(0.0f);
+        const i2 hit = sphere_ray_intersect_t(ld3(p.spheres[s].center), p.spheres[s].radius, O, D, t);
+        if (any2(hit)) {
+            const f2 current_depth = 1.0f - depth_tex;
+            const f2 depth = to_non_linear_depth(t);
+            const i2 win = hit & ~(depth >= current_depth);
+            depth_tex = win ? (1.0f - depth) : depth_tex;
+            obj = win ? i2{-2 - (int)s, -2 - (int)s} : obj;
+            win_t = win ? t : win_t;
+        }
+    }
+
+    if constexpr (CULL) {
+        const TileRect tile_rect = {tx0, ty0, tx0 + kTileWf, ty0 + kTileHf};
+        if (lists) {
+            lut_ready();
+#pragma unroll
+            for (uint32_t k = 0; k < kTileListWords / 2u; k++) {
+                unsigned long long m = live ? ((unsigned long long)set[2u * k + 1u] << 32 | set[2u * k]) : 0ull;
+                if (AUX) dbg_listed += (uint32_t)__popcll(m);
+                while (m) {
+                    const uint32_t idx = 64u * k + (uint32_t)__builtin_ctzll(m);
+                    m &= m - 1ull;
+                    intersect_and_select(tris[idx], to_const_space(p.tnum)[idx], idx, O, D, best);
+                    last_idx = idx;
+                    n_tested++;
+                    if (AUX) dbg_tested++;
+                }
+            }
+        }
+        if constexpr (kRounds) {
+        for (uint32_t base = 0; base < n_list; base += 256u) {
+            if (base) {
+                __syncthreads();
+                load_round(base);
+            }
+            rwait();
+            __syncthreads();
+            const uint32_t n_round = min(n_list - base, 256u);
+            for (uint32_t b = 0; b < n_round; b += 64u) {
+                const uint32_t i = b + lane;
+                const float4 q0 = s_rec[0][i], q1 = s_rec[1][i], q2 = s_rec[2][i], q3 = s_rec[3][i];
+                const FrameTri rec = {q0.x, q0.y, q0.z, q0.w, {q1.x, q1.y, q1.z}, q1.w,
+                                      {q2.x, q2.y, q2.z}, q2.w, {q3.x, q3.y, q3.z}, q3.w};
+                const uint32_t my_face = s_face[i];
+                unsigned long long m = live ? __builtin_amdgcn_ballot_w64(i < n_round && !rect_culls(rec, tile_rect)) : 0ull;
+                if (AUX) dbg_listed += (uint32_t)__popcll(m);
+                while (m) {
+                    const uint32_t bit = (uint32_t)__builtin_ctzll(m);
+                    m &= m - 1ull;
+                    const uint32_t idx = (uint32_t)__builtin_amdgcn_readlane((int)my_face, (int)bit);
+                    if (FUSED) intersect_and_select(load_tri_record(tris_c + idx), tnum_c[idx], idx, O, D, best);
+                    else intersect_and_select(tris[idx], to_const_space(p.tnum)[idx], idx, O, D, best);
+                    last_idx = idx;
+                    n_tested++;
+                    if (AUX) dbg_tested++;
+                }
+            }
+        }
+        if (n_list == 0u && !lists) {
+            rwait();
+            __syncthreads();
+        }
+        }
+    } else {
+        rwait();
+        __syncthreads();
+        for (uint32_t base = 0; base < n_list; base += 64u) {
+            unsigned long long m = __ballot(base + lane < n_list);
+            if (AUX) dbg_listed += (uint32_t)__popcll(m);
+            while (m) {
+                const uint32_t idx = base + (uint32_t)__builtin_ctzll(m);
+                m &= m - 1ull;
+                intersect_and_select(tris[idx], to_const_space(p.tnum)[idx], idx, O, D, best);
+                last_idx = idx;
+                n_tested++;
+                if (AUX) dbg_tested++;
+            }
+        }
+    }
+    if (any2(best.have)) {
+        const f2 current_depth = 1.0f - depth_tex;
+        const bool fast = !__any(any2(best.have & ~depth_fast_domain(best.t)));
+        const f2 depth = fast ? to_non_linear_depth_fast(best.t) : to_non_linear_depth(best.t);
+        const i2 win = best.have & ~(depth >= current_depth);
+        depth_tex = win ? (1.0f - depth) : depth_tex;
+        obj = win ? i2{(int)best.idx.x, (int)best.idx.y} : obj;
+        win_t = win ? best.t : win_t;
+    }
+    }
+
+    const PairSlot ps = pair_slot(px0, py);
+    store_depth(ps, depth_tex);
+
+    uint32_t rgba[2] = {0u, 0u};
+    float4 cf[2];
+    if (AUX) cf[0] = cf[1] = make_float4(0.0f, 0.0f, 0.0f, 0.0f);
+    if (any2(obj < -1)) {
+#pragma unroll
+        for (int k = 0; k < 2; k++) {
+            const int o = k ? obj.y : obj.x;
+            if (o < -1) {
+                const f3 Dk = lane3(D, k);
+                const f3 center = ld3(p.spheres[-2 - o].center);
+                float t = 0.0f;
+                (void)sphere_ray_intersect_t(center, p.spheres[-2 - o].radius, O, Dk, t);
+                const f3 c = shade_sphere(cnormalize(sub3(along(O, t, Dk), center)), Dk);
+                rgba[k] = pack_rgba8(c.x, c.y, c.z, 2.0f);
+                if (AUX) cf[k] = make_float4(c.x, c.y, c.z, 2.0f);
+            }
+        }
+    }
+    if (__any(any2(obj >= 0))) {
+        f2 cr, cg, cb;
+        QuadTex qt = tex;
+        qt.lut = s_lut;
+        const ShadeRec unused = {};
+        if (NMAP) shade_mesh_pair<true, false, true, FrameParams, QuadTex>(p, shade, qt, obj, unused, best, D, cr, cg, cb);
+        else if (!LISTS && p.n_materials > 1u) shade_mesh_pair<true, false, false, FrameParams, QuadTex>(p, shade, qt, obj, unused, best, D, cr, cg, cb);
+        else if (n_tested == 1u) {
+            const ShadeRec last_shade = way == kWayOne ? one_shade : FUSED ? load_shade_record(shade_c + last_idx) : shade[last_idx];
+            shade_mesh_pair<false, true, false, FrameParams, QuadTex>(p, shade, qt, obj, last_shade, best, D, cr, cg, cb);
+        } else shade_mesh_pair<false, false, false, FrameParams, QuadTex>(p, shade, qt, obj, unused, best, D, cr, cg, cb);
+        pack_mesh(obj, cr, cg, cb, rgba, cf);
+    }
+    store_colour(ps, rgba, cf, obj, win_t, dbg_listed, dbg_tested);
```

Result: faster. 237,000 Mray/s, median of 6 (+8.7%).
